# RchalYang/torchrl

Hardware: AMD Instinct MI355X
Metric: env_steps_per_sec_ppo_2048env_halfcheetah_shape (higher is better)
Workload: dtype f32

## Files before the change

include/trl_hip.h:

```cpp
#ifndef TRL_HIP_H
#define TRL_HIP_H
#include <stdint.h>
#ifdef __cplusplus
extern "C" {
#endif

#define TRL_OK            0
#define TRL_EINVAL       -1
#define TRL_EUNSUPPORTED -2

#define TRL_ACT_TANH 0
#define TRL_ACT_RELU 1
#define TRL_ACT_NONE 2

const char* trl_last_error(void);
int trl_abi_version(void);

int trl_gae_f32(const float* rewards, const float* values, const float* terminals,
                const float* time_limits, const float* last_value, const float* last_terminal,
                float* advs, float* rets, int T, int N,
                float gamma, float tau, int tl_filter, void* stream);
int trl_discount_reward_f32(const float* rewards, const float* values, const float* terminals,
                            const float* time_limits, const float* last_value, const float* last_terminal,
                            float* advs, float* rets, int T, int N,
                            float gamma, int tl_filter, void* stream);

int trl_gather_rows_f32(const float* src, const int64_t* row_idx, float* dst,
                        int n_rows, int64_t row_elems, int64_t src_rows, void* stream);
int trl_gather_rows_u8(const uint8_t* src, const int64_t* row_idx, uint8_t* dst,
                       int n_rows, int64_t row_bytes, int64_t src_rows, void* stream);
int trl_gather_rows_multi(const void* const* src, void* const* dst, const int64_t* row_bytes, int n_keys,
                          const int64_t* row_idx, const double* update_count, int n_rows, int64_t src_rows,
                          void* stream);

int trl_adv_stats_f64(const float* advs, const int64_t* row_idx, int n_mb, int rows_mb,
                      int N, double* raw_out, void* stream);
int64_t trl_ppo_epoch_prologue_workspace(int n_mb);
int trl_ppo_epoch_prologue_f64(const float* advs, const int64_t* row_idx, int n_mb, int rows_mb, int N, double* raw_out,
                               void* workspace, double* zero, int64_t zero_doubles, int n_copies, void* const* copy_dst,
                               const void* const* copy_src, const int64_t* copy_words, void* stream);

int trl_mlp2_forward_f32(const float* params, const float* x, float* out,
                         int M, int D, int H, int O, int act, void* stream);
int trl_mlp2_forward_supported(int D, int H, int O);

typedef struct trl_rollout_t {
  const float* pf_params;
  const float* vf_params;
  int D, H, A, act;
  int tanh_action;
  const float* env_A;
  const float* env_B;
  float reward_scale;
  int horizon;
  int64_t env_seed_base;
  float*   cur_obs;
  int32_t* t_env;
  int32_t* cur_step;
  int32_t* episode_idx;
  float*   ep_return;
  const float* noise;
  int64_t noise_step0;
  int deterministic;
  float *obs, *next_obs, *acts, *values, *rewards, *terminals, *time_limits;
  float *old_logp;
  int rows, top;
  int N, n_steps;
  int max_episode_frames;
  float discount;
  double*  epoch_reward;
  int32_t* ep_count;
  float*   ep_log;
  int ep_cap;
  int step0;
  double* norm_state;
  float*  policy_obs;
  double* norm_workspace;
  float norm_clip;
  int norm_update;
  int normalize_partial_reset;
  double* clear_header;
  float* boot_values;
  void* publish_dst; const void* publish_src; int64_t publish_words;
  const uint32_t* noise_flag; uint32_t noise_stamp;
  const float* stage_src; float* stage_dst; int64_t stage_n;
  const uint32_t* stage_ready; uint32_t stage_job; uint32_t* stage_state; uint32_t* stage_ack;
  void* value_wait_event;
} trl_rollout_t;
int trl_rollout_synth_f32(const trl_rollout_t* args, void* stream);
int trl_rollout_supported(int D, int H, int A, int act);
int trl_rollout_synth_cat_f32(const trl_rollout_t* args, int64_t noise_seed, int64_t env_offset, void* stream);
int trl_rollout_cat_supported(int D, int H, int A, int act);
int trl_rollout_synth_sd_f32(const trl_rollout_t* args, void* stream);
int trl_rollout_sd_supported(int D, int H, int A, int act);
int trl_stage_h2d_f32(const float* host_src, float* dev_dst, int64_t n, uint32_t* state, uint32_t stamp, void* stream);
int trl_rollout_norm_workspace(int N);
int trl_rollout_norm_max_envs(int D, int H, int A, int act);

int trl_synth_reset_f32(float* cur_obs, int32_t* t_env, int32_t* cur_step, int32_t* episode_idx,
                        float* ep_return, const uint8_t* mask, int N, int D, int64_t env_seed_base,
                        void* stream);

int trl_gauss_logp_f32(const float* mean, const float* acts, const float* logstd, float* out,
                       int B, int A, int tanh_action, void* stream);

#define TRL_LOSS_PPO_CLIP 0
#define TRL_LOSS_A2C      1
#define TRL_LOSS_REINFORCE 2
typedef struct trl_ppo_batch_t {
  const float *obs, *acts, *advs, *rets, *old_values, *old_logp;
  const int64_t* row_idx;
  int rows_mb, N;
  const double* adv_raw;
  double n_global;
  const float* pf_params; const float* vf_params;
  int D, H, A, act;
  float clip_para, entropy_coeff;
  int clipped_value_loss, tanh_action;
  int loss_mode;
  float* partial;
  double* scal_partial;
  int n_wg;
  int n_wg_pf;
} trl_ppo_batch_t;
int trl_ppo_partial_stride(int D, int H, int A);
int trl_ppo_wg_split(int D, int H, int A, int n_tiles, int n_wg);
int trl_ppo_minibatch_grad_f32(const trl_ppo_batch_t* args, void* stream);
int trl_ppo_reduce_f32(const float* partial, const double* scal_partial, int n_wg, int n_wg_pf,
                       int D, int H, int A, const float* pf_params, float* grads, double* info,
                       void* stream);

int trl_ppo_generic_losses_workspace(int B, int A);
int trl_ppo_generic_losses_f32(const float* mean, const float* logstd, const float* acts, const float* advs,
                               const float* old_logp, const float* v, const float* rets, const float* v_old,
                               const double* adv_raw, double n_global, int B, int A, float clip_para,
                               float entropy_coeff, int clipped_value_loss, int tanh_action, int loss_mode,
                               float* d_mean, float* d_v, float* d_logstd, double* info, double* workspace,
                               void* stream);
int trl_cat_losses_workspace(int B, int A);
int trl_cat_losses_f32(const float* logits, const float* acts, const float* advs, const float* old_logp, const float* v,
                       const float* rets, const float* v_old, const double* adv_raw, double n_global, int B, int A,
                       float clip_para, float entropy_coeff, int clipped_value_loss, int loss_mode, float* d_logits,
                       float* d_v, double* info, double* workspace, void* stream);
int trl_gauss_sd_losses_workspace(int B, int A);
int trl_gauss_sd_losses_f32(const float* head, const float* acts, const float* advs, const float* old_logp, const float* v,
                            const float* rets, const float* v_old, const double* adv_raw, double n_global, int B, int A,
                            float clip_para, float entropy_coeff, int clipped_value_loss, int tanh_action, int loss_mode,
                            float* d_head, float* d_v, double* info, double* workspace, void* stream);

int trl_adv_normalize_f32(const float* advs, const double* adv_raw, double n_global, int B, float eps, float* out,
                          void* stream);
int trl_mse_value_loss_f32(const float* v, const float* rets, int B, double n_global, float* d_v, double* loss_sum,
                           void* stream);
int trl_vmpo_losses_workspace(int n, int A);
int trl_vmpo_losses_f32(const float* mean, const float* target_mean, const float* logstd, const float* target_logstd,
                        const float* acts, const float* adv_n, float* dual_state, int n, int A, int tanh_action,
                        float eta_eps, float alpha_eps, float dual_lr, float* d_mean, float* d_logstd, double* info,
                        double* workspace, void* stream);

int trl_trpo_surrogate_workspace(int n, int A);
int trl_trpo_surrogate_f32(const float* mean, const float* logstd, const float* acts, const float* adv_n, int n, int A,
                           int tanh_action, float entropy_coeff, float* d_mean, float* d_logstd, double* info,
                           double* workspace, void* stream);
int trl_jvp_gate_f32(const float* a, const float* b, const float* h, int act, int64_t n, float* out, void* stream);
int trl_fisher_scale_f32(const float* d_mu, const float* logstd, int n, int A, float* out, void* stream);
int trl_ratio_loss_f32(const float* logp_new, const float* logp_old, const float* adv_n, int n, double* out, void* stream);

typedef struct trl_adam_t {
  float* params; const float* grads; float* exp_avg; float* exp_avg_sq;
  int n_groups;
  int group_sizes[4];
  float group_lr[4];
  float max_norm;
  float beta1, beta2, eps;
  int step_count;
  float grad_scale;
  float* norms_out;
  int device_state;
  double* step_state;
  const float* device_lr;
} trl_adam_t;
int trl_clip_adam_f32(const trl_adam_t* args, void* stream);
int trl_clip_adam_polyak_f32(const trl_adam_t* args, float* target, const float* source, int64_t n, float tau,
                             const void* raw, int raw_bytes, void* ring, int slots, void* stream);
int trl_fold_clip_adam_polyak_workspace(void);
int trl_fold_clip_adam_polyak_f32(int count, const float* const* part, const int* n, const int* splits,
                                  const trl_adam_t* args, float* target, int64_t target_off, int64_t target_n, float tau,
                                  const void* raw, int raw_bytes, void* ring, int slots, void* workspace, void* stream);
int trl_ppo_reduce_adam_workspace(int D, int H, int A);
int trl_ppo_reduce_adam_f32(const float* partial, const double* scal_partial, int n_wg, int n_wg_pf,
                            int D, int H, int A, float* grads, double* info,
                            const trl_adam_t* adam, float* workspace, void* stream);

int trl_ppo_reduce_adam_net_f32(const float* partial, const double* scal_partial, int n_wg, int net,
                                int D, int H, int A, float* grads, double* info,
                                const trl_adam_t* adam, float* workspace, void* stream);

int trl_ppo_cat_supported(int D, int H, int A, int act);
int trl_ppo_cat_partial_stride(int D, int H, int A);
int trl_ppo_cat_minibatch_grad_f32(const trl_ppo_batch_t* args, void* stream);
int trl_ppo_cat_reduce_f32(const float* partial, const double* scal_partial, int n_wg, int n_wg_pf,
                           int D, int H, int A, const float* pf_params, float* grads, double* info,
                           void* stream);
int trl_ppo_cat_reduce_adam_workspace(int D, int H, int A);
int trl_ppo_cat_reduce_adam_f32(const float* partial, const double* scal_partial, int n_wg, int n_wg_pf,
                                int D, int H, int A, float* grads, double* info,
                                const trl_adam_t* adam, float* workspace, void* stream);
int trl_ppo_cat_reduce_adam_net_f32(const float* partial, const double* scal_partial, int n_wg, int net,
                                    int D, int H, int A, float* grads, double* info,
                                    const trl_adam_t* adam, float* workspace, void* stream);

int trl_ppo_sd_supported(int D, int H, int A, int act);
int trl_ppo_sd_partial_stride(int D, int H, int A);
int trl_ppo_sd_scalar_stride(void);
int trl_ppo_sd_minibatch_grad_f32(const trl_ppo_batch_t* args, void* stream);
int trl_ppo_sd_reduce_f32(const float* partial, const double* scal_partial, int n_wg, int n_wg_pf,
                          int D, int H, int A, const float* pf_params, float* grads, double* info,
                          void* stream);
int trl_ppo_sd_reduce_adam_workspace(int D, int H, int A);
int trl_ppo_sd_reduce_adam_f32(const float* partial, const double* scal_partial, int n_wg, int n_wg_pf,
                               int D, int H, int A, float* grads, double* info,
                               const trl_adam_t* adam, float* workspace, void* stream);
int trl_ppo_sd_reduce_adam_net_f32(const float* partial, const double* scal_partial, int n_wg, int net,
                                   int D, int H, int A, float* grads, double* info,
                                   const trl_adam_t* adam, float* workspace, void* stream);

typedef struct trl_comm trl_comm_t;
int trl_comm_unique_id_bytes(void);
int trl_comm_peer_handle_bytes(void);
int trl_comm_max_ranks(void);
int trl_comm_get_unique_id(void* id_out);
int trl_comm_init(trl_comm_t** comm, int rank, int world, const void* unique_id);
int trl_comm_peer_export(trl_comm_t* comm, void* handle_out);
int trl_comm_peer_open(trl_comm_t* comm, const void* handles);
int trl_comm_peer_ready(const trl_comm_t* comm);
int trl_comm_set_wait_footprint(trl_comm_t* comm, int blocks);
int trl_comm_peer_buffer_kind(const trl_comm_t* comm);
int trl_comm_peer_enable(trl_comm_t* comm, int on);
int trl_comm_has_rccl(const trl_comm_t* comm);
int trl_comm_error(trl_comm_t* comm);
int trl_comm_error_peek(trl_comm_t* comm);
int trl_comm_error_detail(trl_comm_t* comm, int32_t* out);
int trl_comm_link_info(int dev_a, int dev_b, int32_t* out);
int trl_comm_destroy(trl_comm_t* comm);
int trl_allreduce_sum_f32(float* buf, int64_t n, trl_comm_t* comm, void* stream);
int trl_allreduce_f64(double* buf, int64_t n, int period, uint64_t max_mask, trl_comm_t* comm, void* stream);
int trl_ppo_reduce_adam_xrank_f32(const float* partial, const double* scal_partial, int n_wg, int n_wg_pf,
                                  int D, int H, int A, float* grads, double* info,
                                  const trl_adam_t* adam, float* workspace, trl_comm_t* comm, void* stream);
int trl_ppo_reduce_adam_xrank_net_f32(const float* partial, const double* scal_partial, int n_wg, int net,
                                      int D, int H, int A, float* grads, double* info,
                                      const trl_adam_t* adam, float* workspace, trl_comm_t* comm, void* stream);

int trl_linear_fwd_f32(const float* x, const float* w, const float* bias, float* y,
                       int M, int K, int N, int act, void* stream);
int trl_linear_fwd_workspace(int M, int K, int N);
int trl_linear_fwd_splitk_group_f32(int G, const float* const* x, const float* const* w, const float* const* bias,
                                    float* const* y, int M, int K, int N, int act, float* workspace, void* stream);
int trl_linear_fwd_splitk_f32(const float* x, const float* w, const float* bias, float* y,
                              int M, int K, int N, int act, float* workspace, void* stream);
int trl_linear_bwd_input_f32(const float* dy, const float* y_gate, int gate_act, const float* w,
                             float* dx, int M, int K, int N, void* stream);
int trl_linear_bwd_input_workspace(int M, int K, int N);
int trl_linear_bwd_input_splitk_f32(const float* dy, const float* y_gate, int gate_act, const float* w, float* dx,
                                    float* workspace, int M, int K, int N, void* stream);
int trl_linear_bwd_weight_workspace(int M, int K, int N);
int trl_linear_bwd_weight_f32(const float* dy, const float* y_gate, int gate_act, const float* x,
                              float* dw, float* db, float* workspace, int M, int K, int N,
                              void* stream);
int trl_linear_fwd_group_f32(int G, const float* const* x, const float* const* w, const float* const* bias,
                             float* const* y, int M, int K, int N, int act, void* stream);
int trl_linear_bwd_input_group_f32(int G, const float* const* dy, const float* const* y_gate, int gate_act,
                                   const float* const* w, float* const* dx, int M, int K, int N, void* stream);
int trl_linear_bwd_weight_group_f32(int G, const float* const* dy, const float* const* y_gate, int gate_act,
                                    const float* const* x, float* const* dw, float* const* db, float* workspace,
                                    int M, int K, int N, void* stream);

int trl_linear_bwd_weight_splits(int M, int K, int N);
int trl_linear_bwd_weight_partials_group_f32(int G, const float* const* dy, const float* const* y_gate, int gate_act,
                                             const float* const* x, int want_db, float* workspace, int M, int K,
                                             int N, void* stream);
int trl_fold_partials_multi_f32(int count, const float* const* part, float* const* out, const int* n,
                                const int* splits, void* stream);
int trl_fold_scope_begin(void);
int trl_fold_scope_end(void* stream);
int trl_linear_bwd_weight_multi_splits(int M, int K, int N);
int trl_linear_bwd_weight_partials_multi_f32(int G, const float* const* dy, const float* const* y_gate, int gate_act,
                                             const float* const* x, const int* K, const int* N, int want_db,
                                             float* const* workspace, int M, void* stream);

int trl_mlp3_forward_ok(int D, int H1, int H2, int O);
int trl_mlp3_forward_group_f32(int G, const float* const* x, const float* const* w1, const float* const* b1,
                               const float* const* w2, const float* const* b2, const float* const* w3,
                               const float* const* b3, float* const* h1, float* const* h2, float* const* y, int M,
                               int D, int O, int act, int last_act, void* stream);

int trl_concat2_f32(const float* a, const float* b, float* out, int rows, int fa, int fb, void* stream);
int trl_tanh_gauss_rsample_fwd_f32(const float* head, const float* eps, float* act, float* logp,
                                   int B, int A, int tanh_action, void* stream);
int trl_tanh_gauss_rsample_bwd_f32(const float* head, const float* eps, const float* act,
                                   const float* d_act, const float* d_logp_ptr, float d_logp_mul,
                                   float w_std, float w_mean, float* d_head, int B, int A,
                                   int tanh_action, void* stream);
int trl_tanh_gauss_rsample_bwd_cols_f32(const float* head, const float* eps, const float* act, const float* dx1,
                                        const float* dx2, int ld, int off, const float* d_logp_ptr,
                                        float d_logp_mul, float w_std, float w_mean, float* d_head, int B,
                                        int A, int tanh_action, void* stream);
int trl_sac_policy_grad_supported(int H, int A);
int trl_sac_policy_grad_f32(int n, const float* const* dy, const float* const* y, int gate_act, const float* const* w,
                            int H, int ldw, int off, const float* head, const float* eps, const float* act,
                            const float* d_logp_ptr, float d_logp_mul, float w_std, float w_mean, float* d_head, int B,
                            int A, int tanh_action, const float* head_w, const float* head_h, int head_act, float* head_dz,
                            void* stream);
int trl_sac_samples_f32(const float* head, const float* head2, float* eps1, const float* eps2,
                        const double* step_state, int64_t seed, const float* obs, const float* acts,
                        const float* next_obs, float* new_a, float* logp, float* next_a, float* next_logp,
                        float* x_sa, float* x_next, float* x_new, int B, int D, int A, int tanh_action,
                        double* mom_part, void* stream);
int trl_sac_alpha_step_f32(const float* logp, int B, float target_entropy, float lr, float beta1,
                           float beta2, float eps, float* state, float* out, void* stream);
int trl_sac_losses_f32(const float* q1, const float* q2, const float* tq1, const float* tq2,
                       const float* logp_next, const float* rew, const float* term, const float* q1n,
                       const float* q2n, const float* logp, const float* alpha, float gamma, int B,
                       float* dq1, float* dq2, float* dq1n, float* dq2n, double* sums,
                       float* alpha_state, float* alpha_out, float target_entropy, float lr, float beta1,
                       float beta2, float eps, const double* mom_part, int A, double* mom_out, void* stream);
int trl_sacv_samples_f32(const float* head, float* eps, const double* step_state, int64_t seed, const float* obs,
                         const float* acts, float* new_a, float* logp, float* x_sa, float* x_new, int B, int D, int A,
                         int tanh_action, double* mom_part, void* stream);
int trl_sacv_losses_f32(const float* q1, const float* q2, const float* tv, const float* rew, const float* term,
                        const float* v, const float* q1n, const float* q2n, const float* logp, const float* alpha,
                        float gamma, int B, int n, float* dq1, float* dq2, float* dv, float* dq1n, float* dq2n,
                        double* sums, float* alpha_state, float* alpha_out, float target_entropy, float lr, float beta1,
// ... 179 lines not shown
```

torchrl_amd/_C.py:

```python
import ctypes as C
import os

import torch

_HERE = os.path.dirname(os.path.abspath(__file__))
LIB_PATH = os.environ.get("TRL_LIB") or os.path.join(_HERE, "lib", "libtrl_hip.so")
_lib = None

ACT_TANH, ACT_RELU, ACT_NONE = 0, 1, 2
ACT_CODES = {"tanh": ACT_TANH, "relu": ACT_RELU}

c_float_p = C.POINTER(C.c_float)
c_double_p = C.POINTER(C.c_double)
c_i64_p = C.POINTER(C.c_int64)
c_i32_p = C.POINTER(C.c_int32)
c_u8_p = C.POINTER(C.c_uint8)


EAGER_FALLBACKS = {}


def note_eager(site, why=""):
    EAGER_FALLBACKS[site] = EAGER_FALLBACKS.get(site, 0) + 1
    if os.environ.get("TRL_STRICT") == "1":
        raise TrlError("%s left the HIP path (%s) and TRL_STRICT=1" % (site, why))
    if EAGER_FALLBACKS[site] == 1:
        import logging
        logging.getLogger("torchrl_amd").warning("%s: a CUDA tensor takes the eager PyTorch route (%s); "
                                                 "this is outside the HIP hot path", site, why)


def eager_fallback_count():
    return sum(EAGER_FALLBACKS.values())


class TrlError(RuntimeError):
    pass


class RolloutArgs(C.Structure):
    _fields_ = [
        ("pf_params", C.c_void_p), ("vf_params", C.c_void_p),
        ("D", C.c_int), ("H", C.c_int), ("A", C.c_int), ("act", C.c_int),
        ("tanh_action", C.c_int),
        ("env_A", C.c_void_p), ("env_B", C.c_void_p),
        ("reward_scale", C.c_float), ("horizon", C.c_int), ("env_seed_base", C.c_int64),
        ("cur_obs", C.c_void_p), ("t_env", C.c_void_p), ("cur_step", C.c_void_p),
        ("episode_idx", C.c_void_p), ("ep_return", C.c_void_p),
        ("noise", C.c_void_p), ("noise_step0", C.c_int64), ("deterministic", C.c_int),
        ("obs", C.c_void_p), ("next_obs", C.c_void_p), ("acts", C.c_void_p), ("values", C.c_void_p),
        ("rewards", C.c_void_p), ("terminals", C.c_void_p), ("time_limits", C.c_void_p),
        ("old_logp", C.c_void_p),
        ("rows", C.c_int), ("top", C.c_int), ("N", C.c_int), ("n_steps", C.c_int),
        ("max_episode_frames", C.c_int), ("discount", C.c_float),
        ("epoch_reward", C.c_void_p), ("ep_count", C.c_void_p), ("ep_log", C.c_void_p),
        ("ep_cap", C.c_int), ("step0", C.c_int),
        ("norm_state", C.c_void_p), ("policy_obs", C.c_void_p), ("norm_workspace", C.c_void_p),
        ("norm_clip", C.c_float), ("norm_update", C.c_int), ("normalize_partial_reset", C.c_int),
        ("clear_header", C.c_void_p), ("boot_values", C.c_void_p),
        ("publish_dst", C.c_void_p), ("publish_src", C.c_void_p), ("publish_words", C.c_int64),
        ("noise_flag", C.c_void_p), ("noise_stamp", C.c_uint32),
        ("stage_src", C.c_void_p), ("stage_dst", C.c_void_p), ("stage_n", C.c_int64),
        ("stage_ready", C.c_void_p), ("stage_job", C.c_uint32), ("stage_state", C.c_void_p), ("stage_ack", C.c_void_p),
        ("value_wait_event", C.c_void_p),
    ]


LOSS_PPO_CLIP, LOSS_A2C, LOSS_REINFORCE = 0, 1, 2


class PpoBatchArgs(C.Structure):
    _fields_ = [
        ("obs", C.c_void_p), ("acts", C.c_void_p), ("advs", C.c_void_p), ("rets", C.c_void_p),
        ("old_values", C.c_void_p), ("old_logp", C.c_void_p),
        ("row_idx", C.c_void_p), ("rows_mb", C.c_int), ("N", C.c_int),
        ("adv_raw", C.c_void_p), ("n_global", C.c_double),
        ("pf_params", C.c_void_p), ("vf_params", C.c_void_p),
        ("D", C.c_int), ("H", C.c_int), ("A", C.c_int), ("act", C.c_int),
        ("clip_para", C.c_float), ("entropy_coeff", C.c_float),
        ("clipped_value_loss", C.c_int), ("tanh_action", C.c_int), ("loss_mode", C.c_int),
        ("partial", C.c_void_p), ("scal_partial", C.c_void_p), ("n_wg", C.c_int), ("n_wg_pf", C.c_int),
    ]


class AdamArgs(C.Structure):
    _fields_ = [
        ("params", C.c_void_p), ("grads", C.c_void_p), ("exp_avg", C.c_void_p), ("exp_avg_sq", C.c_void_p),
        ("n_groups", C.c_int), ("group_sizes", C.c_int * 4), ("group_lr", C.c_float * 4),
        ("max_norm", C.c_float), ("beta1", C.c_float), ("beta2", C.c_float), ("eps", C.c_float),
        ("step_count", C.c_int), ("grad_scale", C.c_float), ("norms_out", C.c_void_p),
        ("device_state", C.c_int), ("step_state", C.c_void_p), ("device_lr", C.c_void_p),
    ]


def adam_args(flat, grads, m, v, sizes, lrs, *, offset=0, max_norm=0.0, eps=1e-8, grad_scale=1.0, norms_out=None,
              step_state=None, step_count=0, device_state=0, device_lr=None):
    a = AdamArgs()
    a.params, a.grads, a.exp_avg, a.exp_avg_sq = (t.data_ptr() + int(offset) * t.element_size() for t in (flat, grads, m, v))
    a.n_groups = len(sizes)
    for k, (size, lr) in enumerate(zip(sizes, lrs)):
        a.group_sizes[k], a.group_lr[k] = size, lr
    a.max_norm, a.beta1, a.beta2, a.eps = max_norm, 0.9, 0.999, eps
    a.step_count, a.grad_scale, a.norms_out, a.step_state = step_count, grad_scale, norms_out, step_state
    a.device_state, a.device_lr = device_state, device_lr
    return a


class ConvRiders(C.Structure):
    _fields_ = [("n_perm", C.c_int), ("perm_src", C.c_void_p * 4), ("perm_dst", C.c_void_p * 4), ("perm_cout", C.c_int * 4),
                ("perm_c", C.c_int * 4), ("perm_khw", C.c_int * 4), ("n_dx", C.c_int), ("dx_w", C.c_void_p * 4),
                ("dx_ws", C.c_void_p * 4), ("dx_cin", C.c_int * 4), ("dx_cout", C.c_int * 4), ("dx_kh", C.c_int * 4),
                ("dx_kw", C.c_int * 4), ("dx_sh", C.c_int * 4), ("dx_sw", C.c_int * 4)]


SIGNATURES = {
    "trl_last_error": (C.c_char_p, []),
    "trl_abi_version": (C.c_int, []),
    "trl_gae_f32": (C.c_int, [C.c_void_p] * 8 + [C.c_int, C.c_int, C.c_float, C.c_float, C.c_int, C.c_void_p]),
    "trl_discount_reward_f32": (C.c_int, [C.c_void_p] * 8 + [C.c_int, C.c_int, C.c_float, C.c_int, C.c_void_p]),
    "trl_gather_rows_f32": (C.c_int, [C.c_void_p, C.c_void_p, C.c_void_p, C.c_int, C.c_int64, C.c_int64, C.c_void_p]),
    "trl_gather_rows_u8": (C.c_int, [C.c_void_p, C.c_void_p, C.c_void_p, C.c_int, C.c_int64, C.c_int64, C.c_void_p]),
    "trl_gather_rows_multi": (C.c_int, [C.c_void_p, C.c_void_p, C.c_void_p, C.c_int, C.c_void_p, C.c_void_p, C.c_int,
                                       C.c_int64, C.c_void_p]),
    "trl_adv_stats_f64": (C.c_int, [C.c_void_p, C.c_void_p, C.c_int, C.c_int, C.c_int, C.c_void_p, C.c_void_p]),
    "trl_ppo_epoch_prologue_workspace": (C.c_int64, [C.c_int]),
    "trl_ppo_epoch_prologue_f64": (C.c_int, [C.c_void_p, C.c_void_p, C.c_int, C.c_int, C.c_int, C.c_void_p, C.c_void_p,
                                           C.c_void_p, C.c_int64, C.c_int, C.c_void_p, C.c_void_p, C.c_void_p, C.c_void_p]),
    "trl_mlp2_forward_f32": (C.c_int, [C.c_void_p, C.c_void_p, C.c_void_p, C.c_int, C.c_int, C.c_int, C.c_int, C.c_int, C.c_void_p]),
    "trl_rollout_synth_f32": (C.c_int, [C.POINTER(RolloutArgs), C.c_void_p]),
    "trl_rollout_supported": (C.c_int, [C.c_int, C.c_int, C.c_int, C.c_int]),
    "trl_rollout_synth_cat_f32": (C.c_int, [C.POINTER(RolloutArgs), C.c_int64, C.c_int64, C.c_void_p]),
    "trl_rollout_cat_supported": (C.c_int, [C.c_int, C.c_int, C.c_int, C.c_int]),
    "trl_rollout_synth_sd_f32": (C.c_int, [C.POINTER(RolloutArgs), C.c_void_p]),
    "trl_rollout_sd_supported": (C.c_int, [C.c_int, C.c_int, C.c_int, C.c_int]),
    "trl_stage_h2d_f32": (C.c_int, [C.c_void_p, C.c_void_p, C.c_int64, C.c_void_p, C.c_uint32, C.c_void_p]),
    "trl_ppo_partial_stride": (C.c_int, [C.c_int, C.c_int, C.c_int]),
    "trl_mlp2_forward_supported": (C.c_int, [C.c_int, C.c_int, C.c_int]),
    "trl_ppo_minibatch_grad_f32": (C.c_int, [C.POINTER(PpoBatchArgs), C.c_void_p]),
    "trl_ppo_wg_split": (C.c_int, [C.c_int, C.c_int, C.c_int, C.c_int, C.c_int]),
    "trl_rollout_norm_workspace": (C.c_int, [C.c_int]),
    "trl_rollout_norm_max_envs": (C.c_int, [C.c_int, C.c_int, C.c_int, C.c_int]),
    "trl_frame_stream_append_u8": (C.c_int, [C.c_void_p, C.c_void_p, C.c_void_p, C.c_void_p, C.c_int, C.c_int, C.c_int, C.c_int, C.c_int, C.c_void_p]),
    "trl_frame_stream_gather_u8": (C.c_int, [C.c_void_p, C.c_void_p, C.c_void_p, C.c_int, C.c_int, C.c_void_p, C.c_void_p, C.c_void_p,
                                             C.c_int, C.c_int, C.c_int, C.c_int, C.c_void_p]),
    "trl_detac_losses_f32": (C.c_int, [C.c_void_p] * 7 + [C.c_float, C.c_int] + [C.c_void_p] * 5),
    "trl_noisy_action_f32": (C.c_int, [C.c_void_p, C.c_void_p, C.c_float, C.c_float, C.c_float, C.c_float, C.c_void_p, C.c_int64, C.c_void_p]),
    "trl_gauss_explore_f32": (C.c_int, [C.c_void_p, C.c_void_p, C.c_void_p, C.c_void_p, C.c_void_p, C.c_int, C.c_int, C.c_int, C.c_void_p]),
    "trl_onpolicy_bookkeep_f32": (C.c_int, [C.c_void_p, C.c_void_p, C.c_void_p, C.c_float, C.c_void_p, C.c_void_p, C.c_void_p, C.c_int,
                                            C.c_void_p, C.c_void_p, C.c_void_p, C.c_void_p, C.c_void_p, C.c_int, C.c_int, C.c_int, C.c_void_p]),
    "trl_select_on_flag_f32": (C.c_int, [C.c_void_p, C.c_void_p, C.c_void_p, C.c_void_p, C.c_int64, C.c_void_p]),
    "trl_comm_unique_id_bytes": (C.c_int, []),
    "trl_comm_peer_handle_bytes": (C.c_int, []),
    "trl_comm_max_ranks": (C.c_int, []),
    "trl_comm_get_unique_id": (C.c_int, [C.c_void_p]),
    "trl_comm_init": (C.c_int, [C.POINTER(C.c_void_p), C.c_int, C.c_int, C.c_void_p]),
    "trl_comm_peer_export": (C.c_int, [C.c_void_p, C.c_void_p]),
    "trl_comm_peer_open": (C.c_int, [C.c_void_p, C.c_void_p]),
    "trl_comm_peer_ready": (C.c_int, [C.c_void_p]),
    "trl_comm_peer_enable": (C.c_int, [C.c_void_p, C.c_int]),
    "trl_comm_has_rccl": (C.c_int, [C.c_void_p]),
    "trl_comm_error": (C.c_int, [C.c_void_p]),
    "trl_comm_error_peek": (C.c_int, [C.c_void_p]),
    "trl_comm_error_detail": (C.c_int, [C.c_void_p, C.c_void_p]),
    "trl_comm_link_info": (C.c_int, [C.c_int, C.c_int, C.c_void_p]),
    "trl_comm_set_wait_footprint": (C.c_int, [C.c_void_p, C.c_int]),
    "trl_comm_peer_buffer_kind": (C.c_int, [C.c_void_p]),
    "trl_comm_destroy": (C.c_int, [C.c_void_p]),
    "trl_allreduce_sum_f32": (C.c_int, [C.c_void_p, C.c_int64, C.c_void_p, C.c_void_p]),
    "trl_allreduce_f64": (C.c_int, [C.c_void_p, C.c_int64, C.c_int, C.c_uint64, C.c_void_p, C.c_void_p]),
    "trl_ppo_reduce_adam_xrank_f32": (C.c_int, [C.c_void_p, C.c_void_p, C.c_int, C.c_int, C.c_int, C.c_int, C.c_int, C.c_void_p,
                                                C.c_void_p, C.POINTER(AdamArgs), C.c_void_p, C.c_void_p, C.c_void_p]),
    "trl_select_on_mask_f32": (C.c_int, [C.c_void_p, C.c_int, C.c_void_p, C.c_void_p, C.c_void_p, C.c_int64, C.c_void_p]),
    "trl_norm_update_filt_f32": (C.c_int, [C.c_void_p, C.c_void_p, C.c_void_p, C.c_int, C.c_int, C.c_float, C.c_int, C.c_void_p]),
    "trl_norm_batch_moments_f64": (C.c_int, [C.c_void_p, C.c_int, C.c_int, C.c_void_p, C.c_void_p]),
    "trl_norm_shard_moments_f64": (C.c_int, [C.c_void_p, C.c_void_p, C.c_int, C.c_int, C.c_void_p, C.c_void_p]),
    "trl_norm_shard_merge_f64": (C.c_int, [C.c_void_p, C.c_void_p, C.c_int, C.c_void_p]),
    "trl_norm_merge_f64": (C.c_int, [C.c_void_p, C.c_void_p, C.c_int, C.c_void_p]),
    "trl_norm_filt_f32": (C.c_int, [C.c_void_p, C.c_void_p, C.c_void_p, C.c_int, C.c_int, C.c_float, C.c_void_p]),
    "trl_ppo_reduce_f32": (C.c_int, [C.c_void_p, C.c_void_p, C.c_int, C.c_int, C.c_int, C.c_int, C.c_int, C.c_void_p, C.c_void_p, C.c_void_p, C.c_void_p]),
    "trl_clip_adam_f32": (C.c_int, [C.POINTER(AdamArgs), C.c_void_p]),
    "trl_clip_adam_polyak_f32": (C.c_int, [C.POINTER(AdamArgs), C.c_void_p, C.c_void_p, C.c_int64, C.c_float, C.c_void_p, C.c_int,
                                          C.c_void_p, C.c_int, C.c_void_p]),
    "trl_ppo_reduce_adam_workspace": (C.c_int, [C.c_int, C.c_int, C.c_int]),
    "trl_ppo_reduce_adam_f32": (C.c_int, [C.c_void_p, C.c_void_p, C.c_int, C.c_int, C.c_int, C.c_int, C.c_int, C.c_void_p, C.c_void_p,
                                          C.POINTER(AdamArgs), C.c_void_p, C.c_void_p]),
    "trl_ppo_reduce_adam_net_f32": (C.c_int, [C.c_void_p, C.c_void_p, C.c_int, C.c_int, C.c_int, C.c_int, C.c_int, C.c_void_p, C.c_void_p,
                                              C.POINTER(AdamArgs), C.c_void_p, C.c_void_p]),
    "trl_ppo_reduce_adam_xrank_net_f32": (C.c_int, [C.c_void_p, C.c_void_p, C.c_int, C.c_int, C.c_int, C.c_int, C.c_int, C.c_void_p,
                                                    C.c_void_p, C.POINTER(AdamArgs), C.c_void_p, C.c_void_p, C.c_void_p]),
    "trl_ppo_cat_supported": (C.c_int, [C.c_int, C.c_int, C.c_int, C.c_int]),
    "trl_ppo_cat_partial_stride": (C.c_int, [C.c_int, C.c_int, C.c_int]),
    "trl_ppo_cat_minibatch_grad_f32": (C.c_int, [C.POINTER(PpoBatchArgs), C.c_void_p]),
    "trl_ppo_cat_reduce_f32": (C.c_int, [C.c_void_p, C.c_void_p, C.c_int, C.c_int, C.c_int, C.c_int, C.c_int, C.c_void_p, C.c_void_p, C.c_void_p, C.c_void_p]),
    "trl_ppo_cat_reduce_adam_workspace": (C.c_int, [C.c_int, C.c_int, C.c_int]),
    "trl_ppo_cat_reduce_adam_f32": (C.c_int, [C.c_void_p, C.c_void_p, C.c_int, C.c_int, C.c_int, C.c_int, C.c_int, C.c_void_p, C.c_void_p,
                                              C.POINTER(AdamArgs), C.c_void_p, C.c_void_p]),
    "trl_ppo_cat_reduce_adam_net_f32": (C.c_int, [C.c_void_p, C.c_void_p, C.c_int, C.c_int, C.c_int, C.c_int, C.c_int, C.c_void_p, C.c_void_p,
                                                  C.POINTER(AdamArgs), C.c_void_p, C.c_void_p]),
    "trl_ppo_sd_supported": (C.c_int, [C.c_int, C.c_int, C.c_int, C.c_int]),
    "trl_ppo_sd_partial_stride": (C.c_int, [C.c_int, C.c_int, C.c_int]),
    "trl_ppo_sd_scalar_stride": (C.c_int, []),
    "trl_ppo_sd_minibatch_grad_f32": (C.c_int, [C.POINTER(PpoBatchArgs), C.c_void_p]),
    "trl_ppo_sd_reduce_f32": (C.c_int, [C.c_void_p, C.c_void_p, C.c_int, C.c_int, C.c_int, C.c_int, C.c_int, C.c_void_p, C.c_void_p, C.c_void_p, C.c_void_p]),
    "trl_ppo_sd_reduce_adam_workspace": (C.c_int, [C.c_int, C.c_int, C.c_int]),
    "trl_ppo_sd_reduce_adam_f32": (C.c_int, [C.c_void_p, C.c_void_p, C.c_int, C.c_int, C.c_int, C.c_int, C.c_int, C.c_void_p, C.c_void_p,
                                              C.POINTER(AdamArgs), C.c_void_p, C.c_void_p]),
    "trl_ppo_sd_reduce_adam_net_f32": (C.c_int, [C.c_void_p, C.c_void_p, C.c_int, C.c_int, C.c_int, C.c_int, C.c_int, C.c_void_p, C.c_void_p,
                                                  C.POINTER(AdamArgs), C.c_void_p, C.c_void_p]),
    "trl_synth_reset_f32": (C.c_int, [C.c_void_p] * 6 + [C.c_int, C.c_int, C.c_int64, C.c_void_p]),
    "trl_gauss_logp_f32": (C.c_int, [C.c_void_p] * 4 + [C.c_int, C.c_int, C.c_int, C.c_void_p]),
    "trl_concat2_f32": (C.c_int, [C.c_void_p] * 3 + [C.c_int] * 3 + [C.c_void_p]),
    "trl_tanh_gauss_rsample_fwd_f32": (C.c_int, [C.c_void_p] * 4 + [C.c_int] * 3 + [C.c_void_p]),
    "trl_tanh_gauss_rsample_bwd_f32": (C.c_int, [C.c_void_p] * 5 + [C.c_float] * 3 + [C.c_void_p] + [C.c_int] * 3 + [C.c_void_p]),
    "trl_tanh_gauss_rsample_bwd_cols_f32": (C.c_int, [C.c_void_p] * 5 + [C.c_int] * 2 + [C.c_void_p] + [C.c_float] * 3 +
                                            [C.c_void_p] + [C.c_int] * 3 + [C.c_void_p]),
    "trl_fold_clip_adam_polyak_workspace": (C.c_int, []),
    "trl_fold_clip_adam_polyak_f32": (C.c_int, [C.c_int, C.c_void_p, C.c_void_p, C.c_void_p, C.POINTER(AdamArgs), C.c_void_p,
                                              C.c_int64, C.c_int64, C.c_float, C.c_void_p, C.c_int, C.c_void_p, C.c_int,
                                              C.c_void_p, C.c_void_p]),
    "trl_fold_scope_begin": (C.c_int, []),
    "trl_fold_scope_end": (C.c_int, [C.c_void_p]),
    "trl_sac_policy_grad_supported": (C.c_int, [C.c_int, C.c_int]),
    "trl_sac_policy_grad_f32": (C.c_int, [C.c_int, C.c_void_p, C.c_void_p, C.c_int, C.c_void_p, C.c_int, C.c_int, C.c_int] +
                                [C.c_void_p] * 4 + [C.c_float] * 3 + [C.c_void_p, C.c_int, C.c_int, C.c_int] +
                                [C.c_void_p, C.c_void_p, C.c_int, C.c_void_p, C.c_void_p]),
    "trl_sac_samples_f32": (C.c_int, [C.c_void_p] * 5 + [C.c_int64] + [C.c_void_p] * 10 + [C.c_int] * 4 +
                            [C.c_void_p, C.c_void_p]),
    "trl_moments_multi_f64": (C.c_int, [C.c_int] + [C.c_void_p] * 9 + [C.c_int, C.c_void_p, C.c_int, C.c_void_p, C.c_void_p]),
    "trl_sac_losses_f32": (C.c_int, [C.c_void_p] * 11 + [C.c_float, C.c_int] + [C.c_void_p] * 7 + [C.c_float] * 5 +
                           [C.c_void_p, C.c_int, C.c_void_p, C.c_void_p]),
    "trl_sacv_samples_f32": (C.c_int, [C.c_void_p] * 3 + [C.c_int64] + [C.c_void_p] * 6 + [C.c_int] * 4 +
                             [C.c_void_p, C.c_void_p]),
    "trl_sacv_losses_f32": (C.c_int, [C.c_void_p] * 10 + [C.c_float, C.c_int, C.c_int] + [C.c_void_p] * 8 + [C.c_float] * 5 +
                            [C.c_void_p, C.c_int, C.c_void_p, C.c_void_p]),
    "trl_synth_collect_step_f32": (C.c_int, [C.c_void_p] * 3 + [C.c_int64, C.c_int64, C.c_int] + [C.c_void_p] * 6 +
                                   [C.c_float, C.c_int, C.c_int, C.c_int64] + [C.c_void_p] * 6 + [C.c_int, C.c_void_p] +
                                   [C.c_void_p] * 4 + [C.c_int] * 6 + [C.c_void_p]),
    "trl_collector_bookkeep_f32": (C.c_int, [C.c_void_p] * 4 + [C.c_int] + [C.c_void_p] * 4 + [C.c_int] * 3 + [C.c_void_p]),
    "trl_sac_alpha_step_f32": (C.c_int, [C.c_void_p, C.c_int] + [C.c_float] * 5 + [C.c_void_p] * 3),
    "trl_slice_add_f32": (C.c_int, [C.c_void_p] * 3 + [C.c_int] * 4 + [C.c_void_p]),
    "trl_polyak_f32": (C.c_int, [C.c_void_p, C.c_void_p, C.c_int64, C.c_float, C.c_void_p]),
    "trl_philox_normal_f32": (C.c_int, [C.c_void_p, C.c_int64, C.c_int64, C.c_int64, C.c_void_p]),
    "trl_synth_env_step_f32": (C.c_int, [C.c_void_p] * 5 + [C.c_float, C.c_int] + [C.c_void_p] * 3 + [C.c_int] * 3 + [C.c_void_p]),
    "trl_im2col_f32": (C.c_int, [C.c_void_p, C.c_void_p] + [C.c_int] * 8 + [C.c_void_p]),
    "trl_im2col_u8_nchw": (C.c_int, [C.c_void_p, C.c_void_p] + [C.c_int] * 8 + [C.c_float, C.c_float, C.c_void_p]),
    "trl_col2im_f32": (C.c_int, [C.c_void_p, C.c_void_p] + [C.c_int] * 8 + [C.c_void_p]),
    "trl_conv_bwd_input_nhwc_ok": (C.c_int, [C.c_int] * 6),
    "trl_conv_bwd_input_nhwc_workspace": (C.c_int, [C.c_int] * 4),
    "trl_conv_bwd_input_nhwc_f32": (C.c_int, [C.c_void_p, C.c_void_p, C.c_int, C.c_void_p, C.c_void_p, C.c_void_p, C.c_int,
                                             C.c_void_p] + [C.c_int] * 10 + [C.c_void_p]),
    "trl_conv_bwd_input_nhwc_prep_f32": (C.c_int, [C.c_int] + [C.c_void_p] * 8 + [C.c_void_p]),
    "trl_transpose_bpc_gate_f32": (C.c_int, [C.c_void_p, C.c_void_p, C.c_int, C.c_int, C.c_void_p] + [C.c_int] * 3
                                   + [C.c_void_p]),
    "trl_transpose_bpc_f32": (C.c_int, [C.c_void_p, C.c_void_p] + [C.c_int] * 3 + [C.c_void_p]),
    "trl_conv_fwd_u8_f32": (C.c_int, [C.c_void_p] * 4 + [C.c_int] * 8 + [C.c_float, C.c_float, C.c_int, C.c_int] +
                            [C.POINTER(ConvRiders), C.c_void_p]),
    "trl_conv_fwd_u8_pair_f32": (C.c_int, [C.c_void_p] * 8 + [C.c_int] * 8 + [C.c_float, C.c_float, C.c_int, C.c_int] +
                                 [C.POINTER(ConvRiders), C.c_void_p]),
    "trl_conv_bwd_weight_workspace": (C.c_int, [C.c_int] * 9),
    "trl_conv_fwd_nhwc_f32": (C.c_int, [C.c_void_p] * 4 + [C.c_int] * 12 + [C.c_void_p]),
    "trl_conv_bwd_weight_nhwc_f32": (C.c_int, [C.c_void_p, C.c_void_p, C.c_int] + [C.c_void_p] * 4 + [C.c_int] * 9
                                     + [C.c_void_p]),
    "trl_conv_bwd_weight_u8_f32": (C.c_int, [C.c_void_p, C.c_void_p, C.c_int] + [C.c_void_p] * 4 + [C.c_int] * 8
                                   + [C.c_float, C.c_float, C.c_int, C.c_void_p]),
    "trl_dqn_td_loss_f32": (C.c_int, [C.c_void_p] * 6 + [C.c_float, C.c_int, C.c_int, C.c_void_p, C.c_void_p, C.c_void_p,
                                     C.c_int, C.c_void_p, C.c_void_p]),
    "trl_dqn_head_supported": (C.c_int, [C.c_int, C.c_int]),
    "trl_dqn_head_workspace": (C.c_int64, [C.c_int, C.c_int]),
    "trl_dqn_head_f32": (C.c_int, [C.c_void_p] * 10 + [C.c_float, C.c_int, C.c_int, C.c_int] + [C.c_void_p] * 7 +
                         [C.c_int, C.c_void_p, C.c_void_p, C.c_void_p]),
    "trl_quantile_huber_f32": (C.c_int, [C.c_void_p] * 6 + [C.c_float, C.c_int, C.c_int, C.c_int] + [C.c_void_p] * 4 +
                               [C.c_int, C.c_void_p, C.c_void_p]),
    "trl_boot_act_i64": (C.c_int, [C.c_void_p, C.c_void_p, C.c_int, C.c_int, C.c_int, C.c_void_p, C.c_void_p, C.c_void_p,
                                   C.c_void_p]),
    "trl_boot_heads_i64": (C.c_int, [C.c_void_p, C.c_void_p, C.c_int, C.c_int, C.c_int64, C.c_int64, C.c_int64, C.c_void_p]),
    "trl_boot_masks_f32": (C.c_int, [C.c_void_p, C.c_int, C.c_int, C.c_float, C.c_int64, C.c_int64, C.c_int64, C.c_void_p]),
    "trl_boot_td_loss_workspace": (C.c_int64, []),
    "trl_boot_td_loss_f32": (C.c_int, [C.c_void_p] * 7 + [C.c_float, C.c_int, C.c_int, C.c_int, C.c_void_p, C.c_void_p,
                                                          C.c_void_p, C.c_int, C.c_void_p, C.c_void_p, C.c_void_p]),
    "trl_boot_fold_f32": (C.c_int, [C.c_void_p, C.c_void_p, C.c_int, C.c_int64, C.c_void_p]),
    "trl_dqn_act_supported": (C.c_int, [C.c_int, C.c_int]),
    "trl_dqn_act_f32": (C.c_int, [C.c_void_p, C.c_void_p, C.c_void_p, C.c_int, C.c_int, C.c_int, C.c_void_p, C.c_void_p, C.c_float,
                                  C.c_void_p, C.c_void_p, C.c_void_p, C.c_int, C.c_void_p]),
    "trl_eps_greedy_i64": (C.c_int, [C.c_void_p, C.c_int, C.c_int, C.c_int, C.c_void_p, C.c_void_p, C.c_float, C.c_void_p, C.c_void_p,
                                     C.c_int, C.c_void_p]),
    "trl_synth_frames_step_u8": (C.c_int, [C.c_void_p] * 3 + [C.c_int64, C.c_int, C.c_int] + [C.c_void_p] * 3 + [C.c_int] * 3 + [C.c_void_p]),
    "trl_synth_frames_reset_u8": (C.c_int, [C.c_void_p, C.c_void_p, C.c_int64, C.c_void_p, C.c_void_p] + [C.c_int] * 4 + [C.c_void_p]),
    "trl_synth_frames_collect_u8": (C.c_int, [C.c_void_p] * 3 + [C.c_int64, C.c_int, C.c_int] + [C.c_void_p] * 7 + [C.c_int] +
                                    [C.c_void_p] * 2 + [C.c_void_p, C.c_void_p, C.c_int, C.c_void_p, C.c_void_p, C.c_void_p,
                                                        C.c_void_p, C.c_int, C.c_int] + [C.c_int] * 3 + [C.c_void_p]),
    "trl_linear_fwd_f32": (C.c_int, [C.c_void_p] * 4 + [C.c_int, C.c_int, C.c_int, C.c_int, C.c_void_p]),
    "trl_mt19937_advance": (C.c_int, [C.c_void_p, C.c_void_p, C.c_void_p, C.c_int64]),
# ... 141 lines not shown
        k = self._k
        dst.copy_(self._bufs[k], non_blocking=True)
        if dst.is_cuda:
            ev = self._events[k] or torch.cuda.Event()
            ev.record(torch.cuda.current_stream(dst.device))
            self._events[k] = ev
        self._k = (k + 1) % len(self._bufs)
        return dst


def gae(rewards, values, terminals, time_limits, last_value, advs, rets, gamma, tau, tl_filter,
        last_terminal=None):
    T, N = rewards.shape[0], rewards.shape[1]
    check(lib().trl_gae_f32(dev_ptr(rewards, name="rewards"), dev_ptr(values, name="values"),
                            dev_ptr(terminals, name="terminals"),
                            dev_ptr(time_limits, name="time_limits", allow_none=not tl_filter),
                            dev_ptr(last_value, name="last_value"),
                            dev_ptr(last_terminal, name="last_terminal", allow_none=True),
                            dev_ptr(advs, name="advs"),
                            dev_ptr(rets, name="rets"), T, N, float(gamma), float(tau), int(bool(tl_filter)),
                            stream_ptr(rewards.device)), "trl_gae_f32")


def discount_reward(rewards, values, terminals, time_limits, last_value, advs, rets, gamma, tl_filter,
                    last_terminal=None):
    T, N = rewards.shape[0], rewards.shape[1]
    check(lib().trl_discount_reward_f32(dev_ptr(rewards, name="rewards"), dev_ptr(values, name="values"),
                                        dev_ptr(terminals, name="terminals"),
                                        dev_ptr(time_limits, name="time_limits", allow_none=not tl_filter),
                                        dev_ptr(last_value, name="last_value"),
                                        dev_ptr(last_terminal, name="last_terminal", allow_none=True),
                                        dev_ptr(advs, name="advs"),
                                        dev_ptr(rets, name="rets"), T, N, float(gamma), int(bool(tl_filter)),
                                        stream_ptr(rewards.device)), "trl_discount_reward_f32")


def gather_rows(src, row_idx, out=None):
    n = int(row_idx.numel())
    if out is None:
        out = torch.empty((n,) + tuple(src.shape[1:]), dtype=src.dtype, device=src.device)
    row_elems = 1
    for s in src.shape[1:]:
        row_elems *= int(s)
    if src.dtype == torch.float32:
        fn, name = lib().trl_gather_rows_f32, "trl_gather_rows_f32"
    elif src.dtype == torch.uint8:
        fn, name = lib().trl_gather_rows_u8, "trl_gather_rows_u8"
    else:
        raise TrlError("gather_rows: dtype %s not supported" % src.dtype)
    check(fn(dev_ptr(src, src.dtype, "src"), dev_ptr(row_idx, torch.int64, "row_idx"),
             dev_ptr(out, src.dtype, "out"), n, row_elems, int(src.shape[0]), stream_ptr(src.device)), name)
    return out


def gather_rows_multi(srcs, row_idx, outs, slab_counter=None, n_rows=None):
    n, k = int(row_idx.numel()) if slab_counter is None else int(n_rows), len(srcs)
    rows = int(srcs[0].shape[0])
    if any(int(s.shape[0]) != rows for s in srcs):
        raise TrlError("gather_rows_multi: keys with different row counts")
    sp, dp, nb = (C.c_void_p * k)(), (C.c_void_p * k)(), (C.c_int64 * k)()
    for j, (s, o) in enumerate(zip(srcs, outs)):
        if s.dtype != o.dtype or o.numel() != n * s[0].numel():
            raise TrlError("gather_rows_multi: out[%d] does not match the batch" % j)
        sp[j], dp[j] = dev_ptr(s, s.dtype, "src"), dev_ptr(o, o.dtype, "out")
        nb[j] = s[0].numel() * s.element_size()
    check(lib().trl_gather_rows_multi(sp, dp, nb, k, dev_ptr(row_idx, torch.int64, "row_idx"),
                                      dev_ptr(slab_counter, torch.float64, "counter", allow_none=True), n, rows,
                                      stream_ptr(srcs[0].device)), "trl_gather_rows_multi")
    return outs


def adv_stats(advs, row_idx_2d, raw_out):
    n_mb, rows_mb = int(row_idx_2d.shape[0]), int(row_idx_2d.shape[1])
    check(lib().trl_adv_stats_f64(dev_ptr(advs, name="advs"), dev_ptr(row_idx_2d, torch.int64, "row_idx"),
                                  n_mb, rows_mb, int(advs.shape[1]),
                                  dev_ptr(raw_out, torch.float64, "raw_out"), stream_ptr(advs.device)),
          "trl_adv_stats_f64")
    return raw_out


def stage_h2d(host, dev, state, stamp, stream):
    if not (host.is_pinned() and host.dtype == torch.float32 and host.is_contiguous() and host.numel() == dev.numel()):
        raise TrlError("stage_h2d: a contiguous page-locked float32 source of the destination's size is required")
    check(lib().trl_stage_h2d_f32(C.c_void_p(host.data_ptr()), dev_ptr(dev, name="dev"), host.numel(),
                                  dev_ptr(state, torch.int32, "state"), int(stamp) & 0xFFFFFFFF,
                                  C.c_void_p(stream.cuda_stream)), "trl_stage_h2d_f32")


def ppo_epoch_prologue_workspace(n_mb, device):
    return torch.zeros(int(lib().trl_ppo_epoch_prologue_workspace(int(n_mb))), dtype=torch.uint8, device=device)


def _mapped_ptr(t, name):
    if not isinstance(t, torch.Tensor) or not t.is_contiguous():
        raise TrlError("%s must be a contiguous tensor" % name)
    if t.device.type != "cuda" and not t.is_pinned():
        raise TrlError("%s lives in pageable host memory: the device cannot read it" % name)
    return C.c_void_p(t.data_ptr())


def ppo_epoch_prologue(advs, row_idx_2d, raw_out, workspace, zero=None, copies=()):
    n_mb, rows_mb = int(row_idx_2d.shape[0]), int(row_idx_2d.shape[1])
    if row_idx_2d.dtype != torch.int64:
        raise TrlError("row_idx must be int64")
    n = len(copies)
    dsts, srcs, words = (C.c_void_p * max(n, 1))(), (C.c_void_p * max(n, 1))(), (C.c_int64 * max(n, 1))()
    for q, (dst, src) in enumerate(copies):
        nb = dst.numel() * dst.element_size()
        if nb != src.numel() * src.element_size() or nb % 4:
            raise TrlError("ppo_epoch_prologue: copy %d needs two tensors of one byte size, a multiple of 4" % q)
        dsts[q], srcs[q], words[q] = dev_ptr(dst, dst.dtype, "copy_dst").value, _mapped_ptr(src, "copy_src").value, nb // 4
    check(lib().trl_ppo_epoch_prologue_f64(
        dev_ptr(advs, name="advs"), _mapped_ptr(row_idx_2d, "row_idx"), n_mb, rows_mb, int(advs.shape[1]),
        dev_ptr(raw_out, torch.float64, "raw_out"), dev_ptr(workspace, torch.uint8, "workspace", allow_none=True),
        dev_ptr(zero, torch.float64, "zero", allow_none=True), 0 if zero is None else zero.numel(),
        n, dsts, srcs, words, stream_ptr(advs.device)), "trl_ppo_epoch_prologue_f64")
    return raw_out


def mlp2_forward(params, x, D, H, O, act, out=None):
    M = int(x.shape[0])
    if out is None:
        out = torch.empty((M, O), dtype=torch.float32, device=x.device)
    check(lib().trl_mlp2_forward_f32(dev_ptr(params, name="params"), dev_ptr(x, name="x"),
                                     dev_ptr(out, name="out"), M, D, H, O, act, stream_ptr(x.device)),
          "trl_mlp2_forward_f32")
    return out


def rollout(args, device):
    check(lib().trl_rollout_synth_f32(C.byref(args), stream_ptr(device)), "trl_rollout_synth_f32")


def rollout_cat(args, noise_seed, env_offset, device):
    check(lib().trl_rollout_synth_cat_f32(C.byref(args), int(noise_seed), int(env_offset), stream_ptr(device)),
          "trl_rollout_synth_cat_f32")


def rollout_sd(args, device):
    check(lib().trl_rollout_synth_sd_f32(C.byref(args), stream_ptr(device)), "trl_rollout_synth_sd_f32")


def _partial_stride(name, D, H, A):
    ps = getattr(lib(), name)(D, H, A)
    if ps < 0:
        check(ps, name)
    return ps


def ppo_partial_stride(D, H, A):
    return _partial_stride("trl_ppo_partial_stride", D, H, A)


def ppo_cat_partial_stride(D, H, A):
    return _partial_stride("trl_ppo_cat_partial_stride", D, H, A)


def ppo_cat_minibatch_grad(args, device):
    check(lib().trl_ppo_cat_minibatch_grad_f32(C.byref(args), stream_ptr(device)), "trl_ppo_cat_minibatch_grad_f32")


def ppo_cat_reduce(partial, scal_partial, n_wg, D, H, A, grads, info, n_wg_pf=0):
    check(lib().trl_ppo_cat_reduce_f32(dev_ptr(partial, name="partial"),
                                       dev_ptr(scal_partial, torch.float64, "scal_partial"), n_wg, n_wg_pf, D, H, A,
                                       None, dev_ptr(grads, name="grads"), dev_ptr(info, torch.float64, "info"),
                                       stream_ptr(partial.device)), "trl_ppo_cat_reduce_f32")


def ppo_sd_partial_stride(D, H, A):
    return _partial_stride("trl_ppo_sd_partial_stride", D, H, A)


def ppo_sd_scalar_stride():
    return lib().trl_ppo_sd_scalar_stride()


def ppo_sd_minibatch_grad(args, device):
    check(lib().trl_ppo_sd_minibatch_grad_f32(C.byref(args), stream_ptr(device)), "trl_ppo_sd_minibatch_grad_f32")


def ppo_sd_reduce(partial, scal_partial, n_wg, D, H, A, grads, info, n_wg_pf=0):
    check(lib().trl_ppo_sd_reduce_f32(dev_ptr(partial, name="partial"),
                                      dev_ptr(scal_partial, torch.float64, "scal_partial"), n_wg, n_wg_pf, D, H, A,
                                      None, dev_ptr(grads, name="grads"), dev_ptr(info, torch.float64, "info"),
                                      stream_ptr(partial.device)), "trl_ppo_sd_reduce_f32")


def ppo_minibatch_grad(args, device):
    check(lib().trl_ppo_minibatch_grad_f32(C.byref(args), stream_ptr(device)), "trl_ppo_minibatch_grad_f32")


def ppo_reduce(partial, scal_partial, n_wg, D, H, A, grads, info, pf_params=None, n_wg_pf=0):
    check(lib().trl_ppo_reduce_f32(dev_ptr(partial, name="partial"),
                                   dev_ptr(scal_partial, torch.float64, "scal_partial"), n_wg, n_wg_pf, D, H, A,
                                   dev_ptr(pf_params, name="pf_params", allow_none=True),
                                   dev_ptr(grads, name="grads"), dev_ptr(info, torch.float64, "info"),
                                   stream_ptr(partial.device)), "trl_ppo_reduce_f32")


def clip_adam(args, device):
    check(lib().trl_clip_adam_f32(C.byref(args), stream_ptr(device)), "trl_clip_adam_f32")


def clip_adam_polyak(args, target, source, tau, device, file=None):
    raw, ring = file if file is not None else (None, None)
    if ring is not None and (ring.dim() != 2 or int(ring.shape[1]) != raw.numel() or not ring.is_contiguous()):
        raise TrlError("clip_adam_polyak: ring rows must be statistics blocks")
    check(lib().trl_clip_adam_polyak_f32(C.byref(args), dev_ptr(target, name="target"), dev_ptr(source, name="source"),
                                         int(target.numel()), float(tau), dev_ptr(raw, torch.uint8, "raw", allow_none=True),
                                         0 if raw is None else int(raw.numel()),
                                         dev_ptr(ring, torch.uint8, "ring", allow_none=True),
                                         0 if ring is None else int(ring.shape[0]), stream_ptr(device)),
          "trl_clip_adam_polyak_f32")


def fold_clip_adam_polyak_workspace(device):
    return torch.zeros(int(lib().trl_fold_clip_adam_polyak_workspace()), dtype=torch.uint8, device=device)


def synth_collect_step(env, head, eps, cur_step, ep_return, max_frames, rows, mask, epoch_reward, ep_count, ep_log, step,
                       tanh_action, noise=None):
    N, D, A = int(env.cur_obs.shape[0]), int(env.cur_obs.shape[1]), int(head.shape[1]) // 2
    obs_row, acts_row, next_row, rew_row, done_row, tl_row = rows
    seed, ctr, row0 = noise if eps is None else (0, 0, 0)
    check(lib().trl_synth_collect_step_f32(
        dev_ptr(env.cur_obs, name="cur_obs"), dev_ptr(head, name="head"), dev_ptr(eps, name="eps", allow_none=True),
        int(seed), int(ctr), int(row0), dev_ptr(env.env_A, name="env_A"), dev_ptr(env.env_B, name="env_B"), dev_ptr(env.t_env, torch.int32, "t_env"),
        dev_ptr(cur_step, torch.int32, "cur_step"), dev_ptr(env.episode_idx, torch.int32, "episode_idx"),
        dev_ptr(ep_return, name="ep_return"), float(env.effective_reward_scale), int(env.horizon), int(max_frames),
        int(env.seed_base), dev_ptr(obs_row, name="obs_row", allow_none=True),
        dev_ptr(acts_row, name="acts_row", allow_none=True), dev_ptr(next_row, name="next_row"),
        dev_ptr(rew_row, name="rew_row"), dev_ptr(done_row, name="done_row"),
        dev_ptr(tl_row, name="tl_row", allow_none=True), 0, None, dev_ptr(mask, torch.uint8, "mask"),
        dev_ptr(epoch_reward, torch.float64, "epoch_reward"), dev_ptr(ep_count, torch.int32, "ep_count"),
        dev_ptr(ep_log, name="ep_log"), int(ep_log.shape[0]), int(step), N, D, A, int(bool(tanh_action)),
        stream_ptr(head.device)), "trl_synth_collect_step_f32")


def synth_collect_step_dyn(env, head, cur_step, ep_return, max_frames, ring, state, mask, epoch_reward, ep_count, ep_log,
                           tanh_action, noise_seed, noise_row0):
    N, D, A = int(env.cur_obs.shape[0]), int(env.cur_obs.shape[1]), int(head.shape[1]) // 2
    check(lib().trl_synth_collect_step_f32(
        dev_ptr(env.cur_obs, name="cur_obs"), dev_ptr(head, name="head"), None, int(noise_seed), 0, int(noise_row0),
        dev_ptr(env.env_A, name="env_A"), dev_ptr(env.env_B, name="env_B"), dev_ptr(env.t_env, torch.int32, "t_env"),
        dev_ptr(cur_step, torch.int32, "cur_step"), dev_ptr(env.episode_idx, torch.int32, "episode_idx"),
        dev_ptr(ep_return, name="ep_return"), float(env.effective_reward_scale), int(env.horizon), int(max_frames),
        int(env.seed_base), *[dev_ptr(t, name="ring") for t in ring], int(ring[0].shape[0]),
        dev_ptr(state, torch.int64, "state"), dev_ptr(mask, torch.uint8, "mask"),
        dev_ptr(epoch_reward, torch.float64, "epoch_reward"), dev_ptr(ep_count, torch.int32, "ep_count"),
        dev_ptr(ep_log, name="ep_log"), int(ep_log.shape[0]), 0, N, D, A, int(bool(tanh_action)), stream_ptr(head.device)),
        "trl_synth_collect_step_f32")


def synth_reset(cur_obs, t_env, cur_step, episode_idx, ep_return, mask, seed_base):
    N, D = int(cur_obs.shape[0]), int(cur_obs.shape[1])
    check(lib().trl_synth_reset_f32(dev_ptr(cur_obs, name="cur_obs"), dev_ptr(t_env, torch.int32, "t_env"),
                                    dev_ptr(cur_step, torch.int32, "cur_step"),
                                    dev_ptr(episode_idx, torch.int32, "episode_idx"),
                                    dev_ptr(ep_return, name="ep_return"),
                                    dev_ptr(mask, torch.uint8, "mask", allow_none=True), N, D, int(seed_base),
                                    stream_ptr(cur_obs.device)), "trl_synth_reset_f32")


def gauss_logp(mean, acts, logstd, tanh_action, out=None):
    B, A = int(mean.shape[0]), int(mean.shape[1])
    if out is None:
        out = torch.empty((B,), dtype=torch.float32, device=mean.device)
    check(lib().trl_gauss_logp_f32(dev_ptr(mean, name="mean"), dev_ptr(acts, name="acts"),
                                   dev_ptr(logstd, name="logstd"), dev_ptr(out, name="out"), B, A,
                                   int(bool(tanh_action)), stream_ptr(mean.device)), "trl_gauss_logp_f32")
    return out


def linear_fwd(x, w, bias, act):
    M, K = int(x.shape[0]), int(x.shape[1])
    N = int(w.shape[0])
    y = torch.empty((M, N), dtype=torch.float32, device=x.device)
    need = lib().trl_linear_fwd_workspace(M, K, N)
    if need > 0:
        ws = torch.empty((need,), dtype=torch.float32, device=x.device)
        check(lib().trl_linear_fwd_splitk_f32(dev_ptr(x, name="x"), dev_ptr(w, name="w"),
                                              dev_ptr(bias, name="bias", allow_none=True), dev_ptr(y, name="y"),
                                              M, K, N, act, dev_ptr(ws, name="workspace"), stream_ptr(x.device)),
              "trl_linear_fwd_splitk_f32")
        return y
    check(lib().trl_linear_fwd_f32(dev_ptr(x, name="x"), dev_ptr(w, name="w"),
                                   dev_ptr(bias, name="bias", allow_none=True), dev_ptr(y, name="y"),
                                   M, K, N, act, stream_ptr(x.device)), "trl_linear_fwd_f32")
    return y


def ppo_generic_losses(mean, logstd, acts, advs, old_logp, v, rets, v_old, adv_raw, n_global, clip_para, entropy_coeff,
                       clipped_value_loss, tanh_action, loss_mode, d_logstd, info, workspace=None):
    B, A = int(mean.shape[0]), int(mean.shape[1])
    critic = int(loss_mode) != LOSS_REINFORCE
    need = lib().trl_ppo_generic_losses_workspace(B, A)
    if need < 0:
        raise TrlError("ppo_generic_losses: unsupported sizes B=%d A=%d" % (B, A))
    if workspace is None or workspace.numel() < need:
        workspace = torch.empty((need,), dtype=torch.float64, device=mean.device)
    d_mean = torch.empty((B, A), dtype=torch.float32, device=mean.device)
    d_v = torch.empty((B, 1), dtype=torch.float32, device=mean.device) if critic else None
    check(lib().trl_ppo_generic_losses_f32(
        dev_ptr(mean, name="mean"), dev_ptr(logstd, name="logstd"), dev_ptr(acts, name="acts"), dev_ptr(advs, name="advs"),
        dev_ptr(old_logp, name="old_logp", allow_none=True), dev_ptr(v, name="v", allow_none=not critic),
        dev_ptr(rets, name="rets", allow_none=not critic),
# ... 1309 lines not shown
```

torchrl_amd/algo/on_policy/ppo.py:

```python
import copy
import os
import math

import numpy as np
import torch
import torch.optim as optim

from ... import _C
from ... import dist
from ...networks import flatten_into
from ...policies.continuous_policy import HEAD_CAT, HEAD_GAUSS, HEAD_NAME, HEAD_SD, HEAD_TAG, head_kind, is_state_std
from .. import utils as atu
from .._graphs import GraphCache, LastGraph
from .a2c import A2C

_HALF_LOG_2PI_PLUS_HALF = 0.5 + 0.5 * math.log(2 * math.pi)


def _hyper(algo):
    return (float(getattr(algo, "clip_para", 0.0)), float(algo.entropy_coeff),
            int(bool(getattr(algo, "clipped_value_loss", False))), int(bool(algo.pf.tanh_action)))


def _stat_views(block, K):
    return block[:4 * K].view(K, 4), block[4 * K:28 * K].view(K, 24), block[28 * K:].view(torch.float32).view(K, 2)


class PPO(A2C):
    loss_mode = _C.LOSS_PPO_CLIP

    def __init__(self, pf, clip_para=0.2, opt_epochs=10, clipped_value_loss=False, **kwargs):
        self.target_pf = copy.deepcopy(pf)
        super().__init__(pf=pf, **kwargs)
        self.clip_para = clip_para
        self.opt_epochs = opt_epochs
        self.clipped_value_loss = clipped_value_loss
        self.sample_key = ["obs", "acts", "advs", "estimate_returns", "values"]
        self._engine = None

    @property
    def networks(self):
        return [self.pf, self.vf, self.target_pf]

    def engine(self):
        if self._engine is None:
            if self.optimizer_class is not optim.Adam:
                raise _C.TrlError("the fused PPO step implements torch.optim.Adam only")
            self._engine = make_engine(self)
        return self._engine

    def _fill_old_logp(self):
        buf = self.replay_buffer
        rows, n = buf._max_replay_buffer_size, buf.env_nums
        tgt = self.target_pf
        kind = head_kind(tgt)
        if kind == HEAD_CAT:
            with torch.no_grad():
                _C.cat_logp(tgt.logits(buf._obs.reshape(rows * n, -1)).contiguous(), buf._acts.reshape(rows * n),
                            out=buf._ensure_key("old_logp", (n, 1)).view(rows * n))
            return
        if kind == HEAD_SD:
            from ... import ops
            with torch.no_grad():
                layers, code = ops.net_layers(tgt)
                head, _ = ops.mlp_forward(layers, buf._obs.reshape(rows * n, -1), code, keep=False)
                _C.gauss_sd_logp(head, buf._acts.reshape(rows * n, -1), bool(tgt.tanh_action),
                                 out=buf._ensure_key("old_logp", (n, 1)).view(rows * n))
            return
        with torch.no_grad():
            mean, _, log_std = tgt.forward(buf._obs.reshape(rows * n, -1))
            _C.gauss_logp(mean.contiguous(), buf._acts.reshape(rows * n, -1), log_std.float().contiguous(),
                          bool(tgt.tanh_action), out=buf._ensure_key("old_logp", (n, 1)).view(rows * n))

    def update_per_epoch(self):
        atu.update_linear_schedule(self.pf_optimizer, self.current_epoch, self.num_epochs, self.plr)
        atu.update_linear_schedule(self.vf_optimizer, self.current_epoch, self.num_epochs, self.vlr)
        buf = self.replay_buffer
        buf._scan_inputs()
        buf._ensure_key("old_logp", (buf.env_nums, 1))
        passes = [buf.epoch_row_indices(self.batch_size, self.shuffle) for _ in range(self.opt_epochs)]
        row_idx = np.concatenate(passes, axis=0)
        tensors = {"obs": buf._obs, "acts": buf._acts, "advs": buf._advs, "rets": buf._estimate_returns,
                   "old_values": buf._values, "old_logp": buf._old_logp}
        fresh = bool(getattr(buf, "_old_logp_fresh", False))
        buf._old_logp_fresh = False

        def device_prologue():
            self.process_epoch_samples()
            self.engine().sync_target_pf(in_prologue=True)
            if not fresh:
                self._fill_old_logp()
        self._run_and_log(tensors, row_idx, buf.env_nums, pre=device_prologue,
                          pre_key=(fresh, self.gae, bool(getattr(buf, "_boot_fresh", False))))

    def update(self, batch):
        self.training_update_num += 1
        dev = self.device
        as_t = lambda x: (x if isinstance(x, torch.Tensor) else torch.as_tensor(np.asarray(x))) \
            .to(device=dev, dtype=torch.float32).contiguous()
        obs, acts = as_t(batch['obs']), as_t(batch['acts'])
        B = obs.shape[0]
        if "old_logp" in batch:
            old_lp = as_t(batch["old_logp"]).reshape(B, 1)
        else:
            with torch.no_grad():
                old_lp = self.target_pf.update(obs, acts)["log_prob"].reshape(B, 1).contiguous()
        tensors = {"obs": obs.reshape(1, B, -1), "acts": acts.reshape(1, B, -1),
                   "advs": as_t(batch['advs']).reshape(1, B, 1), "rets": as_t(batch['estimate_returns']).reshape(1, B, 1),
                   "old_values": as_t(batch['values']).reshape(1, B, 1), "old_logp": old_lp.reshape(1, B, 1)}
        return self.engine().run(tensors, np.zeros((1, 1), dtype=np.int64), B)[0]


class _FusedPPO:

    def __init__(self, algo):
        self.algo = algo
        pf, vf = algo.pf, algo.vf
        ps, vs = pf.mlp2_spec(), vf.mlp2_spec()
        needs = "fused PPO needs MLP2 nets and a GuassianContPolicyBasicBias, GuassianContPolicy or CategoricalDisPolicy policy"
        if ps is None or vs is None:
            raise _C.TrlError(needs)
        self.head = head_kind(pf, refuse=needs)
        self.categorical, self.state_std = self.head == HEAD_CAT, self.head == HEAD_SD
        if self.head != HEAD_GAUSS:
            ps = _head_spec(self.head, ps)
            why = _fused_head_refusal(self.head, ps)
            if why:
                raise _C.TrlError(why)
        if vs[0] != ps[0] or vs[1] != ps[1] or vs[2] != 1 or vs[3] != ps[3]:
            raise _C.TrlError("policy %s and value %s must share input, width and activation" % (ps, vs))
        self.D, self.H, self.A, self.act = ps
        self.dev = next(pf.parameters()).device
        if self.dev.type != "cuda":
            raise _C.TrlError("PPO networks live on %s: the fused path needs a GPU (no CPU path exists)" % self.dev)
        tail = (lambda net: []) if (self.categorical or self.state_std) else (lambda net: [net.logstd])
        pf_list = pf._mlp2_param_list() + tail(pf)
        vf_list = vf._mlp2_param_list()
        tgt = getattr(algo, "target_pf", None)
        self._home(pf_list, vf_list, None if tgt is None else tgt._mlp2_param_list() + tail(tgt))
        if tgt is not None and (self.categorical or self.state_std):
            tgt._flat = self.target_flat
        lib = _C.lib()
        sfx = HEAD_TAG[self.head]
        kernel = lambda name: (getattr(lib, name), name)
        self._k_grad = kernel("trl_ppo_%sminibatch_grad_f32" % sfx)
        self._k_fold, self._k_fold_net = kernel("trl_ppo_%sreduce_adam_f32" % sfx), kernel("trl_ppo_%sreduce_adam_net_f32" % sfx)
        self._k_fold_x, self._k_fold_net_x = kernel("trl_ppo_reduce_adam_xrank_f32"), kernel("trl_ppo_reduce_adam_xrank_net_f32")
        self.p_stride = getattr(_C, "ppo_%spartial_stride" % sfx)(self.D, self.H, self.A)
        self.scal_w = _C.ppo_sd_scalar_stride() if self.state_std else 8
        self.n_cu = torch.cuda.get_device_properties(self.dev).multi_processor_count
        self.max_wg = 2 * max(1, self.n_cu // 2)
        self.partial = torch.zeros(self.max_wg, self.p_stride, device=self.dev)
        self.scal = torch.zeros(self.max_wg, self.scal_w, dtype=torch.float64, device=self.dev)
        n_ws = getattr(lib, "trl_ppo_%sreduce_adam_workspace" % sfx)(self.D, self.H, self.A)
        self.red_ws = torch.zeros(n_ws, device=self.dev)
        self.two_chains = os.environ.get("TRL_PPO_CHAINS", "two") != "joint"
        self.red_ws_v = torch.zeros(n_ws, device=self.dev)
        self.red_ws_v[4:8].view(torch.float64).fill_(1.0)
        self._side, self._value_done, self._hdr_owner, self._chain_graphs = None, None, "joint", {}
        self._joint = LastGraph()
        self._pending, self._chain_pend, self._chain_seen = None, [], set()
        self._stats2_key = self._chain_rows = self._pro_ws = None
        self.red_ws[4:8].view(torch.float64).fill_(1.0)

    def _home(self, pf_list, vf_list, target_list):
        self.P_pf = sum(p.numel() for p in pf_list)
        self.P_vf = sum(p.numel() for p in vf_list)
        self.flat = flatten_into(pf_list + vf_list)
        for net, lo, hi in ((self.algo.pf, 0, self.P_pf), (self.algo.vf, self.P_pf, self.P_pf + self.P_vf)):
            if getattr(net, "mlp2_spec", lambda: None)() is not None:
                net._flat = self.flat[lo:hi]
        self.m, self.v, self.grads = torch.zeros_like(self.flat), torch.zeros_like(self.flat), torch.zeros_like(self.flat)
        self.step_count = 0
        self.target_flat = None if target_list is None else flatten_into(target_list)
        self._alias_optimizer_state(self.algo.pf_optimizer, pf_list, 0)
        self._alias_optimizer_state(self.algo.vf_optimizer, vf_list, self.P_pf)

    def _alias_optimizer_state(self, opt, plist, offset):
        self._opt_steps = getattr(self, "_opt_steps", [])
        for p in plist:
            n = p.numel()
            step = torch.tensor(0.0)
            opt.state[p] = {"step": step, "exp_avg": self.m[offset:offset + n].view(p.shape),
                            "exp_avg_sq": self.v[offset:offset + n].view(p.shape)}
            self._opt_steps.append(step)
            offset += n

    def sync_target_pf(self, in_prologue=False):
        if self.target_flat is not None and in_prologue:
            self._copy_in_prologue = True
        elif self.target_flat is not None:
            self.target_flat.copy_(self.flat[:self.P_pf])
        else:
            atu.copy_model_params_from_to(self.algo.pf, self.algo.target_pf)

    def _n_wg(self, n_samples):
        tiles = (n_samples + 15) // 16
        n_wg = 2 * max(1, min(self.max_wg // 2, (tiles + 3) // 4))
        n_pf = _C.lib().trl_ppo_wg_split(self.D, self.H, self.A, tiles, n_wg)
        if not 0 < n_pf < n_wg:
            raise _C.TrlError("trl_ppo_wg_split(%d tiles, %d workgroups) returned %d" % (tiles, n_wg, n_pf))
        if n_wg >= self.n_cu and n_wg % 8 == 0 and n_wg >= 16:
            waves = lambda x: -(-tiles // (4 * x))
            cost = lambda x: max(waves(x) * 15.3, waves(n_wg - x) * 11.8)
            cands = [x for x in (n_pf // 8 * 8, -(-n_pf // 8) * 8) if 0 < x < n_wg]
            if cands:
                n_pf = min(cands, key=lambda x: (cost(x), abs(x - n_pf)))
        return n_wg, n_pf

    def _buffers(self, K, rows_mb):
        key = (K, rows_mb)
        if getattr(self, "_buf_key", None) != key:
            self._buf_key = key
            self._idx_buf = torch.zeros(K * rows_mb, dtype=torch.int64, device=self.dev)
            self._stats = torch.zeros(29 * K, dtype=torch.float64, device=self.dev)
            self._slab_host = torch.zeros(K * rows_mb + 1, dtype=torch.int64).pin_memory()
            self._idx_host = self._slab_host[:K * rows_mb]
            self._hyper_host = self._slab_host[K * rows_mb:].view(torch.float32)
            self._hyper = None
            self._stats_host = torch.zeros(29 * K, dtype=torch.float64).pin_memory()
            if self._joint is not None:
                self._joint.clear()
        return self._idx_buf, self._stats

    @property
    def _graph(self):
        return None if self._joint is None else self._joint.graph

    def _set_device_hyper(self, lr_pf, lr_vf, upload=True):
        hyper = (float(lr_pf), float(lr_vf))
        if getattr(self, "_hyper", None) != hyper or not upload:
            self._hyper = hyper if upload else None
            self._hyper_host[0], self._hyper_host[1] = hyper
            if upload:
                self.red_ws[2:4].copy_(self._hyper_host, non_blocking=True)

    def _adam_args(self, lrs=(0.0, 0.0), **kw):
        return _C.adam_args(self.flat, self.grads, self.m, self.v, (self.P_pf, self.P_vf), lrs, max_norm=0.5, eps=1e-5, **kw)

    def _batch_args(self, t, hyper, loss_mode, rows_mb, N, n_global, partial, scal, n_wg, n_wg_pf):
        g = _C.PpoBatchArgs()
        for k in ("obs", "acts", "advs", "rets", "old_values", "old_logp"):
            setattr(g, k, _C.dev_ptr(t[k], name=k).value if t.get(k) is not None else None)
        g.loss_mode = loss_mode
        g.rows_mb, g.N, g.n_global = rows_mb, N, n_global
        g.pf_params, g.vf_params = self.flat.data_ptr(), self.flat.data_ptr() + 4 * self.P_pf
        g.D, g.H, g.A, g.act = self.D, self.H, self.A, self.act
        g.clip_para, g.entropy_coeff, g.clipped_value_loss, g.tanh_action = hyper
        g.partial, g.scal_partial, g.n_wg, g.n_wg_pf = partial.data_ptr(), scal.data_ptr(), n_wg, n_wg_pf
        return g

    def _prologue(self, pre, advs, idx, raw, zero, copies):
        self._copy_in_prologue = False
        if pre is not None:
            pre()
        if self._pro_ws is None or self._pro_ws_k != tuple(idx.shape):
            self._pro_ws, self._pro_ws_k = _C.ppo_epoch_prologue_workspace(idx.shape[0], self.dev), tuple(idx.shape)
        if self._copy_in_prologue:
            copies = [(self.target_flat, self.flat[:self.P_pf])] + copies
        _C.ppo_epoch_prologue(advs, idx, raw, self._pro_ws, zero=zero, copies=copies)
        dist.reduce_adv_raw_(raw)

    def _fold(self, kernel, partial, scal, n_wg, which, info, ws, comm=False):
        import ctypes as C
        fn, name = kernel
        head = (partial.data_ptr(), scal.data_ptr(), n_wg, which, self.D, self.H, self.A, self.grads.data_ptr())
        tail = (ws.data_ptr(),) + ((dist.comm_handle(),) if comm else ()) + (_C.stream_ptr(self.dev),)
        info_base = info.data_ptr()
        return lambda k, g, a: _C.check(fn(*head, info_base + 192 * k, C.byref(a), *tail), name)

    def _minibatches(self, K, g, a, idx_dev, raw, norms, fold, probe=None):
        import ctypes as C
        stream = _C.stream_ptr(self.dev)
        idx_base, raw_base, norm_base = idx_dev.data_ptr(), raw.data_ptr(), norms.data_ptr()
        for k in range(K):
            g.row_idx = idx_base + 8 * g.rows_mb * k
            g.adv_raw = raw_base + 32 * k
            a.step_count = self.step_count + k + 1
            a.norms_out = norm_base + 8 * k
            if probe is not None:
                ev = (torch.cuda.Event(enable_timing=True), torch.cuda.Event(enable_timing=True))
                ev[0].record()
            _C.check(self._k_grad[0](C.byref(g), stream), self._k_grad[1])
            if probe is not None:
                ev[1].record()
                probe.append(ev)
            fold(k, g, a)

    def _stepped(self, K):
        self.step_count += K
        for s in self._opt_steps:
            s.fill_(float(self.step_count))

    defers = True

    def run(self, t, row_idx, N, pre=None, pre_key=None, defer=False):
        algo, dev = self.algo, self.dev
        K, rows_mb = row_idx.shape
        world = dist.world_size()
        n_local = rows_mb * N
        n_global = float(n_local * world)
        n_wg, n_wg_pf = self._n_wg(n_local)
        loss_mode = int(getattr(algo, "loss_mode", _C.LOSS_PPO_CLIP))
        probe = getattr(self, "probe", None)
        fused = not dist.collectives_active()
        if (self.categorical or self.state_std) and not fused:
            raise _C.TrlError("the fused %s update runs on one rank (no cross-rank fold exists for this head)"
                              % ("categorical" if self.categorical else "state-dependent-std"))
        xrank_chains = not fused and self.chains_across_ranks()
        if (fused or xrank_chains) and probe is None and self.two_chains and n_wg_pf >= 1 and n_wg - n_wg_pf >= 1:
            return self._run_chains(t, row_idx, N, pre, pre_key, defer, n_wg, n_wg_pf, loss_mode, n_global, xrank=not fused)
        for last in [self._pending] + list(self._chain_pend):
            if last is not None:
                last.land()
        self._pending, self._chain_pend = None, []
        idx_dev, stats = self._buffers(K, rows_mb)
        self._idx_host.numpy()[:] = row_idx.reshape(-1)
        rows_total = t["advs"].shape[0]
        raw, info, norms = _stat_views(stats, K)
        xrank = not fused and dist.peer_ready()
        self._settle_value_chain()
        if self._value_done is not None:
            from ...networks import nets as _nets
            _nets.set_pending(algo.vf, None)
            self._value_done = None
        self._hdr_owner = "joint"
        graph_coll = not fused and not xrank and os.environ.get("TRL_GRAPH_COLLECTIVES") == "1"
        lr_pf, lr_vf = algo.pf_optimizer.param_groups[0]['lr'], algo.vf_optimizer.param_groups[0]['lr']
        in_place = fused and probe is None
        if not in_place:
            idx_dev.copy_(self._idx_host, non_blocking=True)
        if fused or xrank:
            self._set_device_hyper(lr_pf, lr_vf, upload=not in_place)
        elif graph_coll:
            if getattr(self, "step_state", None) is None:
                n = float(self.step_count)
                self.step_state = torch.tensor([n, 0.9 ** n, 0.999 ** n, 0.0], dtype=torch.float64, device=dev)
                self.lr_dev = torch.zeros(2, device=dev)
            if getattr(self, "_lr_host", None) != (float(lr_pf), float(lr_vf)):
                self._lr_host = (float(lr_pf), float(lr_vf))
                self.lr_dev.copy_(torch.tensor(self._lr_host, dtype=torch.float32), non_blocking=True)
        hyper = _hyper(algo)
        use_graph = (fused or xrank or graph_coll) and probe is None and os.environ.get("TRL_NO_GRAPH") != "1"
        key = (n_wg, n_wg_pf, loss_mode, n_global, rows_total, N, pre_key, pre is not None, xrank, in_place) + hyper + tuple(
            0 if t.get(k) is None else t[k].data_ptr() for k in ("obs", "acts", "advs", "rets", "old_values", "old_logp"))

        def launch_all():
            g = self._batch_args(t, hyper, loss_mode, rows_mb, N, n_global, self.partial, self.scal, n_wg, n_wg_pf)
            a = self._adam_args((lr_pf, lr_vf), device_state=int(fused or xrank))
            slab = [(idx_dev, self._idx_host), (self.red_ws[2:4], self._hyper_host)] if in_place else []
            self._prologue(pre, t["advs"].reshape(rows_total, N), (self._idx_host if in_place else idx_dev).view(K, rows_mb),
                           raw, stats[4 * K:], slab)
            if fused:
                fold = self._fold(self._k_fold, self.partial, self.scal, n_wg, n_wg_pf, info, self.red_ws)
            elif xrank:
                fold = self._fold(self._k_fold_x, self.partial, self.scal, n_wg, n_wg_pf, info, self.red_ws, comm=True)
            else:
                import ctypes as C
                lib, stream = _C.lib(), _C.stream_ptr(dev)

                def fold(k, g, a):
                    _C.check(lib.trl_ppo_reduce_f32(self.partial.data_ptr(), self.scal.data_ptr(), n_wg, n_wg_pf, self.D,
                                                    self.H, self.A, self.flat.data_ptr(), self.grads.data_ptr(),
                                                    info.data_ptr() + 192 * k, stream), "trl_ppo_reduce_f32")
                    dist.all_reduce_sum_(self.grads)
                    if graph_coll:
                        a.step_count, a.step_state, a.device_lr = 0, self.step_state.data_ptr(), self.lr_dev.data_ptr()
                    _C.check(lib.trl_clip_adam_f32(C.byref(a), stream), "trl_clip_adam_f32")
            self._minibatches(K, g, a, idx_dev, raw, norms, fold, probe)

        self._joint.run(key, launch_all, eager=not use_graph)
        dist.reduce_info_(info)
        self._stats_host.copy_(stats, non_blocking=True)
        landed = torch.cuda.Event()
        landed.record()
        self._stepped(K)
        host = self._stats_host
        make = self._infos_a2c if loss_mode == _C.LOSS_A2C else self._infos

        def build(host):
            if xrank:
                dist.check_comm(peek=True)
            return make(*(v.numpy() for v in _stat_views(host, K)), n_global)
        pending = _PendingInfos(K, landed, host, build)
        if defer:
            self._pending = pending
            return pending
        return pending.resolve()

    def chains_across_ranks(self):
        if not (self.two_chains and dist.collectives_active() and dist.peer_ready()):
            return False
        want = os.environ.get("TRL_PPO_CHAINS_XRANK")
        return want == "1" if want in ("0", "1") else dist.ranks_per_device() == 1

    def _settle_value_chain(self):
        if self._value_done is not None:
            torch.cuda.current_stream(self.dev).wait_event(self._value_done)

    def _sync_headers(self, owner):
        if self._hdr_owner != owner:
            if owner == "two":
                self.red_ws_v[:8].copy_(self.red_ws[:8])
            self._hdr_owner = owner

    def _run_chains(self, t, row_idx, N, pre, pre_key, defer, n_wg, n_wg_pf, loss_mode, n_global, xrank=False):
        algo, dev = self.algo, self.dev
        K, rows_mb = row_idx.shape
        main = torch.cuda.current_stream(dev)
        if self._side is None:
            self._side = torch.cuda.Stream(dev)
        side = self._side
        last = self._pending
        if last is not None:
            last.land()
            self._pending = None
        pend = self._chain_pend
        while len(pend) > (0 if os.environ.get("TRL_CHAIN_HOST_AHEAD") == "0" else 1):
            pend.pop(0).land()
        self._settle_value_chain()
        self._sync_headers("two")
        idx_dev, _ = self._buffers(K, rows_mb)
        if self._stats2_key != (K, rows_mb):
            for q in pend:
                q.land()
            del pend[:]
            self._stats2_key = (K, rows_mb)
            self._stats2 = torch.zeros(2, 29 * K, dtype=torch.float64, device=dev)
            self._chain_host = [(torch.zeros(K * rows_mb + 1, dtype=torch.int64).pin_memory(),
                                 torch.zeros(2, 29 * K, dtype=torch.float64).pin_memory()) for _ in range(2)]
            self._chain_graphs, self._chain_turn = {}, 0
        stats2 = self._stats2
        turn = self._chain_turn = 1 - self._chain_turn
        slab, stats_host = self._chain_host[turn]
        idx_host, hyper_host = slab[:K * rows_mb], slab[K * rows_mb:].view(torch.float32)
        idx_host.numpy()[:] = row_idx.reshape(-1)
        rows_total = t["advs"].shape[0]
        raw = stats2[0, :4 * K].view(K, 4)
        lr_pf, lr_vf = algo.pf_optimizer.param_groups[0]['lr'], algo.vf_optimizer.param_groups[0]['lr']
        hyper_host[0], hyper_host[1] = float(lr_pf), float(lr_vf)
        self._hyper = None
        hyper = _hyper(algo)
        n_wg_vf = n_wg - n_wg_pf
        if self._chain_rows is None:
            self._chain_rows = (torch.zeros(self.max_wg, self.p_stride, device=dev),
                                torch.zeros(self.max_wg, self.scal_w, dtype=torch.float64, device=dev))
        partial_v, scal_v = self._chain_rows
        shape_key = (n_wg, n_wg_pf, loss_mode, n_global, rows_total, N, pre_key, pre is not None, xrank) + hyper
        key = shape_key + (turn,) + tuple(
            0 if t.get(k) is None else t[k].data_ptr() for k in ("obs", "acts", "advs", "rets", "old_values", "old_logp"))

        def head():
            self._prologue(pre, t["advs"].reshape(rows_total, N), idx_host.view(K, rows_mb), raw, stats2.view(-1)[4 * K:],
                           [(idx_dev, idx_host), (self.red_ws[2:4], hyper_host), (self.red_ws_v[2:4], hyper_host)])

        def chain(net):
            part, scal, ws, wgs, wgs_pf = (self.partial, self.scal, self.red_ws, n_wg_pf, n_wg_pf) if net == 0 else \
                (partial_v, scal_v, self.red_ws_v, n_wg_vf, -1)
            g = self._batch_args(t, hyper, loss_mode, rows_mb, N, n_global, part, scal, wgs, wgs_pf)
            a = self._adam_args((lr_pf, lr_vf), device_state=1)
            _, info, norms = _stat_views(stats2[net], K)
            fold = self._fold(self._k_fold_net_x if xrank else self._k_fold_net, part, scal, wgs, net, info, ws, comm=xrank)
            self._minibatches(K, g, a, idx_dev, raw, norms, fold)

        use_graph = os.environ.get("TRL_NO_GRAPH") != "1"
        cache, seen = self._chain_graphs, self._chain_seen
        graphs = cache.get(key) if use_graph else None
        if use_graph and graphs is None and shape_key in seen and len(cache) < 8:
            g0, _ = _C.capture_graph(head)
            gp, _ = _C.capture_graph(lambda: chain(0))
            with torch.cuda.stream(side):
                gv, _ = _C.capture_graph(lambda: chain(1))
            graphs = cache[key] = (g0, gp, gv)
        elif graphs is None:
            seen.add(shape_key)
        run_head, run_p, run_v = (head, lambda: chain(0), lambda: chain(1)) if graphs is None else \
            (graphs[0].replay, graphs[1].replay, graphs[2].replay)
        only = os.environ.get("TRL_CHAIN_ONLY")
        if only == "v":
            run_p = lambda: None
        if only == "p":
            run_v = lambda: None
        run_head()
        forked = torch.cuda.Event()
        forked.record(main)
        run_p()
        if not xrank:
            stats_host[0].copy_(stats2[0], non_blocking=True)
        landed_p = torch.cuda.Event()
        landed_p.record(main)
        with torch.cuda.stream(side):
            side.wait_event(forked)
            if getattr(self, "_test_value_chain_delay", 0):
                torch.cuda._sleep(int(self._test_value_chain_delay))
            run_v()
            if xrank:
                side.wait_event(landed_p)
                for st_ in (stats2[0], stats2[1]):
                    dist.reduce_info_(st_[4 * K:28 * K].view(K, 24))
                stats_host[0].copy_(stats2[0], non_blocking=True)
            stats_host[1].copy_(stats2[1], non_blocking=True)
            done_v = torch.cuda.Event()
            done_v.record(side)
        self._value_done = done_v
        from ...networks import nets as _nets
        _nets.set_pending(algo.vf, done_v)
        self._stepped(K)
        make = self._infos_a2c if loss_mode == _C.LOSS_A2C else self._infos

        class _Both:
            @staticmethod
            def synchronize():
                landed_p.synchronize()
                done_v.synchronize()

        def build(host):
            if xrank:
                dist.check_comm(peek=True)
            (raw, info, norms), (_, info_v, norms_v) = _stat_views(host[0], K), _stat_views(host[1], K)
            info, norms = info.clone(), norms.clone()
            for col in (7, 12, 13, 14, 15):
                info[:, col] = info_v[:, col]
            norms[:, 1] = norms_v[:, 1]
            return make(raw.numpy(), info.numpy(), norms.numpy(), n_global)
        pending = _PendingInfos(K, _Both, stats_host, build)
        if defer:
            pend.append(pending)
            return pending
        out = pending.resolve()
        self._settle_value_chain()
        return out

    def _infos_a2c(self, raw, info, norms, n):
        out = []
        c_ent = float(self.algo.entropy_coeff)
        A = self.A
        categorical, state_std = getattr(self, "categorical", False), getattr(self, "state_std", False)
        for r, i, g in zip(raw, info, norms):
            v_var = max((i[13] - i[12] * i[12] / n) / (n - 1), 0.0)
            if categorical or state_std:
                ent, std_std = i[20] / n, i[17]
            else:
                ent = A * _HALF_LOG_2PI_PLUS_HALF + A * i[8]
                std_ss = (i[17] ** 2) * (A - 1) if A > 1 else 0.0
                std_std = math.sqrt(n * std_ss / (n * A - 1))
            d = {'Training/policy_loss': i[0] / n - c_ent * ent, 'Training/vf_loss': i[7] / n,
                 'v_pred/mean': i[12] / n, 'v_pred/std': math.sqrt(v_var), 'v_pred/max': i[14], 'v_pred/min': -i[15]}
            if not categorical:
                d.update({'std/mean': i[16], 'std/std': std_std, 'std/max': i[18], 'std/min': i[19]})
            d['ent'], d['log_prob'] = ent, i[1] / n
            out.append(d)
        return out

    def _infos(self, raw, info, norms, n):
        c_ent = float(self.algo.entropy_coeff)
        r, i = raw, info
        adv_var = np.maximum((r[:, 1] - r[:, 0] * r[:, 0] / n) / (n - 1), 0.0)
        lp_var = np.maximum((i[:, 2] - i[:, 1] * i[:, 1] / n) / (n - 1), 0.0)
        categorical = getattr(self, "categorical", False)
        ent = i[:, 20] / n if (categorical or getattr(self, "state_std", False)) else \
            self.A * _HALF_LOG_2PI_PLUS_HALF + self.A * i[:, 8]
        cols = (('advs/mean', r[:, 0] / n), ('advs/std', np.sqrt(adv_var)), ('advs/max', r[:, 2]), ('advs/min', -r[:, 3]),
                ('Training/vf_loss', i[:, 7] / n), ('grad_norm/vf', norms[:, 1].astype(np.float64)),
                ('Training/policy_loss', i[:, 0] / n - c_ent * ent),
                ('logprob/mean', i[:, 1] / n), ('logprob/std', np.sqrt(lp_var)), ('logprob/max', i[:, 3]),
                ('logprob/min', -i[:, 4]), ('log_std/mean', i[:, 8]), ('log_std/std', i[:, 9]), ('log_std/max', i[:, 10]),
                ('log_std/min', i[:, 11]), ('ratio/max', i[:, 5]), ('ratio/min', -i[:, 6]),
                ('grad_norm/pf', norms[:, 0].astype(np.float64)))
        if categorical:
            cols = tuple(c for c in cols if not c[0].startswith('log_std/'))
        keys = [k for k, _ in cols]
        table = np.stack([v for _, v in cols], axis=1).tolist()
        return [dict(zip(keys, row)) for row in table]


class _PendingInfos:

    def __init__(self, count, landed, host, build):
        self.count, self._landed, self._host, self._build, self._snap, self._infos = count, landed, host, build, None, None

    def __len__(self):
        return self.count

    def land(self):
        if self._snap is None and self._infos is None:
            self._landed.synchronize()
            self._snap, self._host = self._host.clone(), None

    def resolve(self):
        if self._infos is None:
            self.land()
            self._infos, self._build, self._snap = self._build(self._snap), None, None
        return self._infos


_HEAD_OPT_IN = {HEAD_CAT: "TRL_CAT_FUSED_UPDATE", HEAD_SD: "TRL_SD_FUSED_UPDATE"}


def _head_spec(kind, ps):
    return (ps[0], ps[1], ps[2] // 2, ps[3]) if kind == HEAD_SD else tuple(ps)


def _fused_head_refusal(kind, ps):
    if not getattr(_C.lib(), "trl_ppo_%ssupported" % HEAD_TAG[kind])(*ps):
        return "the fused %s update carries H == 64, 2 <= D <= 32, %d <= A <= 8, Tanh / ReLU; got %s" \
            % (HEAD_NAME[kind], 2 if kind == HEAD_CAT else 1, ps)
    if dist.collectives_active():
        return "the fused %s update runs on one rank (no cross-rank fold exists for this head)" % HEAD_NAME[kind]
    return None


def make_engine(algo):
    pf, vf = algo.pf, algo.vf
# ... 149 lines not shown
```

torchrl_amd/algo/on_policy/reinforce.py:

```python
import math
import os

import numpy as np
import torch
import torch.optim as optim

from ... import _C
from ... import dist
from ...networks import ZeroNet, flatten_into
from ...policies.continuous_policy import HEAD_CAT, HEAD_GAUSS, HEAD_NAME, HEAD_SD, HEAD_TAG, head_kind
from .._graphs import GraphCache, LastGraph
from .a2c import A2C
from .on_rl_algo import OnRLAlgo
from .ppo import (_FusedPPO, _GenericPPO, _HEAD_OPT_IN, _HALF_LOG_2PI_PLUS_HALF, _PendingInfos, _fused_head_refusal,
                  _head_spec, _hyper, _stat_views)

_ONE_RANK = "Reinforce runs on one rank (several ranks are not built: no cross-rank fold of a policy-only update exists)"


class Reinforce(OnRLAlgo):
    loss_mode = _C.LOSS_REINFORCE
    sample_key = ("obs", "acts", "advs")

    def __init__(self, pf=None, plr=None, optimizer_class=optim.Adam, entropy_coeff=0.001, **kwargs):
        if pf is None or plr is None:
            raise _C.TrlError("Reinforce without a policy (`pf`, `plr`) is not built: pass the policy network and its "
                              "learning rate (reference: torchrl/algo/on_policy/reinforce.py)")
        super().__init__(**kwargs)
        self.pf = pf
        self.vf = ZeroNet()
        self.to(self.device)
        self.plr = plr
        self.optimizer_class = optimizer_class
        self.pf_optimizer = optimizer_class(self.pf.parameters(), lr=self.plr)
        self.entropy_coeff = entropy_coeff
        self.gae = False
        self._engine = None

    def engine(self):
        if self._engine is None:
            if self.optimizer_class is not optim.Adam:
                raise _C.TrlError("the Reinforce step implements torch.optim.Adam only")
            self._engine = make_engine(self)
        return self._engine

    _run_and_log = A2C._run_and_log

    def update_per_epoch(self):
        self.process_epoch_samples()
        buf = self.replay_buffer
        row_idx = buf.epoch_row_indices(self.batch_size, self.shuffle)
        tensors = {"obs": buf._obs, "acts": buf._acts, "advs": buf._advs}
        self._run_and_log(tensors, row_idx, buf.env_nums)

    def update(self, batch):
        self.training_update_num += 1
        dev = self.device
        as_t = lambda x: (x if isinstance(x, torch.Tensor) else torch.as_tensor(np.asarray(x))) \
            .to(device=dev, dtype=torch.float32).contiguous()
        obs, acts = as_t(batch['obs']), as_t(batch['acts'])
        B = obs.shape[0]
        tensors = {"obs": obs.reshape(1, B, -1), "acts": acts.reshape(1, B, -1), "advs": as_t(batch['advs']).reshape(1, B, 1)}
        return self.engine().run(tensors, np.zeros((1, 1), dtype=np.int64), B)[0]

    @property
    def snapshot_networks(self):
        return [("pf", self.pf)]


def make_engine(algo):
    if dist.collectives_active() or dist.world_size() > 1:
        raise _C.TrlError(_ONE_RANK)
    pf = algo.pf
    ps = pf.mlp2_spec() if hasattr(pf, "mlp2_spec") else None
    kind = head_kind(pf)
    generic = os.environ.get("TRL_GENERIC_PPO") == "1"
    if kind in _HEAD_OPT_IN:
        if os.environ.get(_HEAD_OPT_IN[kind]) == "1" and not generic and ps is not None \
                and _fused_head_refusal(kind, _head_spec(kind, ps)) is None:
            return _FusedReinforce(algo)
        return _GenericReinforce(algo)
    if ps is not None and hasattr(pf, "logstd") and _C.lib().trl_ppo_partial_stride(ps[0], ps[1], ps[2]) > 0 and not generic:
        return _FusedReinforce(algo)
    return _GenericReinforce(algo)


def _infos_reinforce(engine, raw, info, n):
    c_ent = float(engine.algo.entropy_coeff)
    out = []
    for r, i in zip(raw, info):
        adv_var = max((r[1] - r[0] * r[0] / n) / n, 0.0)
        lp_var = max((i[2] - i[1] * i[1] / n) / (n - 1), 0.0)
        ent = i[20] / n if (engine.categorical or engine.state_std) else \
            engine.A * _HALF_LOG_2PI_PLUS_HALF + engine.A * i[8]
        out.append({'advs/mean': r[0] / n, 'advs/std': math.sqrt(adv_var), 'advs/max': r[2], 'advs/min': -r[3],
                    'Training/policy_loss': i[0] / n - c_ent * ent, 'ent': ent,
                    'logprob/mean': i[1] / n, 'logprob/std': math.sqrt(lp_var), 'logprob/max': i[3], 'logprob/min': -i[4]})
    return [{k: float(v) for k, v in d.items()} for d in out]


class _PolicyOnly:

    def _home(self, pf_list, vf_list, target_list):
        assert not vf_list and target_list is None
        self.P_pf, self.P_vf = sum(p.numel() for p in pf_list), 0
        self.flat = flatten_into(pf_list)
        if getattr(self.algo.pf, "mlp2_spec", lambda: None)() is not None:
            self.algo.pf._flat = self.flat
        self.m, self.v, self.grads = torch.zeros_like(self.flat), torch.zeros_like(self.flat), torch.zeros_like(self.flat)
        self.step_count = 0
        self.target_flat = None
        self._alias_optimizer_state(self.algo.pf_optimizer, pf_list, 0)

    def _adam_args(self, lrs=(0.0,), **kw):
        eps = float(self.algo.pf_optimizer.param_groups[0]['eps'])
        return _C.adam_args(self.flat, self.grads, self.m, self.v, (self.P_pf,), lrs[:1], max_norm=0.5, eps=eps, **kw)

    def _infos_reinforce(self, raw, info, norms, n):
        return _infos_reinforce(self, raw, info, n)


class _FusedReinforce(_PolicyOnly, _FusedPPO):

    def __init__(self, algo):
        self.algo = algo
        pf = algo.pf
        ps = pf.mlp2_spec()
        needs = "fused Reinforce needs an MLP2 GuassianContPolicyBasicBias, GuassianContPolicy or CategoricalDisPolicy policy"
        if ps is None:
            raise _C.TrlError(needs)
        self.head = head_kind(pf, refuse=needs)
        self.categorical, self.state_std = self.head == HEAD_CAT, self.head == HEAD_SD
        if self.head != HEAD_GAUSS:
            ps = _head_spec(self.head, ps)
            why = _fused_head_refusal(self.head, ps)
            if why:
                raise _C.TrlError(why)
        self.D, self.H, self.A, self.act = ps
        self.dev = next(pf.parameters()).device
        if self.dev.type != "cuda":
            raise _C.TrlError("Reinforce networks live on %s: the fused path needs a GPU (no CPU path exists)" % self.dev)
        tail = [] if (self.categorical or self.state_std) else [pf.logstd]
        self._home(pf._mlp2_param_list() + tail, [], None)
        lib = _C.lib()
        sfx = HEAD_TAG[self.head]
        kernel = lambda name: (getattr(lib, name), name)
        self._k_grad = kernel("trl_ppo_%sminibatch_grad_f32" % sfx)
        self._k_fold_net = kernel("trl_ppo_%sreduce_adam_net_f32" % sfx)
        self.p_stride = getattr(_C, "ppo_%spartial_stride" % sfx)(self.D, self.H, self.A)
        if self.p_stride <= 0:
            raise _C.TrlError("fused Reinforce: shape %s is not instantiated in the gradient kernel" % (ps,))
        self.scal_w = _C.ppo_sd_scalar_stride() if self.state_std else 8
        self.n_cu = torch.cuda.get_device_properties(self.dev).multi_processor_count
        self.max_wg = 2 * max(1, self.n_cu // 2)
        self.partial = torch.zeros(self.max_wg, self.p_stride, device=self.dev)
        self.scal = torch.zeros(self.max_wg, self.scal_w, dtype=torch.float64, device=self.dev)
        n_ws = getattr(lib, "trl_ppo_%sreduce_adam_workspace" % sfx)(self.D, self.H, self.A)
        self.red_ws = torch.zeros(n_ws, device=self.dev)
        self.red_ws[4:8].view(torch.float64).fill_(1.0)
        self._joint = LastGraph()
        self._pending = None
        self._pro_ws = None

    def _n_wg(self, n_samples):
        tiles = (n_samples + 15) // 16
        return max(1, min(self.max_wg, (tiles + 3) // 4))

    def sync_target_pf(self, in_prologue=False):
        raise _C.TrlError("Reinforce has no target policy")

    def run(self, t, row_idx, N, pre=None, pre_key=None, defer=False):
        algo, dev = self.algo, self.dev
        if dist.collectives_active():
            raise _C.TrlError(_ONE_RANK)
        K, rows_mb = row_idx.shape
        n_local = rows_mb * N
        n_global = float(n_local)
        n_wg = self._n_wg(n_local)
        if self._pending is not None:
            self._pending.land()
            self._pending = None
        idx_dev, stats = self._buffers(K, rows_mb)
        self._idx_host.numpy()[:] = row_idx.reshape(-1)
        rows_total = t["advs"].shape[0]
        raw, info, norms = _stat_views(stats, K)
        lr_pf = float(algo.pf_optimizer.param_groups[0]['lr'])
        self._set_device_hyper(lr_pf, 0.0, upload=False)
        hyper = _hyper(algo)
        use_graph = os.environ.get("TRL_NO_GRAPH") != "1"
        key = (n_wg, n_global, rows_total, N, pre_key, pre is not None) + hyper + tuple(
            t[k].data_ptr() for k in ("obs", "acts", "advs"))

        def launch_all():
            g = self._batch_args(t, hyper, _C.LOSS_REINFORCE, rows_mb, N, n_global, self.partial, self.scal, n_wg, n_wg)
            g.vf_params = None
            a = self._adam_args((lr_pf,), device_state=1)
            slab = [(idx_dev, self._idx_host), (self.red_ws[2:4], self._hyper_host)]
            self._prologue(pre, t["advs"].reshape(rows_total, N), self._idx_host.view(K, rows_mb), raw, stats[4 * K:], slab)
            fold = self._fold(self._k_fold_net, self.partial, self.scal, n_wg, 0, info, self.red_ws)
            self._minibatches(K, g, a, idx_dev, raw, norms, fold)

        self._joint.run(key, launch_all, eager=not use_graph)
        self._stats_host.copy_(stats, non_blocking=True)
        landed = torch.cuda.Event()
        landed.record()
        self._stepped(K)
        build = lambda host: _infos_reinforce(self, *(v.numpy() for v in _stat_views(host, K)[:2]), n_global)
        pending = _PendingInfos(K, landed, self._stats_host, build)
        if defer:
            self._pending = pending
            return pending
        return pending.resolve()


class _GenericReinforce(_PolicyOnly, _GenericPPO):

    def __init__(self, algo):
        from ... import ops
        self.algo, self.ops = algo, ops
        pf = algo.pf
        self.head = head_kind(pf, refuse="Reinforce kernels need a GuassianContPolicyBasicBias, a GuassianContPolicy or a "
                                         "CategoricalDisPolicy")
        self.categorical, self.state_std = self.head == HEAD_CAT, self.head == HEAD_SD
        if self.state_std:
            head_w = int(ops.linear_layers(pf)[-1][0].shape[0])
            if not 1 <= head_w // 2 <= 32:
                raise _C.TrlError("a state-dependent-std policy emits [mean | log_std] with 1 <= A <= 32 action dimensions, "
                                  "got a head of %d" % head_w)
        self.dev = next(pf.parameters()).device
        if self.dev.type != "cuda":
            raise _C.TrlError("Reinforce networks live on %s: the HIP path needs a GPU (no CPU path exists)" % self.dev)
        self.pf_layers, self.act = ops.net_layers(pf)
        self.vf_layers = []
        tail = [] if (self.categorical or self.state_std) else [pf.logstd]
        self.D, self.A = int(self.pf_layers[0][0].shape[1]), int(self.pf_layers[-1][0].shape[0])
        if self.state_std:
            self.A //= 2
        self._home(ops.plan_params(self.pf_layers) + tail, [], None)
        views, off = [], 0
        for layer in self.pf_layers:
            view = []
            for p in ops.plan_params([layer]):
                view.append(self.grads[off:off + p.numel()].view(p.shape)); off += p.numel()
            views.append(tuple(view))
        self.gviews = [views]
        if tail:
            self.g_logstd = self.grads[off:off + self.A]
        self.step_state = torch.tensor([0.0, 1.0, 1.0, 0.0], dtype=torch.float64, device=self.dev)
        self.lr_dev = torch.zeros(1, device=self.dev)
        self._graphs, self._joint = GraphCache(4), None
        self.workspace = None

    def sync_target_pf(self, in_prologue=False):
        raise _C.TrlError("Reinforce has no target policy")

    def run(self, t, row_idx, N, pre=None, pre_key=None):
        algo, dev, ops = self.algo, self.dev, self.ops
        if dist.collectives_active():
            raise _C.TrlError(_ONE_RANK)
        K, rows_mb = row_idx.shape
        n_local = rows_mb * N
        n_global = float(n_local)
        idx_dev, stats = self._buffers(K, rows_mb)
        idx_dev.copy_(torch.from_numpy(np.ascontiguousarray(row_idx).reshape(-1)), non_blocking=True)
        rows_total = t["advs"].shape[0]
        raw, info, norms = _stat_views(stats, K)
        ws = self._ws(n_local)
        idx2d = idx_dev.view(K, rows_mb)
        lr = float(algo.pf_optimizer.param_groups[0]['lr'])
        if getattr(self, "_lr_host", None) != lr:
            self._lr_host = lr
            self.lr_dev.copy_(torch.tensor([lr], dtype=torch.float32), non_blocking=True)
        gather = lambda key, k: _C.gather_rows(t[key].reshape(rows_total, N, -1), idx2d[k]).reshape(n_local, -1)
        c_ent, tanh = float(algo.entropy_coeff), int(bool(algo.pf.tanh_action))
        mode = _C.LOSS_REINFORCE

        def launch_all():
            if pre is not None:
                pre()
            stats.zero_()
            _C.adv_stats(t["advs"].reshape(rows_total, N), idx2d, raw)
            for k in range(K):
                obs, acts, advs = gather("obs", k), gather("acts", k), gather("advs", k)
                mean, tape_pf = ops.mlp_forward(self.pf_layers, obs, self.act)
                if self.categorical:
                    d_mean, _ = _C.cat_losses(mean, acts.view(-1), advs.view(-1), None, None, None, None, raw[k], n_global,
                                              0.0, c_ent, 0, mode, info[k])
                elif self.state_std:
                    d_mean, _ = _C.gauss_sd_losses(mean, acts, advs.view(-1), None, None, None, None, raw[k], n_global,
                                                   0.0, c_ent, 0, tanh, mode, info[k])
                else:
                    d_mean, _ = _C.ppo_generic_losses(mean, algo.pf.logstd.detach(), acts, advs.view(-1), None, None, None,
                                                      None, raw[k], n_global, 0.0, c_ent, 0, tanh, mode, self.g_logstd,
                                                      info[k])
                ops.mlp_backward(tape_pf, d_mean, grads=self.gviews[0], workspace=ws)
                _C.clip_adam(self._adam_args(norms_out=norms[k].data_ptr(), step_state=self.step_state.data_ptr(),
                                             device_lr=self.lr_dev.data_ptr()), dev)

        key = (K, rows_mb, N, rows_total, n_global, idx_dev.data_ptr(), stats.data_ptr(), pre_key, pre is not None, c_ent,
               tanh) + tuple(t[k_].data_ptr() for k_ in ("obs", "acts", "advs"))
        self._graphs.run(key, launch_all)
        self._stepped(K)
        host = stats.cpu()
        return _infos_reinforce(self, *(v.numpy() for v in _stat_views(host, K)[:2]), n_global)
```

torchrl_amd/csrc/k_ppo.hip:

```cpp
#include <cstdlib>
#include "trl_common.h"
#include "trl_mlp.h"
#include "trl_head.h"
#include "trl_comm.h"

struct PpoDev {
  const float *obs, *acts, *advs, *rets, *old_values, *old_logp;
  const int64_t* row_idx;
  int rows_mb, N;
  const double* adv_raw;
  double n_global;
  const float *pf_params, *vf_params;
  float clip_para, entropy_coeff;
  int clipped_value_loss, tanh_action;
  int loss_mode;
  float* partial;
  double* scal_partial;
  int n_wg, n_pf, p_stride;
  int D, A;
};

template <int D, int H, int A> struct PpoShape {
  static_assert(H == 64 && D > 16 && D <= 32 && A <= 8, "instantiated for 16 < D <= 32, H == 64, A <= 8");
  static constexpr int P_PF = MlpFlat<D, H, A>::P_PF, P_VF = MlpFlat<D, H, 1>::P_VF;
  static constexpr int P_STRIDE = ((P_PF > P_VF ? P_PF : P_VF) + 63) & ~63;
};

#define WV_WAVES 4
#ifdef TRL_EXP_CLK
#define WCLK_DECL long long clk_prev = clock64(); float clk_acc[24]; for (int q_ = 0; q_ < 24; ++q_) clk_acc[q_] = 0.f;
#define WCLK(ph) { __builtin_amdgcn_sched_barrier(0); const long long c_ = clock64(); clk_acc[ph] += (float)(c_ - clk_prev); clk_prev = c_; __builtin_amdgcn_sched_barrier(0); }
#else
#define WCLK_DECL
#define WCLK(ph)
#endif
#define WV_THREADS (64 * WV_WAVES)
#define LDT 20
#define LDW 68

template <int D, int H, int A> struct WvShape {
  static_assert(H == 64 && (D == 17 || D == 32) && A <= 8, "instantiated for D == 17 / 32, H == 64, A <= 8");
  static constexpr int O_W2F = 0, O_W2B = H * LDW, O_B1 = 2 * H * LDW, O_B2 = O_B1 + H, O_SCR = O_B2 + H;
  static constexpr int O_H1 = 0, O_H2 = H * LDT, O_DZ2 = 2 * H * LDT, O_DO = 3 * H * LDT, WSCR = O_DO + 16 * LDT;
  static constexpr int P_STRIDE = PpoShape<D, H, A>::P_STRIDE;
  static constexpr int MAIN = O_SCR + WV_WAVES * WSCR;
  static constexpr int XS_W2 = 0, XS_W1 = 16, XS_W1B = 20, XS_W3 = D > 17 ? 24 : 20, XS_PF = XS_W3 + 4, XS_VF = XS_W3;
  static constexpr int XSC_PF = 3 * H + 32, XSC_VF = 4 * H + 16;
  static constexpr int XCH_PF = WV_WAVES * (XS_PF * 256 + XSC_PF), XCH_VF = WV_WAVES * (XS_VF * 256 + XSC_VF);
  static constexpr int XCH = XCH_PF > XCH_VF ? XCH_PF : XCH_VF;
  static constexpr int LDS_FLOATS = MAIN > XCH ? MAIN : XCH;
};

template <int D, int H, int A> struct WvShapeSD : WvShape<D, H, A> {
  static constexpr int P_PF_SD = H * D + H + H * H + H + 2 * A * H + 2 * A, P_VF = MlpFlat<D, H, 1>::P_VF;
  static constexpr int P_STRIDE = ((P_PF_SD > P_VF ? P_PF_SD : P_VF) + 63) & ~63;
};
template <int D, int H, int A, int HEAD> struct WvPick { using T = WvShape<D, H, A>; };
template <int D, int H, int A> struct WvPick<D, H, A, HEAD_SD> { using T = WvShapeSD<D, H, A>; };
#define SD_HALF_LOG_2PI_PLUS_HALF 1.4189385332046727f

__device__ __forceinline__ f32x4 lds4(const float* p) { return *reinterpret_cast<const f32x4*>(p); }
__device__ __forceinline__ float row_sum16(float v) {
  v += __builtin_bit_cast(float, __builtin_amdgcn_update_dpp(0, __builtin_bit_cast(int, v), 0x128, 0xF, 0xF, false));
  v += __builtin_bit_cast(float, __builtin_amdgcn_update_dpp(0, __builtin_bit_cast(int, v), 0x124, 0xF, 0xF, false));
  v += __builtin_bit_cast(float, __builtin_amdgcn_update_dpp(0, __builtin_bit_cast(int, v), 0x122, 0xF, 0xF, false));
  v += __builtin_bit_cast(float, __builtin_amdgcn_update_dpp(0, __builtin_bit_cast(int, v), 0x121, 0xF, 0xF, false));
  return v;
}

template <int D, int H, int A, int ACT, bool IS_PF, bool CONTIG, bool RT, int HEAD = HEAD_GAUSS>
__device__ void ppo_wave_pass(const PpoDev& a, float* lds, int wg_in_net, int n_wg_net) {
  using S = typename WvPick<D, H, A, HEAD>::T;
  constexpr bool WIDE = D > 17,
                 CAT = HEAD == HEAD_CAT, SD = HEAD == HEAD_SD,
                 SDP = SD && IS_PF;
  static_assert(!WIDE || RT, "the wide tile exists as a runtime-dims instantiation only");
  static_assert(!CAT || (IS_PF && RT), "the categorical head is a policy pass of the runtime-dims kernels");
  static_assert(!SD || RT, "the state-dependent-std head belongs to the runtime-dims kernels");
  constexpr int AS = CAT ? 1 : 0;
  const int Dr = RT ? a.D : D;
  const int O = IS_PF ? (RT ? a.A : A) : 1;
  const int OH = SDP ? 2 * O : O;
  const int F_W1 = 0, F_B1 = H * Dr, F_W2 = F_B1 + H, F_B2 = F_W2 + H * H, F_W3 = F_B2 + H, F_B3 = F_W3 + OH * H,
            F_LS = F_B3 + OH, F_END = (CAT || SDP) ? F_LS : F_LS + O;
  auto sd_has = [&](int o) -> bool { return (o & 7) < O; };
  auto sd_row = [&](int o) -> int { return o < 8 ? o : O + (o - 8); };
  const int PS = RT ? a.p_stride : S::P_STRIDE;
  const int tid = threadIdx.x, lane = tid & 63, wave = tid >> 6;
  const int j = lane & 15, g = lane >> 4, i = j;
  const float* gp = IS_PF ? a.pf_params : a.vf_params;
  WCLK_DECL
  float* W2F = lds + S::O_W2F;
  float* W2B = lds + S::O_W2B;
  float* scr = lds + S::O_SCR + wave * S::WSCR;
  float* H1S = scr + S::O_H1;
  float* H2S = scr + S::O_H2;
  float* DZ2S = scr + S::O_DZ2;
  float* DOS = scr + S::O_DO;

  const double adv_s1 = IS_PF ? a.adv_raw[0] : 0.0, adv_s2 = IS_PF ? a.adv_raw[1] : 0.0;
  const int B = a.rows_mb * a.N;
  const int n_tiles = (B + 15) / 16;
  const int tile_stride = n_wg_net * WV_WAVES;

  float xq[5], xtq[4], lq[6];
  float xq2[4], xtq2[4];
  int tile = wg_in_net * WV_WAVES + wave;
  const int tpr = a.N >> 4;
  int p1r = 0, p1c = 0, p2r = 0, p2c = 0, st_r = 0, st_c = 0;
  int64_t ridx1 = 0, ridx2 = 0;
  bool fv[4], fv2[4];
  const bool f16 = !WIDE && (!RT || Dr > 16), jv = !RT || i < Dr, jv2 = WIDE && 16 + i < Dr;
  const unsigned ox16 = (unsigned)(j * Dr + (f16 ? 16 : 0)) * 4u, os = (unsigned)j * 4u;
  unsigned oxq[4], oxt[4], oa_[4], oxq2[4], oxt2[4];
#pragma unroll
  for (int q = 0; q < 4; ++q) {
    fv[q] = !RT || 4 * g + q < Dr;
    fv2[q] = WIDE && 16 + 4 * g + q < Dr;
    oxq[q] = (unsigned)(j * Dr + (fv[q] ? 4 * g + q : 0)) * 4u;
    oxt[q] = (unsigned)((4 * g + q) * Dr + (jv ? i : 0)) * 4u;
    oxq2[q] = (unsigned)(j * Dr + (fv2[q] ? 16 + 4 * g + q : 0)) * 4u;
    oxt2[q] = (unsigned)((4 * g + q) * Dr + (jv2 ? 16 + i : 0)) * 4u;
    if constexpr (SDP) oa_[q] = (unsigned)(j * O + (4 * (g & 1) + q < O ? 4 * (g & 1) + q : 0)) * 4u;
    else oa_[q] = CAT ? (unsigned)j * 4u : (unsigned)(j * O + (4 * g + q < O ? 4 * g + q : 0)) * 4u;
  }
  auto ldb = [](const float* base, unsigned byte_off) -> float {
    return *reinterpret_cast<const float*>(reinterpret_cast<const char*>(base) + byte_off);
  };
  auto pos_advance = [&](int& r, int& c) { c += st_c; r += st_r; if (c >= tpr) { c -= tpr; ++r; } };
  auto load_ridx = [&](int r) -> int64_t {
    const int rr = r < a.rows_mb ? r : 0;
    return a.row_idx ? a.row_idx[rr] : (int64_t)rr;
  };
  auto fetch_contig = [&](int64_t ridx, int r, int c) {
    const int64_t cell0 = (r < a.rows_mb) ? ridx * a.N + 16 * c : 0;
    const float* ob = a.obs + cell0 * Dr;
#pragma unroll
    for (int q = 0; q < 4; ++q) xq[q] = ldb(ob, oxq[q]);
    xq[4] = ldb(ob, ox16);
#pragma unroll
    for (int q = 0; q < 4; ++q) xtq[q] = ldb(ob, oxt[q]);
    if constexpr (WIDE) {
#pragma unroll
      for (int q = 0; q < 4; ++q) { xq2[q] = ldb(ob, oxq2[q]); xtq2[q] = ldb(ob, oxt2[q]); }
    }
    if constexpr (IS_PF) {
      const float* ab = a.acts + cell0 * (CAT ? AS : O);
      if constexpr (CAT) { lq[0] = ldb(ab, oa_[0]); lq[1] = lq[2] = lq[3] = 0.0f; }
      else {
#pragma unroll
        for (int q = 0; q < 4; ++q) lq[q] = ldb(ab, oa_[q]);
      }
      lq[4] = ldb(a.advs + cell0, os);
      lq[5] = a.old_logp ? ldb(a.old_logp + cell0, os) : 0.0f;
    } else {
      lq[0] = lq[1] = lq[2] = lq[3] = 0.0f;
      lq[4] = ldb(a.rets + cell0, os);
      lq[5] = a.clipped_value_loss ? ldb(a.old_values + cell0, os) : 0.0f;
    }
  };
  auto row_of = [&](int smp, int& e) -> int { const int sm = smp < B ? smp : 0; const int r = sm / a.N; e = sm - r * a.N; return r; };
  auto fetch_inputs = [&](int64_t p, int s0) {
#pragma unroll
    for (int r = 0; r < 4; ++r) xq[r] = a.obs[p * Dr + (fv[r] ? 4 * g + r : 0)];
    xq[4] = a.obs[p * Dr + (f16 ? 16 : 0)];
#pragma unroll
    for (int q = 0; q < 4; ++q) {
      const int sj = 4 * g + q;
      const int64_t pr = __shfl(p, sj, 64);
      xtq[q] = a.obs[(s0 + sj < B ? pr : 0) * Dr + (jv ? i : 0)];
      if constexpr (WIDE) {
        xq2[q] = a.obs[p * Dr + (fv2[q] ? 16 + 4 * g + q : 0)];
        xtq2[q] = a.obs[(s0 + sj < B ? pr : 0) * Dr + (jv2 ? 16 + i : 0)];
      }
    }
    if constexpr (IS_PF) {
      if constexpr (CAT) { lq[0] = a.acts[p]; lq[1] = lq[2] = lq[3] = 0.0f; }
      else if constexpr (SDP) {
#pragma unroll
        for (int r = 0; r < 4; ++r) lq[r] = a.acts[p * O + (4 * (g & 1) + r < O ? 4 * (g & 1) + r : 0)];
      } else {
#pragma unroll
        for (int r = 0; r < 4; ++r) lq[r] = a.acts[p * O + (4 * g + r < O ? 4 * g + r : 0)];
      }
      lq[4] = a.advs[p]; lq[5] = a.old_logp ? a.old_logp[p] : 0.0f;
    } else {
      lq[0] = lq[1] = lq[2] = lq[3] = 0.0f;
      lq[4] = a.rets[p]; lq[5] = a.clipped_value_loss ? a.old_values[p] : 0.0f;
    }
  };
  int e_nn = 0;
  int64_t ridx_nn = 0;
  auto fetch_row = [&](int t) {
    const int r = row_of(t * 16 + j, e_nn);
    ridx_nn = a.row_idx ? a.row_idx[r] : (int64_t)r;
  };
  auto prefetch_next = [&](int nt) {
    if constexpr (CONTIG) {
      fetch_contig(ridx1, p1r, p1c);
      p1r = p2r; p1c = p2c; ridx1 = ridx2;
      pos_advance(p2r, p2c);
      ridx2 = load_ridx(p2r);
    } else {
      const int64_t pn = (nt * 16 + j < B) ? ridx_nn * a.N + e_nn : 0;
      fetch_inputs(pn, nt * 16);
      fetch_row(nt + tile_stride);
    }
  };
  if constexpr (CONTIG) {
    const int t0 = __builtin_amdgcn_readfirstlane(tile);
    const int ts = __builtin_amdgcn_readfirstlane(tile_stride);
    st_r = ts / tpr; st_c = ts - st_r * tpr;
    int r0 = t0 / tpr, c0 = t0 - (t0 / tpr) * tpr;
    fetch_contig(load_ridx(r0), r0, c0);
    p1r = r0; p1c = c0;
    pos_advance(p1r, p1c);
    ridx1 = load_ridx(p1r);
    p2r = p1r; p2c = p1c;
    pos_advance(p2r, p2c);
    ridx2 = load_ridx(p2r);
  } else {
    fetch_row(tile);
    const int64_t p0 = (tile * 16 + j < B) ? ridx_nn * a.N + e_nn : 0;
    fetch_inputs(p0, tile * 16);
    fetch_row(tile + tile_stride);
  }
  constexpr int NV = H * H / (4 * WV_THREADS);
  f32x4 wv[NV], wt[NV];
  const int tc = tid & 63, tq = tid >> 6;
  const float bias1 = tid < H ? gp[F_B1 + tid] : 0.0f, bias2 = tid < H ? gp[F_B2 + tid] : 0.0f;
  {
    static_assert(WV_THREADS == 256 && H == 64, "the transposed staging maps (column, 4 rows) onto 256 threads");
    const bool w2_al = !RT || ((reinterpret_cast<uintptr_t>(gp + F_W2) & 15) == 0);
#pragma unroll
    for (int t = 0; t < NV; ++t) {
      if (w2_al) wv[t] = *reinterpret_cast<const f32x4*>(gp + F_W2 + 4 * (tid + WV_THREADS * t));
      else {
#pragma unroll
        for (int x = 0; x < 4; ++x) wv[t][x] = gp[F_W2 + 4 * (tid + WV_THREADS * t) + x];
      }
    }
#pragma unroll
    for (int t = 0; t < NV; ++t)
#pragma unroll
      for (int x = 0; x < 4; ++x) wt[t][x] = gp[F_W2 + (4 * (tq + 4 * t) + x) * H + tc];
  }
  for (int e = lane; e < 16 * LDT; e += 64) DOS[e] = 0.0f;
  float w1[4][5], w3h[4][4], w3t[4][4];
  float w1b[4][4];
#pragma unroll
  for (int so = 0; so < 4; ++so) {
    const int row = 16 * so + i;
#pragma unroll
    for (int r = 0; r < 4; ++r) w1[so][r] = fv[r] ? gp[F_W1 + row * Dr + (fv[r] ? 4 * g + r : 0)] : 0.0f;
    w1[so][4] = (g == 0 && f16) ? gp[F_W1 + row * Dr + (f16 ? 16 : 0)] : 0.0f;
    if constexpr (WIDE) {
#pragma unroll
      for (int r = 0; r < 4; ++r) w1b[so][r] = fv2[r] ? gp[F_W1 + row * Dr + (fv2[r] ? 16 + 4 * g + r : 0)] : 0.0f;
    }
#pragma unroll
    for (int r = 0; r < 4; ++r) {
      if constexpr (SDP) {
        const int o = 4 * g + r;
        w3h[so][r] = sd_has(i) ? gp[F_W3 + (sd_has(i) ? sd_row(i) : 0) * H + 16 * so + 4 * g + r] : 0.0f;
        w3t[so][r] = sd_has(o) ? gp[F_W3 + (sd_has(o) ? sd_row(o) : 0) * H + row] : 0.0f;
      } else if constexpr (IS_PF) {
        w3h[so][r] = (i < O) ? gp[F_W3 + (i < O ? i : 0) * H + 16 * so + 4 * g + r] : 0.0f;
        const int o = 4 * g + r;
        w3t[so][r] = (o < O) ? gp[F_W3 + (o < O ? o : 0) * H + row] : 0.0f;
      } else {
        w3h[so][r] = gp[F_W3 + 16 * so + 4 * g + r];
        w3t[so][r] = 0.0f;
      }
    }
  }
  float lsv[4], ivv[4], b3v[4], lspass[4];
#pragma unroll
  for (int r = 0; r < 4; ++r) {
    const int o = 4 * g + r;
    const float raw = (IS_PF && !CAT && !SDP && o < O) ? gp[F_LS + (o < O ? o : 0)] : 0.0f;
    lsv[r] = fminf(fmaxf(raw, -20.0f), 2.0f);
    ivv[r] = __expf(-2.0f * lsv[r]);
    lspass[r] = (raw >= -20.0f && raw <= 2.0f) ? 1.0f : 0.0f;
    if constexpr (SDP) b3v[r] = sd_has(o) ? gp[F_B3 + (sd_has(o) ? sd_row(o) : 0)] : 0.0f;
    else b3v[r] = (o < O) ? gp[F_B3 + (o < O ? o : 0)] : 0.0f;
  }
  const float vb3 = IS_PF ? 0.0f : gp[F_B3];
#ifdef TRL_EXP_CLK
  WCLK(22)
  __builtin_amdgcn_s_waitcnt(0);
  WCLK(23)
#endif
#pragma unroll
  for (int t = 0; t < NV; ++t) {
    const int e = 4 * (tid + WV_THREADS * t), r = e / H, c = e - r * H;
    *reinterpret_cast<f32x4*>(W2F + r * LDW + c) = wv[t];
    *reinterpret_cast<f32x4*>(W2B + tc * LDW + 4 * (tq + 4 * t)) = wt[t];
  }
  if (tid < H) { lds[S::O_B1 + tid] = bias1; lds[S::O_B2 + tid] = bias2; }
  __syncthreads();

  const double ng = a.n_global;
  const double adv_mean = adv_s1 / ng;
  const double adv_var = (adv_s2 - adv_s1 * adv_s1 / ng) / (ng - 1.0);
  const float adv_mu = (float)adv_mean;
  const float adv_rstd = 1.0f / ((float)sqrt(fmax(adv_var, 0.0)) + 1e-5f);
  const float inv_b = (float)(1.0 / ng);

  f32x4 gW2[4][4], gW1[4], gW3[4];
  f32x4 gW1b[4];
  float gb1[4][4], gb2[4][4], gW1c[4][4];
  float db3[4], dls[4], stv[7];
  float ent_sum = 0.0f;
  float sdst[8] = {0.0f, 0.0f, -INFINITY, -INFINITY, 0.0f, 0.0f, -INFINITY, -INFINITY}, sd_cnt = 0.0f;
#pragma unroll
  for (int x = 0; x < 4; ++x) {
    gW1[x] = gW3[x] = gW1b[x] = f32x4{0.f, 0.f, 0.f, 0.f};
    db3[x] = dls[x] = 0.0f;
#pragma unroll
    for (int y = 0; y < 4; ++y) { gW2[x][y] = f32x4{0.f, 0.f, 0.f, 0.f}; gb1[x][y] = gb2[x][y] = gW1c[x][y] = 0.0f; }
  }
#pragma unroll
  for (int k = 0; k < 7; ++k) stv[k] = (k >= 2 && k <= 5) ? -INFINITY : 0.0f;

  WCLK(0)
  for (; tile < n_tiles; tile += tile_stride) {
    const int s = tile * 16 + j;
    const bool valid = CONTIG ? true : (s < B);
    float xb[5], xt[4], lin[6], xb2[4], xt2[4];
#pragma unroll
    for (int r = 0; r < 4; ++r) xb[r] = (valid && fv[r]) ? xq[r] : 0.0f;
    xb[4] = (valid && f16) ? xq[4] : 0.0f;
#pragma unroll
    for (int q = 0; q < 4; ++q) xt[q] = (jv && (CONTIG || tile * 16 + 4 * g + q < B)) ? xtq[q] : 0.0f;
    if constexpr (WIDE) {
#pragma unroll
      for (int q = 0; q < 4; ++q) {
        xb2[q] = (valid && fv2[q]) ? xq2[q] : 0.0f;
        xt2[q] = (jv2 && (CONTIG || tile * 16 + 4 * g + q < B)) ? xtq2[q] : 0.0f;
      }
    }
#pragma unroll
    for (int q = 0; q < 6; ++q) lin[q] = lq[q];
    const float x16 = xb[4];

#define PIN_DS() __builtin_amdgcn_sched_barrier(0x676)
    f32x4 h1[4], h2[4];
    f32x4 wq[4], bq;
#pragma unroll
    for (int so = 0; so < 4; ++so) h1[so] = lds4(lds + S::O_B1 + 16 * so + 4 * g);
#pragma unroll
    for (int sl = 0; sl < 4; ++sl) wq[sl] = lds4(W2F + i * LDW + 16 * sl + 4 * g);
    bq = lds4(lds + S::O_B2 + 4 * g);
    PIN_DS();
    WCLK(9)
#pragma unroll
    for (int q = 0; q < (WIDE ? 4 : 5); ++q)
#pragma unroll
      for (int so = 0; so < 4; ++so) h1[so] = mfma16(w1[so][q], xb[q], h1[so]);
    if constexpr (WIDE) {
#pragma unroll
      for (int q = 0; q < 4; ++q)
#pragma unroll
        for (int so = 0; so < 4; ++so) h1[so] = mfma16(w1b[so][q], xb2[q], h1[so]);
    }
    WCLK(10)
#pragma unroll
    for (int so = 0; so < 4; ++so)
#pragma unroll
      for (int r = 0; r < 4; ++r) {
        h1[so][r] = act_fn<ACT>(h1[so][r]);
        H1S[(16 * so + 4 * g + r) * LDT + j] = h1[so][r];
      }
    WCLK(1)
#pragma unroll
    for (int so = 0; so < 4; ++so) {
      f32x4 acc = bq;
      f32x4 wc[4];
#pragma unroll
      for (int sl = 0; sl < 4; ++sl) wc[sl] = wq[sl];
      if (so < 3) {
#pragma unroll
        for (int sl = 0; sl < 4; ++sl) wq[sl] = lds4(W2F + (16 * (so + 1) + i) * LDW + 16 * sl + 4 * g);
        bq = lds4(lds + S::O_B2 + 16 * (so + 1) + 4 * g);
        PIN_DS();
      }
#pragma unroll
      for (int sl = 0; sl < 4; ++sl)
#pragma unroll
        for (int r = 0; r < 4; ++r) acc = mfma16(wc[sl][r], h1[sl][r], acc);
      WCLK(11)
#pragma unroll
      for (int r = 0; r < 4; ++r) h2[so][r] = act_fn<ACT>(acc[r]);
      WCLK(12)
    }

    prefetch_next(tile + tile_stride);
    WCLK(2)
    f32x4 dz2[4];
    f32x4 wb[4];
    if constexpr (IS_PF) {
#pragma unroll
      for (int so = 0; so < 4; ++so)
#pragma unroll
        for (int r = 0; r < 4; ++r) H2S[(16 * so + 4 * g + r) * LDT + j] = h2[so][r];
      f32x4 oa = f32x4{b3v[0], b3v[1], b3v[2], b3v[3]}, ob = f32x4{0.f, 0.f, 0.f, 0.f};
#pragma unroll
      for (int sl = 0; sl < 4; sl += 2)
#pragma unroll
        for (int r = 0; r < 4; ++r) { oa = mfma16(w3h[sl][r], h2[sl][r], oa); ob = mfma16(w3h[sl + 1][r], h2[sl + 1][r], ob); }
      WCLK(14)
      float zc[4], lp = 0.0f;
      float pk[4], lpk[4], ent = 0.0f;
      int ai = 0;
      if constexpr (CAT) {
        float lg[4], ek[4], m = -INFINITY;
#pragma unroll
        for (int r = 0; r < 4; ++r) {
          lg[r] = oa[r] + ob[r];
          m = (4 * g + r < O) ? fmaxf(m, lg[r]) : m;
        }
        m = fmaxf(m, __shfl_xor(m, 16, 64));
        m = g < 2 ? m : 0.0f;
#pragma unroll
        for (int r = 0; r < 4; ++r) ek[r] = (4 * g + r < O) ? expf(lg[r] - m) : 0.0f;
        const float c_own = ((ek[0] + ek[1]) + ek[2]) + ek[3];
        const float c_lo = __shfl_xor(c_own, 16, 64);
        float Ssum = g == 1 ? (((c_lo + ek[0]) + ek[1]) + ek[2]) + ek[3] : c_own;
        const float S_hi = __shfl_xor(Ssum, 16, 64);
        Ssum = g == 0 ? S_hi : (g == 1 ? Ssum : 1.0f);
        const float logS = logf(Ssum);
        ai = min(max((int)lin[0], 0), O - 1);
#pragma unroll
        for (int r = 0; r < 4; ++r) {
          const bool has = 4 * g + r < O;
          lpk[r] = has ? (lg[r] - m) - logS : 0.0f;
          pk[r] = ek[r] / Ssum;
          lp += (has && 4 * g + r == ai) ? lpk[r] : 0.0f;
// ... 396 lines not shown
    }
  }
  return fold_chain_tree(acc);
}
__device__ __forceinline__ float fold_waves_tree(const float (*s_acc)[RED_CHUNK], int lane) {
  float t4[RED_WAVES / 4];
#pragma unroll
  for (int q = 0; q < RED_WAVES / 4; ++q)
    t4[q] = (s_acc[4 * q][lane] + s_acc[4 * q + 1][lane]) + (s_acc[4 * q + 2][lane] + s_acc[4 * q + 3][lane]);
  float gval = t4[0];
#pragma unroll
  for (int q = 1; q < RED_WAVES / 4; ++q) gval += t4[q];
  return gval;
}
__device__ __noinline__ void fold_scalar_stats(const double* __restrict__ base, int nrow, int net, int lane,
                                                  double* __restrict__ info) {
  double v[7];
#pragma unroll
  for (int k = 0; k < 7; ++k) v[k] = (k >= 2 && k <= 5) ? -INFINITY : 0.0;
  for (int w0 = 0; w0 < nrow; w0 += 192) {
    double o[3][7];
#pragma unroll
    for (int q = 0; q < 3; ++q) {
      const int w = w0 + lane + 64 * q;
#pragma unroll
      for (int k = 0; k < 7; ++k) {
        double x = (k >= 2 && k <= 5) ? -INFINITY : 0.0;
        if (w < nrow) x = base[(size_t)w * 8 + k];
        o[q][k] = x;
      }
    }
#pragma unroll
    for (int q = 0; q < 3; ++q)
#pragma unroll
      for (int k = 0; k < 7; ++k) v[k] = (k >= 2 && k <= 5) ? fmax(v[k], o[q][k]) : v[k] + o[q][k];
  }
#pragma unroll
  for (int k = 0; k < 7; ++k) v[k] = (k >= 2 && k <= 5) ? wave_max(v[k]) : wave_sum(v[k]);
  if (lane == 0) {
    if (net == 0) {
      info[0] = v[6]; info[1] = v[0]; info[2] = v[1]; info[3] = v[2]; info[4] = v[3]; info[5] = v[4]; info[6] = v[5];
    } else {
      info[7] = v[6];
      info[12] = v[0]; info[13] = v[1]; info[14] = v[2]; info[15] = v[3];
    }
  }
}
__device__ __noinline__ void fold_logstd_stats_raw(float raw, int n_act, int lane, double* __restrict__ info) {
  const bool has = lane < n_act;
  const double x = has ? fmin(fmax((double)raw, -20.0), 2.0) : 0.0;
  const double e = has ? exp(x) : 0.0;
  const double sm = wave_sum(x), sq = wave_sum(x * x), es = wave_sum(e), eq = wave_sum(e * e);
  const double mx = wave_max(has ? x : -INFINITY), mn = -wave_max(has ? -x : -INFINITY);
  const double emx = wave_max(has ? e : -INFINITY), emn = -wave_max(has ? -e : -INFINITY);
  if (lane == 0) {
    const double mean = sm / n_act, em = es / n_act;
    info[8] = mean;
    info[9] = n_act > 1 ? sqrt(fmax((sq - sm * mean) / (n_act - 1), 0.0)) : NAN;
    info[10] = mx; info[11] = mn;
    info[16] = em;
    info[17] = n_act > 1 ? sqrt(fmax((eq - es * em) / (n_act - 1), 0.0)) : NAN;
    info[18] = emx; info[19] = emn;
  }
}
__device__ __forceinline__ void fold_logstd_stats(const float* __restrict__ logstd, int n_act, int lane, double* __restrict__ info) {
  fold_logstd_stats_raw(logstd[lane < n_act ? lane : 0], n_act, lane, info);
}

__device__ __noinline__ void fold_entropy_stats(const double* __restrict__ base, int nrow, int lane, double* __restrict__ info) {
  double v = 0.0;
  for (int w = lane; w < nrow; w += 64) v += base[(size_t)w * 8 + 7];
  v = wave_sum(v);
  if (lane == 0) {
    info[20] = v;
#pragma unroll
    for (int k = 0; k < 4; ++k) info[8 + k] = info[16 + k] = 0.0;
  }
}

__device__ __noinline__ void fold_sd_stats(const double* __restrict__ base, const double* __restrict__ sd, int nrow, int n_act,
                                           int lane, double* __restrict__ info) {
  double v[10];
#pragma unroll
  for (int k = 0; k < 10; ++k) v[k] = (k < 8 && (k & 2)) ? -INFINITY : 0.0;
  for (int w = lane; w < nrow; w += 64) {
#pragma unroll
    for (int k = 0; k < 9; ++k) {
      const double o = sd[(size_t)w * SD_SCAL + k];
      v[k] = (k < 8 && (k & 2)) ? fmax(v[k], o) : v[k] + o;
    }
    v[9] += base[(size_t)w * 8 + 7];
  }
#pragma unroll
  for (int k = 0; k < 10; ++k) v[k] = (k < 8 && (k & 2)) ? wave_max(v[k]) : wave_sum(v[k]);
  if (lane == 0) {
    const double n = v[8] * (double)n_act, lm = v[0] / n, em = v[4] / n;
    info[8] = lm; info[9] = n > 1.0 ? sqrt(fmax((v[1] - v[0] * lm) / (n - 1.0), 0.0)) : NAN;
    info[10] = v[2]; info[11] = -v[3];
    info[16] = em; info[17] = n > 1.0 ? sqrt(fmax((v[5] - v[4] * em) / (n - 1.0), 0.0)) : NAN;
    info[18] = v[6]; info[19] = -v[7];
    info[20] = v[9];
  }
}

template <int HEAD = HEAD_GAUSS>
__device__ __forceinline__ float ppo_reduce_block(const float* __restrict__ partial,
                                                  const double* __restrict__ scal, int n_wg, int n_pf,
                                                  int p_stride, int p_pf, int p_vf,
                                                  const float* __restrict__ logstd, int n_act,
                                                  float* __restrict__ grads, double* __restrict__ info,
                                                  int net, int bx, bool stats) {
  __shared__ float s_acc[RED_WAVES][RED_CHUNK];
  const int row0 = net == 0 ? 0 : n_pf, nrow = net == 0 ? n_pf : n_wg - n_pf;
  const int lane = threadIdx.x & 63, wave = threadIdx.x >> 6;
  const int p = bx * RED_CHUNK + lane;
  const int pn = net == 0 ? p_pf : p_vf;
  s_acc[wave][lane] = fold_rows_wave(partial + (size_t)row0 * p_stride + p, nrow, p_stride, wave, p < pn);
  __syncthreads();
  float gval = 0.0f;
  if (wave == 0 && p < pn) {
    gval = fold_waves_tree(s_acc, lane);
    grads[(net == 0 ? 0 : p_pf) + p] = gval;
  }
  if (stats && wave == 2) fold_scalar_stats(scal + (size_t)row0 * 8, nrow, net, lane, info);
  if constexpr (HEAD == HEAD_SD) {
    if (stats && net == 0 && wave == 3)
      fold_sd_stats(scal + (size_t)row0 * 8, scal + (size_t)n_wg * 8 + (size_t)row0 * SD_SCAL, nrow, n_act, lane, info);
  } else if constexpr (HEAD == HEAD_CAT) {
    if (stats && net == 0 && wave == 3) fold_entropy_stats(scal + (size_t)row0 * 8, nrow, lane, info);
  } else {
    if (stats && net == 0 && wave == 3 && logstd) fold_logstd_stats(logstd, n_act, lane, info);
  }
  return gval;
}

template <int HEAD = HEAD_GAUSS>
__global__ __launch_bounds__(64 * RED_WAVES) void ppo_reduce_kernel(const float* __restrict__ partial,
                                                         const double* __restrict__ scal, int n_wg, int n_pf,
                                                         int p_stride, int p_pf, int p_vf,
                                                         const float* __restrict__ logstd, int n_act,
                                                         float* __restrict__ grads, double* __restrict__ info) {
  ppo_reduce_block<HEAD>(partial, scal, n_wg, n_pf, p_stride, p_pf, p_vf, logstd, n_act, grads, info, blockIdx.y, blockIdx.x,
                        blockIdx.x == gridDim.x - 1);
}

struct AdamDev {
  float* params; const float* grads; float* m; float* v;
  int n_groups; int off[5]; float lr[4];
  float max_norm, beta1, beta2, eps, grad_scale, bc1, bc2_sqrt;
  float* norms_out;
  double* step_state;
  const float* device_lr;
  int self_tick;
};
__global__ __launch_bounds__(256) void clip_adam_kernel(AdamDev a) {
  __shared__ float s_part[4][4];
  __shared__ float s_coef[4];
  __shared__ float s_bc[2];
  const int tid = threadIdx.x, lane = tid & 63, wave = tid >> 6;
  if (a.step_state && tid == 0) {
    s_bc[0] = (float)(1.0 - a.step_state[1] * (double)a.beta1);
    s_bc[1] = (float)sqrt(1.0 - a.step_state[2] * (double)a.beta2);
    if (a.self_tick) {
      unsigned* cnt = reinterpret_cast<unsigned*>(a.step_state + 3);
      const unsigned before = __hip_atomic_fetch_add(cnt, 1u, __ATOMIC_ACQ_REL, __HIP_MEMORY_SCOPE_AGENT);
      if (before == gridDim.x - 1) {
        a.step_state[0] += 1.0; a.step_state[1] *= (double)a.beta1; a.step_state[2] *= (double)a.beta2;
        __hip_atomic_store(cnt, 0u, __ATOMIC_RELAXED, __HIP_MEMORY_SCOPE_AGENT);
      }
    }
  }
  const bool need_norm = a.max_norm > 0.0f;
  for (int g = 0; g < a.n_groups; ++g) {
    if (!need_norm) { if (lane == 0) s_part[g][wave] = 0.0f; continue; }
    float s0 = 0.f, s1 = 0.f, s2 = 0.f, s3 = 0.f;
    int e = a.off[g] + tid;
    for (; e + 7 * 256 < a.off[g + 1]; e += 8 * 256) {
      float x[8];
#pragma unroll
      for (int k = 0; k < 8; ++k) x[k] = a.grads[e + 256 * k];
      s0 = fmaf(x[0], x[0], s0); s1 = fmaf(x[1], x[1], s1); s2 = fmaf(x[2], x[2], s2); s3 = fmaf(x[3], x[3], s3);
      s0 = fmaf(x[4], x[4], s0); s1 = fmaf(x[5], x[5], s1); s2 = fmaf(x[6], x[6], s2); s3 = fmaf(x[7], x[7], s3);
    }
    for (; e < a.off[g + 1]; e += 256) { const float x = a.grads[e]; s0 = fmaf(x, x, s0); }
    float ss = wave_sum((s0 + s1) + (s2 + s3)) * a.grad_scale * a.grad_scale;
    if (lane == 0) s_part[g][wave] = ss;
  }
  __syncthreads();
  if (tid < a.n_groups) {
    const float norm = sqrtf(s_part[tid][0] + s_part[tid][1] + s_part[tid][2] + s_part[tid][3]);
    s_coef[tid] = (a.max_norm > 0.0f) ? fminf(a.max_norm / (norm + 1e-6f), 1.0f) : 1.0f;
    if (blockIdx.x == 0 && a.norms_out) a.norms_out[tid] = norm;
  }
  __syncthreads();
  const float bc1 = a.step_state ? s_bc[0] : a.bc1, bc2_sqrt = a.step_state ? s_bc[1] : a.bc2_sqrt;
  const int e = blockIdx.x * 256 + tid;
  if (e < a.off[a.n_groups]) {
    int g = 0;
    while (e >= a.off[g + 1]) ++g;
    const float gr = a.grads[e] * a.grad_scale * s_coef[g];
    const float m = a.beta1 * a.m[e] + (1.0f - a.beta1) * gr;
    const float v = a.beta2 * a.v[e] + (1.0f - a.beta2) * gr * gr;
    a.m[e] = m; a.v[e] = v;
    const float denom = sqrtf(v) / bc2_sqrt + a.eps;
    const float lr = a.device_lr ? a.device_lr[g] : a.lr[g];
    a.params[e] -= (lr / bc1) * (m / denom);
  }
}

__global__ void adam_tick_kernel(double* __restrict__ st, float beta1, float beta2) {
  st[0] += 1.0; st[1] *= (double)beta1; st[2] *= (double)beta2;
}

__device__ __forceinline__ void adam_element(const AdamDev& a, int e, float gr) {
  const float m = a.beta1 * a.m[e] + (1.0f - a.beta1) * gr;
  const float v = a.beta2 * a.v[e] + (1.0f - a.beta2) * gr * gr;
  a.m[e] = m; a.v[e] = v;
  const float denom = sqrtf(v) / a.bc2_sqrt + a.eps;
  int g = 0;
  while (e >= a.off[g + 1]) ++g;
  a.params[e] -= (a.lr[g] / a.bc1) * (m / denom);
}

template <bool LOOP, int HEAD = HEAD_GAUSS>
__global__ __launch_bounds__(64 * RED_WAVES, 4) void ppo_reduce_adam_kernel(const float* __restrict__ partial,
                                                              const double* __restrict__ scal, int n_wg, int n_pf,
                                                              int p_stride, int p_pf, int p_vf,
                                                              const float* __restrict__ logstd, int n_act,
                                                              float* __restrict__ grads, double* __restrict__ info,
                                                              AdamDev a, float* __restrict__ ws, unsigned epoch,
                                                              int device_state, int xrank, XrArgs xr, int only_net) {
  __shared__ float s_coef[2];
  __shared__ float s_hyper[4];
  const int tid = threadIdx.x, lane = tid & 63, wave = tid >> 6;
  const int nb = (p_stride + RED_CHUNK - 1) / RED_CHUNK, grid = gridDim.x, job0 = only_net == 1 ? nb : 0;
  const int n_jobs = only_net >= 0 ? job0 + nb : 2 * nb, blk = job0 + (int)blockIdx.x;
  double* bpow = reinterpret_cast<double*>(ws + 4);
  double b1p = 0.0, b2p = 0.0;
  float lr0 = 0.0f, lr1 = 0.0f;
  if (device_state) {
    epoch = reinterpret_cast<const unsigned*>(ws)[1] + 1u;
    if (tid == 64 * (RED_WAVES - 1)) { b1p = bpow[0]; b2p = bpow[1]; lr0 = ws[2]; lr1 = ws[3]; }
  }
  unsigned long long* slots = reinterpret_cast<unsigned long long*>(ws + 16);
  unsigned xepoch = 0u;
  if (xrank) {
    const unsigned e4 = __hip_atomic_load(xr.ctl + 4, __ATOMIC_RELAXED, __HIP_MEMORY_SCOPE_AGENT);
    const unsigned e6 = __hip_atomic_load(xr.ctl + 6, __ATOMIC_RELAXED, __HIP_MEMORY_SCOPE_AGENT);
    xepoch = (only_net == 0 ? e4 : only_net == 1 ? e6 : (e4 > e6 ? e4 : e6)) + 1u;
  }
  float gval0 = 0.0f;
  for (int j = blk; j < (LOOP ? n_jobs : blk + 1); j += LOOP ? grid : 1) {
    const int net = j / nb, bx = j - net * nb;
    if (j != blk) __syncthreads();
    float gval = ppo_reduce_block<HEAD>(partial, scal, n_wg, n_pf, p_stride, p_pf, p_vf, logstd, n_act, grads, info, net, bx, bx == nb - 1);
    if (wave == 0) {
      if (xrank) {
        const int pe = bx * RED_CHUNK + lane;
        const bool act = pe < (net == 0 ? p_pf : p_vf);
        const int ge = (net == 0 ? 0 : p_pf) + pe;
        gval = xr_allsum_f32(xr, xepoch, act ? ge : 0, gval, act);
        if (act) grads[ge] = gval;
      }
      if (j == blk) gval0 = gval;
      const float ss = wave_sum(gval * gval);
      if (lane == 0)
        __hip_atomic_store(slots + net * nb + bx, ((unsigned long long)epoch << 32) | (unsigned long long)__float_as_uint(ss),
                           __ATOMIC_RELAXED, __HIP_MEMORY_SCOPE_AGENT);
    }
  }
  if (device_state && tid == 64 * (RED_WAVES - 1)) {
    b1p *= (double)a.beta1; b2p *= (double)a.beta2;
    s_hyper[0] = (float)(1.0 - b1p);
    s_hyper[1] = (float)sqrt(1.0 - b2p);
    s_hyper[2] = lr0; s_hyper[3] = lr1;
  }
  if (LOOP && blk >= n_jobs) return;
  const int net_ = blk / nb, pe_ = (blk - net_ * nb) * RED_CHUNK + lane;
  const bool own_ = wave == 0 && pe_ < (net_ == 0 ? p_pf : p_vf);
  const int ge_ = (net_ == 0 ? 0 : p_pf) + pe_;
  float m_old = 0.0f, v_old = 0.0f, p_old = 0.0f;
  if (own_) { m_old = a.m[ge_]; v_old = a.v[ge_]; p_old = a.params[ge_]; }
  if (wave < 2 && (only_net < 0 || wave == only_net)) {
    float acc = 0.0f;
    for (int b = lane; b < nb; b += 64) {
      unsigned long long v;
      unsigned it = 0;
      unsigned long long t0 = 0;
      while ((unsigned)((v = __hip_atomic_load(slots + wave * nb + b, __ATOMIC_RELAXED, __HIP_MEMORY_SCOPE_AGENT)) >> 32) != epoch) {
        __builtin_amdgcn_s_sleep(1);
        if ((++it & 1023u) == 0) {
          const unsigned long long now = wall_clock64();
          if (t0 == 0) t0 = now;
          if (now - t0 > (xrank ? xr.wait_ticks + xr.wait_ticks / 4 : 200000000ull)) {
            __hip_atomic_store(reinterpret_cast<unsigned*>(ws), 1u, __ATOMIC_RELAXED, __HIP_MEMORY_SCOPE_AGENT);
            break;
          }
        }
      }
      acc += __uint_as_float((unsigned)v);
    }
    acc = wave_sum(acc) * a.grad_scale * a.grad_scale;
    if (lane == 0) {
      const float norm = sqrtf(acc);
      s_coef[wave] = (a.max_norm > 0.0f) ? fminf(a.max_norm / (norm + 1e-6f), 1.0f) : 1.0f;
      if (a.norms_out && blk == job0) a.norms_out[wave] = norm;
    }
  }
  __syncthreads();
  float bc1 = a.bc1, bc2_sqrt = a.bc2_sqrt, lr_pf = a.lr[0], lr_vf = a.lr[1];
  if (device_state) {
    bc1 = s_hyper[0]; bc2_sqrt = s_hyper[1]; lr_pf = s_hyper[2]; lr_vf = s_hyper[3];
    if (blk == job0) {
      if (tid == 0) __hip_atomic_store(reinterpret_cast<unsigned*>(ws) + 1, epoch, __ATOMIC_RELAXED, __HIP_MEMORY_SCOPE_AGENT);
      if (tid == 64 * (RED_WAVES - 1)) { bpow[0] = b1p; bpow[1] = b2p; }
    }
  }
  if (xrank && blk == job0 && tid == 0) {
    if (only_net != 1) __hip_atomic_store(xr.ctl + 4, xepoch, __ATOMIC_RELAXED, __HIP_MEMORY_SCOPE_AGENT);
    if (only_net != 0) __hip_atomic_store(xr.ctl + 6, xepoch, __ATOMIC_RELAXED, __HIP_MEMORY_SCOPE_AGENT);
  }
  const bool xfail = xrank && __hip_atomic_load(xr.ctl + 2, __ATOMIC_RELAXED, __HIP_MEMORY_SCOPE_AGENT) != 0u;
  if (wave == 0 && !xfail) {
    for (int j = blk; j < (LOOP ? n_jobs : blk + 1); j += LOOP ? grid : 1) {
      const int net = j / nb, pe = (j - net * nb) * RED_CHUNK + lane;
      if (pe >= (net == 0 ? p_pf : p_vf)) continue;
      const int ge = (net == 0 ? 0 : p_pf) + pe;
      const bool first = j == blk;
      const float g_ = first ? gval0 : grads[ge];
      const float mo = first ? m_old : a.m[ge], vo = first ? v_old : a.v[ge], po = first ? p_old : a.params[ge];
      const float gr = g_ * a.grad_scale * s_coef[net];
      const float m = a.beta1 * mo + (1.0f - a.beta1) * gr;
      const float v = a.beta2 * vo + (1.0f - a.beta2) * gr * gr;
      a.m[ge] = m; a.v[ge] = v;
      const float denom = sqrtf(v) / bc2_sqrt + a.eps;
      a.params[ge] = po - ((net == 0 ? lr_pf : lr_vf) / bc1) * (m / denom);
    }
  }
}

template <int D, int H, int A, int ACT, bool CONTIG, bool RT, int HEAD = HEAD_GAUSS>
__global__ __launch_bounds__(WV_THREADS, 1) void ppo_grad_wave_kernel(PpoDev a) {
  static_assert(HEAD == HEAD_GAUSS || RT, "categorical / state-dependent-std head: runtime-dims tiles");
  constexpr int HEAD_VF = HEAD == HEAD_CAT ? HEAD_GAUSS : HEAD;
  extern __shared__ __attribute__((aligned(16))) float lds[];
#ifdef TRL_CHAIN_CLK
  const unsigned long long clk0 = wall_clock64();
#endif
  if ((int)blockIdx.x < a.n_pf) ppo_wave_pass<D, H, A, ACT, true, CONTIG, RT, HEAD>(a, lds, blockIdx.x, a.n_pf);
  else                          ppo_wave_pass<D, H, A, ACT, false, CONTIG, RT, HEAD_VF>(a, lds, blockIdx.x - a.n_pf, a.n_wg - a.n_pf);
#ifdef TRL_CHAIN_CLK
  __syncthreads();
  if (threadIdx.x == 0) {
    a.scal_partial[(size_t)blockIdx.x * 8 + 7] = (double)wall_clock64();
    float* pad = a.partial + (size_t)blockIdx.x * a.p_stride + a.p_stride - 3;
    pad[0] = (float)(clk0 >> 40); pad[1] = (float)((clk0 >> 20) & 0xFFFFFull); pad[2] = (float)(clk0 & 0xFFFFFull);
  }
#endif
}

template <int D, int H, int O, int ACT>
__global__ __launch_bounds__(256) void mlp2_forward_kernel(const float* __restrict__ params,
                                                           const float* __restrict__ x,
                                                           float* __restrict__ out, int M) {
  using L = MlpLds<D, H, O>;
  constexpr int NT = H / 32, KS = ksteps_for(D);
  __shared__ __attribute__((aligned(16))) float sp[L::SIZE];
  const int tid = threadIdx.x, lane = tid & 63, wave = tid >> 6, i = lane & 31, hi = lane >> 5;
  L::load(sp, params, false, tid, 256);
  __syncthreads();
  const int n_tiles = (M + 31) / 32;
  for (int tile = blockIdx.x * 4 + wave; tile < n_tiles; tile += gridDim.x * 4) {
    const int s = tile * 32 + i;
    float xb[KS];
#pragma unroll
    for (int q = 0; q < KS; ++q) { const int k = rowmap(q, hi); xb[q] = (k < D && s < M) ? x[(size_t)s * D + k] : 0.0f; }
    f32x16 h1[NT], h2[NT];
#pragma unroll
    for (int mo = 0; mo < NT; ++mo)
      h1[mo] = act_tile<ACT>(layer1_tile<D, L::LD1, KS>(bias_tile(sp + L::B1 + 32 * mo, hi), sp + L::W1, mo, xb, i, hi));
#pragma unroll
    for (int mo = 0; mo < NT; ++mo)
      h2[mo] = act_tile<ACT>(layer_tile<NT, L::LD2>(bias_tile(sp + L::B2 + 32 * mo, hi), sp + L::W2, mo, h1, i, hi));
    float o[O];
    head_fwd<NT, H, O>(sp + L::W3, sp + L::B3, h2, hi, o);
    if (hi == 0 && s < M) {
#pragma unroll
      for (int c = 0; c < O; ++c) out[(size_t)s * O + c] = o[c];
    }
  }
}

#define SHAPE_IS(d, h, o) (D == (d) && H == (h) && A == (o))

static int ppo_stride_for(int D, int H, int A, int head) {
  if (head == HEAD_GAUSS && SHAPE_IS(17, 64, 6)) return PpoShape<17, 64, 6>::P_STRIDE;
  if (head_shape_ok(head, D, H, A)) {
    const int p_pf = ppo_p_pf(D, H, A, head), p_vf = ppo_p_vf(D, H);
    return ((p_pf > p_vf ? p_pf : p_vf) + 63) & ~63;
  }
  trl_set_error("trl_ppo_%spartial_stride: shape D=%d H=%d A=%d not instantiated (H == 64, 2 <= D <= 32, %d <= A <= %d)",
                HEADS[head].tag, D, H, A, HEADS[head].a_min, HEADS[head].a_max);
  return TRL_EUNSUPPORTED;
}
extern "C" int trl_ppo_partial_stride(int D, int H, int A) { return ppo_stride_for(D, H, A, HEAD_GAUSS); }
extern "C" int trl_ppo_cat_partial_stride(int D, int H, int A) { return ppo_stride_for(D, H, A, HEAD_CAT); }
extern "C" int trl_ppo_sd_partial_stride(int D, int H, int A) { return ppo_stride_for(D, H, A, HEAD_SD); }
extern "C" int trl_ppo_cat_supported(int D, int H, int A, int act) { return head_supported(HEAD_CAT, D, H, A, act); }
extern "C" int trl_ppo_sd_supported(int D, int H, int A, int act) { return head_supported(HEAD_SD, D, H, A, act); }
extern "C" int trl_ppo_sd_scalar_stride(void) { return HEADS[HEAD_SD].scal_stride; }
static_assert(WvShapeSD<17, 64, 8>::P_STRIDE == 6400 && WvShapeSD<32, 64, 8>::P_STRIDE == 7360, "SD image strides at A = 8");
static_assert(WvShapeSD<32, 64, 8>::LDS_FLOATS * sizeof(float) <= 160 * 1024, "the wide tile's exchange area fits the LDS");

template <int D, int H, int A, int ACT, bool CONTIG, bool RT, int HEAD>
static int launch_ppo_v(const PpoDev& d, hipStream_t s) {
  using S = typename WvPick<D, H, A, HEAD>::T;
  const size_t lds = S::LDS_FLOATS * sizeof(float);
  static bool attr_set = false;
  if (!attr_set) {
    hipError_t e = hipFuncSetAttribute((const void*)ppo_grad_wave_kernel<D, H, A, ACT, CONTIG, RT, HEAD>,
                                       hipFuncAttributeMaxDynamicSharedMemorySize, (int)lds);
    if (e != hipSuccess) { trl_set_error("ppo_grad: hipFuncSetAttribute: %s", hipGetErrorString(e)); return (int)e; }
    attr_set = true;
  }
  hipLaunchKernelGGL((ppo_grad_wave_kernel<D, H, A, ACT, CONTIG, RT, HEAD>), dim3(d.n_wg), dim3(WV_THREADS), lds, s, d);
  TRL_LAUNCH_CHECK();
  return TRL_OK;
}
template <int D, int H, int A, int ACT, bool RT, int HEAD = HEAD_GAUSS>
static int launch_ppo(const PpoDev& d, hipStream_t s) {
  return (d.N % 16 == 0) ? launch_ppo_v<D, H, A, ACT, true, RT, HEAD>(d, s) : launch_ppo_v<D, H, A, ACT, false, RT, HEAD>(d, s);
}

extern "C" int trl_ppo_wg_split(int D, int H, int A, int n_tiles, int n_wg) {
  if (n_wg < 2 || n_tiles <= 0) { trl_set_error("trl_ppo_wg_split: need n_wg >= 2 and n_tiles > 0"); return TRL_EINVAL; }
  const double c_pf = 16.7, c_vf = 12.1;
  int best = n_wg / 2;
  double best_t = 1e300;
  for (int x = 1; x < n_wg; ++x) {
    const double t_pf = (double)((n_tiles + WV_WAVES * x - 1) / (WV_WAVES * x)) * c_pf;
    const double t_vf = (double)((n_tiles + WV_WAVES * (n_wg - x) - 1) / (WV_WAVES * (n_wg - x))) * c_vf;
    const double t = t_pf > t_vf ? t_pf : t_vf;
    if (t < best_t - 1e-9 || (t < best_t + 1e-9 && abs(2 * x - n_wg) < abs(2 * best - n_wg))) { best_t = t; best = x; }
  }
  (void)D; (void)H; (void)A;
  return best;
}
static int resolve_pf_wgs(int n_wg, int n_wg_pf) { return n_wg_pf < 0 ? 0 : (n_wg_pf > 0 ? n_wg_pf : n_wg / 2); }

static int ppo_grad_launch(const trl_ppo_batch_t* p, void* stream, int head = HEAD_GAUSS) {
  if (!p) { trl_set_error("ppo_grad: null descriptor"); return TRL_EINVAL; }
  if (!head_supported(head, p->D, p->H, p->A, p->act)) {
    trl_set_error("ppo_%sgrad: shape D=%d H=%d A=%d act=%d not instantiated (H == 64, 2 <= D <= 32, %d <= A <= %d, Tanh / ReLU)",
                  HEADS[head].tag, p->D, p->H, p->A, p->act, HEADS[head].a_min, HEADS[head].a_max);
    return TRL_EUNSUPPORTED;
  }
  const bool reinforce = p->loss_mode == TRL_LOSS_REINFORCE;
  TRL_REQUIRE(p->obs && p->acts && p->advs && (p->rets || reinforce), "null rollout tensor");
  TRL_REQUIRE(p->loss_mode == TRL_LOSS_PPO_CLIP || p->loss_mode == TRL_LOSS_A2C || reinforce, "unknown loss_mode");
  TRL_REQUIRE(!reinforce || p->n_wg_pf == p->n_wg, "TRL_LOSS_REINFORCE runs in an all-policy launch only (n_wg_pf == n_wg)");
  TRL_REQUIRE(!reinforce || !p->clipped_value_loss, "TRL_LOSS_REINFORCE has no value loss: clipped_value_loss must be 0");
  TRL_REQUIRE(p->loss_mode != TRL_LOSS_PPO_CLIP || p->old_logp, "the clipped surrogate needs old_logp");
  TRL_REQUIRE(!p->clipped_value_loss || p->old_values, "the clipped value loss needs old_values");
  TRL_REQUIRE(p->adv_raw && (p->pf_params || p->vf_params) && p->partial && p->scal_partial, "null pointer");
  TRL_REQUIRE(p->rows_mb > 0 && p->N > 0, "empty minibatch");
  TRL_REQUIRE(p->n_wg >= 1 && (p->n_wg >= 2 || p->n_wg_pf == -1 || p->n_wg_pf == p->n_wg), "n_wg must be >= 2 (>= 1 for one network)");
  TRL_REQUIRE(p->n_wg_pf >= -1 && p->n_wg_pf <= p->n_wg, "n_wg_pf must be 0 (even split), in [1, n_wg], or -1 (value net only)");
  TRL_REQUIRE(p->n_wg_pf == p->n_wg || p->vf_params, "null value parameters");
  TRL_REQUIRE(p->n_wg_pf == -1 || p->pf_params, "null policy parameters");
  TRL_REQUIRE(p->n_global > 1.0, "n_global must exceed 1 (unbiased std)");
  const int D = p->D, H = p->H, A = p->A;
  TRL_REQUIRE(((uintptr_t)p->partial & 15) == 0 && (((uintptr_t)p->pf_params | (uintptr_t)p->vf_params) & 3) == 0,
              "partial rows must be 16-byte aligned, parameter blocks 4-byte aligned");
  TRL_REQUIRE(head != HEAD_GAUSS || !SHAPE_IS(17, 64, 6) || (((uintptr_t)p->pf_params | (uintptr_t)p->vf_params) & 15) == 0,
              "parameter blocks of the benchmark shape must be 16-byte aligned");
  PpoDev d;
  d.obs = p->obs; d.acts = p->acts; d.advs = p->advs; d.rets = p->rets; d.old_values = p->old_values;
  d.old_logp = p->old_logp; d.row_idx = p->row_idx; d.rows_mb = p->rows_mb; d.N = p->N;
  d.adv_raw = p->adv_raw; d.n_global = p->n_global; d.pf_params = p->pf_params; d.vf_params = p->vf_params;
  d.clip_para = p->clip_para; d.entropy_coeff = p->entropy_coeff;
  d.clipped_value_loss = p->clipped_value_loss; d.tanh_action = p->tanh_action;
  d.loss_mode = reinforce ? TRL_LOSS_A2C : p->loss_mode;
  d.partial = p->partial; d.scal_partial = p->scal_partial; d.n_wg = p->n_wg;
  d.n_pf = resolve_pf_wgs(p->n_wg, p->n_wg_pf);
  d.D = D; d.A = A;
  hipStream_t s = (hipStream_t)stream;
  d.p_stride = ppo_stride_for(D, H, A, head);
  if (head == HEAD_CAT) d.tanh_action = 0;
  if (head == HEAD_GAUSS && SHAPE_IS(17, 64, 6))
    return p->act == TRL_ACT_TANH ? launch_ppo<17, 64, 6, TRL_ACT_TANH, false>(d, s) : launch_ppo<17, 64, 6, TRL_ACT_RELU, false>(d, s);
  return with_head(head, [&](auto hd) {
    return with_tile_act(D, p->act, [&](auto tile, auto act) {
      return launch_ppo<decltype(tile)::value, 64, 8, decltype(act)::value, true, decltype(hd)::value>(d, s);
    });
  });
}

extern "C" int trl_ppo_minibatch_grad_f32(const trl_ppo_batch_t* p, void* stream) { return ppo_grad_launch(p, stream); }
extern "C" int trl_ppo_cat_minibatch_grad_f32(const trl_ppo_batch_t* p, void* stream) { return ppo_grad_launch(p, stream, HEAD_CAT); }
extern "C" int trl_ppo_sd_minibatch_grad_f32(const trl_ppo_batch_t* p, void* stream) { return ppo_grad_launch(p, stream, HEAD_SD); }

static int launch_reduce(const float* partial, const double* scal_partial, int n_wg, int n_wg_pf, int D, int H, int A,
                         const float* pf_params, float* grads, double* info, void* stream, int head) {
  TRL_REQUIRE(partial && scal_partial && grads && info, "null pointer");
  TRL_REQUIRE(n_wg >= 2 && n_wg_pf >= 0 && n_wg_pf < n_wg, "need n_wg >= 2 and n_wg_pf in [0, n_wg)");
  const int ps = ppo_stride_for(D, H, A, head);
  if (ps < 0) return ps;
  const int p_pf = ppo_p_pf(D, H, A, head), p_vf = ppo_p_vf(D, H);
  const float* logstd = (HEADS[head].logstd_tail && pf_params) ? pf_params + (p_pf - A) : nullptr;
  with_head(head, [&](auto hd) {
    hipLaunchKernelGGL(ppo_reduce_kernel<decltype(hd)::value>, dim3(trl_ceil_div(ps, RED_CHUNK), 2), dim3(64 * RED_WAVES), 0,
                       (hipStream_t)stream, partial, scal_partial, n_wg, resolve_pf_wgs(n_wg, n_wg_pf), ps, p_pf, p_vf,
                       logstd, A, grads, info);
    return 0;
  });
  TRL_LAUNCH_CHECK();
  return TRL_OK;
}
extern "C" int trl_ppo_reduce_f32(const float* partial, const double* scal_partial, int n_wg, int n_wg_pf, int D,
                                  int H, int A, const float* pf_params, float* grads, double* info, void* stream) {
  return launch_reduce(partial, scal_partial, n_wg, n_wg_pf, D, H, A, pf_params, grads, info, stream, HEAD_GAUSS);
}
extern "C" int trl_ppo_cat_reduce_f32(const float* partial, const double* scal_partial, int n_wg, int n_wg_pf, int D,
                                      int H, int A, const float* pf_params, float* grads, double* info, void* stream) {
  return launch_reduce(partial, scal_partial, n_wg, n_wg_pf, D, H, A, pf_params, grads, info, stream, HEAD_CAT);
}
extern "C" int trl_ppo_sd_reduce_f32(const float* partial, const double* scal_partial, int n_wg, int n_wg_pf, int D,
                                     int H, int A, const float* pf_params, float* grads, double* info, void* stream) {
  return launch_reduce(partial, scal_partial, n_wg, n_wg_pf, D, H, A, pf_params, grads, info, stream, HEAD_SD);
}

static int fill_adam(const trl_adam_t* p, AdamDev& d) {
  if (!p) { trl_set_error("clip_adam: null descriptor"); return TRL_EINVAL; }
  TRL_REQUIRE(p->params && p->grads && p->exp_avg && p->exp_avg_sq, "null pointer");
  TRL_REQUIRE(p->n_groups >= 1 && p->n_groups <= 4, "n_groups must be 1..4");
  TRL_REQUIRE(p->step_count >= 1 || p->device_state || p->step_state, "step_count starts at 1");
  d.params = p->params; d.grads = p->grads; d.m = p->exp_avg; d.v = p->exp_avg_sq;
  d.n_groups = p->n_groups; d.off[0] = 0;
  for (int g = 0; g < p->n_groups; ++g) {
    TRL_REQUIRE(p->group_sizes[g] >= 0, "negative group size");
    d.off[g + 1] = d.off[g] + p->group_sizes[g];
    d.lr[g] = p->group_lr[g];
  }
  for (int g = p->n_groups; g < 4; ++g) { d.off[g + 1] = d.off[g]; if (g < 4) d.lr[g] = 0.f; }
  d.max_norm = p->max_norm; d.beta1 = p->beta1; d.beta2 = p->beta2; d.eps = p->eps;
  d.grad_scale = p->grad_scale;
  d.bc1 = (float)(1.0 - pow((double)p->beta1, (double)p->step_count));
  d.bc2_sqrt = (float)sqrt(1.0 - pow((double)p->beta2, (double)p->step_count));
  d.norms_out = p->norms_out;
  d.step_state = p->step_state;
  d.device_lr = p->device_lr;
  d.self_tick = 0;
  return TRL_OK;
}

static int reduce_adam_workspace(int D, int H, int A, int head) {
  const int ps = ppo_stride_for(D, H, A, head);
  if (ps < 0) return ps;
  return 16 + 4 * trl_ceil_div(ps, RED_CHUNK);
}
extern "C" int trl_ppo_reduce_adam_workspace(int D, int H, int A) { return reduce_adam_workspace(D, H, A, HEAD_GAUSS); }
extern "C" int trl_ppo_cat_reduce_adam_workspace(int D, int H, int A) { return reduce_adam_workspace(D, H, A, HEAD_CAT); }
extern "C" int trl_ppo_sd_reduce_adam_workspace(int D, int H, int A) { return reduce_adam_workspace(D, H, A, HEAD_SD); }

static int launch_reduce_adam(const float* partial, const double* scal_partial, int n_wg, int n_wg_pf, int D, int H, int A,
                              float* grads, double* info, const trl_adam_t* adam, float* workspace, const XrArgs* xr,
                              int max_blocks, void* stream, int only_net = -1, int head = HEAD_GAUSS) {
  TRL_REQUIRE(partial && scal_partial && grads && info && workspace, "null pointer");
  TRL_REQUIRE(only_net >= 0 ? n_wg >= 1 : (n_wg >= 2 && n_wg_pf >= 0 && n_wg_pf < n_wg), "need n_wg >= 2 and n_wg_pf in [0, n_wg)");
  const int ps = ppo_stride_for(D, H, A, head);
  if (ps < 0) return ps;
  AdamDev d;
  int rc = fill_adam(adam, d);
  if (rc) return rc;
  const int p_pf = ppo_p_pf(D, H, A, head), p_vf = ppo_p_vf(D, H);
  TRL_REQUIRE((adam->n_groups == 2 && adam->group_sizes[0] == p_pf && adam->group_sizes[1] == p_vf) ||
              (only_net == 0 && !xr && adam->n_groups == 1 && adam->group_sizes[0] == p_pf),
              "optimiser groups must be [policy | value] of this shape");
  TRL_REQUIRE(adam->grads == grads, "adam->grads must be the reduce output");
  TRL_REQUIRE(!xr || p_pf + p_vf <= TRL_XR_CAP_GRAD, "gradient exceeds the peer buffer");
  XrArgs none;
  none.rank = 0; none.world = 1; none.ctl = nullptr; none.wait_ticks = 0;
  for (int r = 0; r < TRL_MAX_RANKS; ++r) none.peer[r] = nullptr;
  int grid = (only_net >= 0 ? 1 : 2) * trl_ceil_div(ps, RED_CHUNK);
  if (max_blocks > 0 && max_blocks < grid) grid = max_blocks;
  const int n_pf = only_net == 0 ? n_wg : (only_net == 1 ? 0 : resolve_pf_wgs(n_wg, n_wg_pf));
  const int jobs = (only_net >= 0 ? 1 : 2) * trl_ceil_div(ps, RED_CHUNK);
  const float* logstd = HEADS[head].logstd_tail ? adam->params + (p_pf - A) : nullptr;
  const unsigned epoch = (unsigned)adam->step_count;
  with_head(head, [&](auto hd) {
    auto launch = [&](auto loop) {
      hipLaunchKernelGGL((ppo_reduce_adam_kernel<decltype(loop)::value, decltype(hd)::value>), dim3(grid), dim3(64 * RED_WAVES), 0,
                         (hipStream_t)stream, partial, scal_partial, n_wg, n_pf, ps, p_pf, p_vf, logstd, A, grads, info, d,
                         workspace, epoch, adam->device_state, xr ? 1 : 0, xr ? *xr : none, only_net);
    };
    if (grid == jobs) launch(std::false_type{}); else launch(std::true_type{});
    return 0;
  });
  TRL_LAUNCH_CHECK();
  return TRL_OK;
}

extern "C" int trl_ppo_reduce_adam_f32(const float* partial, const double* scal_partial, int n_wg, int n_wg_pf,
                                       int D, int H, int A, float* grads, double* info, const trl_adam_t* adam,
                                       float* workspace, void* stream) {
  return launch_reduce_adam(partial, scal_partial, n_wg, n_wg_pf, D, H, A, grads, info, adam, workspace, nullptr, 0, stream);
}

extern "C" int trl_ppo_reduce_adam_net_f32(const float* partial, const double* scal_partial, int n_wg, int net,
                                           int D, int H, int A, float* grads, double* info, const trl_adam_t* adam,
                                           float* workspace, void* stream) {
  TRL_REQUIRE(net == 0 || net == 1, "net: 0 = policy, 1 = value function");
  return launch_reduce_adam(partial, scal_partial, n_wg, 0, D, H, A, grads, info, adam, workspace, nullptr, 0, stream, net);
}

extern "C" int trl_ppo_cat_reduce_adam_f32(const float* partial, const double* scal_partial, int n_wg, int n_wg_pf,
                                           int D, int H, int A, float* grads, double* info, const trl_adam_t* adam,
                                           float* workspace, void* stream) {
  return launch_reduce_adam(partial, scal_partial, n_wg, n_wg_pf, D, H, A, grads, info, adam, workspace, nullptr, 0, stream, -1, HEAD_CAT);
}
extern "C" int trl_ppo_cat_reduce_adam_net_f32(const float* partial, const double* scal_partial, int n_wg, int net,
                                               int D, int H, int A, float* grads, double* info, const trl_adam_t* adam,
                                               float* workspace, void* stream) {
  TRL_REQUIRE(net == 0 || net == 1, "net: 0 = policy, 1 = value function");
  return launch_reduce_adam(partial, scal_partial, n_wg, 0, D, H, A, grads, info, adam, workspace, nullptr, 0, stream, net, HEAD_CAT);
}

extern "C" int trl_ppo_sd_reduce_adam_f32(const float* partial, const double* scal_partial, int n_wg, int n_wg_pf,
                                          int D, int H, int A, float* grads, double* info, const trl_adam_t* adam,
                                          float* workspace, void* stream) {
  return launch_reduce_adam(partial, scal_partial, n_wg, n_wg_pf, D, H, A, grads, info, adam, workspace, nullptr, 0, stream, -1, HEAD_SD);
}
extern "C" int trl_ppo_sd_reduce_adam_net_f32(const float* partial, const double* scal_partial, int n_wg, int net,
                                              int D, int H, int A, float* grads, double* info, const trl_adam_t* adam,
                                              float* workspace, void* stream) {
  TRL_REQUIRE(net == 0 || net == 1, "net: 0 = policy, 1 = value function");
  return launch_reduce_adam(partial, scal_partial, n_wg, 0, D, H, A, grads, info, adam, workspace, nullptr, 0, stream, net, HEAD_SD);
}

extern "C" int trl_ppo_reduce_adam_xrank_f32(const float* partial, const double* scal_partial, int n_wg, int n_wg_pf,
                                             int D, int H, int A, float* grads, double* info, const trl_adam_t* adam,
                                             float* workspace, trl_comm_t* comm, void* stream) {
  const XrArgs* xr = trl_comm_xr(comm);
  if (!xr) { trl_set_error("trl_ppo_reduce_adam_xrank_f32: communicator without mapped peers"); return TRL_EINVAL; }
  return launch_reduce_adam(partial, scal_partial, n_wg, n_wg_pf, D, H, A, grads, info, adam, workspace, xr,
                            trl_comm_wait_blocks(comm), stream);
}

extern "C" int trl_ppo_reduce_adam_xrank_net_f32(const float* partial, const double* scal_partial, int n_wg, int net,
                                                 int D, int H, int A, float* grads, double* info, const trl_adam_t* adam,
                                                 float* workspace, trl_comm_t* comm, void* stream) {
  TRL_REQUIRE(net == 0 || net == 1, "net: 0 = policy, 1 = value function");
  const XrArgs* xr = trl_comm_xr(comm);
  if (!xr) { trl_set_error("trl_ppo_reduce_adam_xrank_net_f32: communicator without mapped peers"); return TRL_EINVAL; }
  const int wb = trl_comm_wait_blocks(comm);
  return launch_reduce_adam(partial, scal_partial, n_wg, 0, D, H, A, grads, info, adam, workspace, xr,
                            wb > 0 ? (wb + 1) / 2 : 0, stream, net);
}

#define TICK_PENDING 0x70000001
static int clip_adam_launch(const trl_adam_t* p, void* stream, bool tick_here);
extern "C" int trl_clip_adam_f32(const trl_adam_t* p, void* stream) { return clip_adam_launch(p, stream, true); }

struct FileRing { const uint32_t* raw; uint32_t* ring; const double* count; int words, slots, ticked; };
__global__ __launch_bounds__(256) void polyak_tick_kernel(float* __restrict__ tgt, const float* __restrict__ src, int64_t n,
                                                          float tau, double* __restrict__ st, float beta1, float beta2,
                                                          FileRing file) {
  if (file.ring && blockIdx.x == 0) {
    const int64_t u = (int64_t)file.count[0] - file.ticked;
    __syncthreads();
    uint32_t* row = file.ring + (int64_t)(((u % file.slots) + file.slots) % file.slots) * file.words;
    for (int w = threadIdx.x; w < file.words; w += 256) row[w] = file.raw[w];
  }
  if (st && blockIdx.x == 0 && threadIdx.x == 0) { st[0] += 1.0; st[1] *= (double)beta1; st[2] *= (double)beta2; }
  for (int64_t e = (int64_t)blockIdx.x * 256 + threadIdx.x; e < n; e += (int64_t)gridDim.x * 256)
    tgt[e] = tgt[e] * (1.0f - tau) + src[e] * tau;
}
static int clip_adam_polyak(const trl_adam_t* p, float* target, const float* source, int64_t n, float tau,
                            const void* raw, int raw_bytes, void* ring, int slots, void* stream) {
  TRL_REQUIRE(n > 0 && target && source, "polyak: empty / null");
  int rc = clip_adam_launch(p, stream, false);
  if (rc != TRL_OK && rc != TICK_PENDING) return rc;
  int grid = trl_ceil_div(n, 256);
  if (grid > 1024) grid = 1024;
  FileRing file = {(const uint32_t*)raw, (uint32_t*)ring, p->step_state, raw_bytes / 4, slots, rc == TICK_PENDING ? 0 : 1};
  hipLaunchKernelGGL(polyak_tick_kernel, dim3(grid), dim3(256), 0, (hipStream_t)stream, target, source, n, tau,
                     rc == TICK_PENDING ? p->step_state : (double*)nullptr, p->beta1, p->beta2, file);
  TRL_LAUNCH_CHECK();
  return TRL_OK;
}
extern "C" int trl_clip_adam_polyak_f32(const trl_adam_t* p, float* target, const float* source, int64_t n, float tau,
                                        const void* raw, int raw_bytes, void* ring, int slots, void* stream) {
  if (!ring) return clip_adam_polyak(p, target, source, n, tau, nullptr, 0, nullptr, 0, stream);
  TRL_REQUIRE(raw && raw_bytes > 0 && raw_bytes % 4 == 0 && slots > 0, "clip_adam_polyak: bad ring");
  TRL_REQUIRE(p && p->step_state, "clip_adam_polyak: the ring row is picked by the device-resident step state");
  return clip_adam_polyak(p, target, source, n, tau, raw, raw_bytes, ring, slots, stream);
}

#define FAP_THREADS 1024
#define FAP_MAX_WG 256
#define FAP_MAX_ENTRIES 32
struct FapDev {
  int count;
  int off[FAP_MAX_ENTRIES + 1];
  int splits[FAP_MAX_ENTRIES];
  const float* part[FAP_MAX_ENTRIES];
  float* target; int target_off, target_n; float tau;
  unsigned long long* slots;
  unsigned* err;
  float* grads_out;
};
__global__ __launch_bounds__(FAP_THREADS) void fold_adam_polyak_kernel(AdamDev a, FapDev f, FileRing file) {
  __shared__ float s_ss[4][FAP_THREADS / 64];
  __shared__ float s_coef[4];
  __shared__ float s_bc[2];
  __shared__ int s_fail;
  __shared__ int s_off[FAP_MAX_ENTRIES + 1], s_splits[FAP_MAX_ENTRIES];
  __shared__ const float* s_part[FAP_MAX_ENTRIES];
  const int tid = threadIdx.x, lane = tid & 63, wave = tid >> 6, nb = gridDim.x;
  if (tid <= f.count) s_off[tid] = f.off[tid];
  if (tid < f.count) { s_splits[tid] = f.splits[tid]; s_part[tid] = f.part[tid]; }
  const int total = a.off[a.n_groups];
  const int per = (total + nb - 1) / nb, lo = blockIdx.x * per, hi = min(total, lo + per);
  const double steps = a.step_state[0];
  const unsigned epoch = (unsigned)(long long)steps + 1u;
  if (tid == 0) {
    s_bc[0] = (float)(1.0 - a.step_state[1] * (double)a.beta1);
// ... 170 lines not shown
```

Measured before the change: 100.9 million.

## Keep a lane-swizzled operand image of PPO weights refreshed by the Adam kernel

Adds a per-network 'operand image' buffer that holds the policy and value weights already permuted into the per-lane f32x4 layout the minibatch gradient kernel wants. The fused reduce+Adam kernel writes each updated parameter into its image position(s) through a precomputed map, and a build kernel fills the image from the flat params in the epoch prologue. The gradient kernel then loads W1, W2-transpose, W3 and the head scalars with coalesced vector loads instead of strided scalar gathers. The cost is extra scattered stores in Adam, one build launch per epoch, and a small FP-contract change in the Adam math.

```diff
diff --git a/include/trl_hip.h b/include/trl_hip.h
--- a/include/trl_hip.h
+++ b/include/trl_hip.h
@@ -122,8 +122,12 @@
   double* scal_partial;
   int n_wg;
   int n_wg_pf;
+  const float* pf_image; const float* vf_image;
 } trl_ppo_batch_t;
 int trl_ppo_partial_stride(int D, int H, int A);
+int trl_ppo_image_size(int D, int H, int A);
+int trl_ppo_image_map(int D, int H, int A, int32_t* map, int32_t* inverse);
+int trl_ppo_image_build_f32(const float* flat, const int32_t* inverse, float* image, void* stream);
 int trl_ppo_wg_split(int D, int H, int A, int n_tiles, int n_wg);
 int trl_ppo_minibatch_grad_f32(const trl_ppo_batch_t* args, void* stream);
 int trl_ppo_reduce_f32(const float* partial, const double* scal_partial, int n_wg, int n_wg_pf,
@@ -179,6 +183,8 @@
   int device_state;
   double* step_state;
   const float* device_lr;
+  float* image;
+  const int32_t* image_map;
 } trl_adam_t;
 int trl_clip_adam_f32(const trl_adam_t* args, void* stream);
 int trl_clip_adam_polyak_f32(const trl_adam_t* args, float* target, const float* source, int64_t n, float tau,
diff --git a/torchrl_amd/_C.py b/torchrl_amd/_C.py
--- a/torchrl_amd/_C.py
+++ b/torchrl_amd/_C.py
@@ -80,6 +80,7 @@
         ("clip_para", C.c_float), ("entropy_coeff", C.c_float),
         ("clipped_value_loss", C.c_int), ("tanh_action", C.c_int), ("loss_mode", C.c_int),
         ("partial", C.c_void_p), ("scal_partial", C.c_void_p), ("n_wg", C.c_int), ("n_wg_pf", C.c_int),
+        ("pf_image", C.c_void_p), ("vf_image", C.c_void_p),
     ]
 
 
@@ -90,6 +91,7 @@
         ("max_norm", C.c_float), ("beta1", C.c_float), ("beta2", C.c_float), ("eps", C.c_float),
         ("step_count", C.c_int), ("grad_scale", C.c_float), ("norms_out", C.c_void_p),
         ("device_state", C.c_int), ("step_state", C.c_void_p), ("device_lr", C.c_void_p),
+        ("image", C.c_void_p), ("image_map", C.c_void_p),
     ]
 
 
@@ -138,6 +140,9 @@
     "trl_mlp2_forward_supported": (C.c_int, [C.c_int, C.c_int, C.c_int]),
     "trl_ppo_minibatch_grad_f32": (C.c_int, [C.POINTER(PpoBatchArgs), C.c_void_p]),
     "trl_ppo_wg_split": (C.c_int, [C.c_int, C.c_int, C.c_int, C.c_int, C.c_int]),
+    "trl_ppo_image_size": (C.c_int, [C.c_int, C.c_int, C.c_int]),
+    "trl_ppo_image_map": (C.c_int, [C.c_int, C.c_int, C.c_int, C.c_void_p, C.c_void_p]),
+    "trl_ppo_image_build_f32": (C.c_int, [C.c_void_p, C.c_void_p, C.c_void_p, C.c_void_p]),
     "trl_rollout_norm_workspace": (C.c_int, [C.c_int]),
     "trl_rollout_norm_max_envs": (C.c_int, [C.c_int, C.c_int, C.c_int, C.c_int]),
     "trl_frame_stream_append_u8": (C.c_int, [C.c_void_p, C.c_void_p, C.c_void_p, C.c_void_p, C.c_int, C.c_int, C.c_int, C.c_int, C.c_int, C.c_void_p]),
@@ -585,6 +590,24 @@
     return _partial_stride("trl_ppo_partial_stride", D, H, A)
 
 
+def ppo_image_floats(D, H, A):
+    return int(lib().trl_ppo_image_size(int(D), int(H), int(A))) // 4
+
+
+def ppo_image_map(D, H, A):
+    n = ppo_image_floats(D, H, A)
+    P = (64 * D + 64 + 64 * 64 + 64) * 2 + (64 * A + A + A) + (64 + 1)
+    fwd, inv = torch.empty(P, 2, dtype=torch.int32), torch.empty(2 * n, dtype=torch.int32)
+    check(lib().trl_ppo_image_map(int(D), int(H), int(A), fwd.data_ptr(), inv.data_ptr()), "trl_ppo_image_map")
+    return fwd, inv
+
+
+def ppo_image_build(flat, inverse, image):
+    dev_ptr(flat, name="flat"), dev_ptr(inverse, torch.int32, name="inverse"), dev_ptr(image, name="image")
+    check(lib().trl_ppo_image_build_f32(flat.data_ptr(), inverse.data_ptr(), image.data_ptr(), stream_ptr(flat.device)),
+          "trl_ppo_image_build_f32")
+
+
 def ppo_cat_partial_stride(D, H, A):
     return _partial_stride("trl_ppo_cat_partial_stride", D, H, A)
 
diff --git a/torchrl_amd/algo/on_policy/ppo.py b/torchrl_amd/algo/on_policy/ppo.py
--- a/torchrl_amd/algo/on_policy/ppo.py
+++ b/torchrl_amd/algo/on_policy/ppo.py
@@ -162,6 +162,26 @@
         self._pending, self._chain_pend, self._chain_seen = None, [], set()
         self._stats2_key = self._chain_rows = self._pro_ws = None
         self.red_ws[4:8].view(torch.float64).fill_(1.0)
+        self._make_images()
+
+    def _make_images(self):
+        self.image = self._img_map = self._img_inv = None
+        if self.head != HEAD_GAUSS or os.environ.get("TRL_PPO_OPERAND_IMAGE", "1") == "0":
+            return
+        n = _C.ppo_image_floats(self.D, self.H, self.A)
+        if n == 0:
+            return
+        fwd, inv = _C.ppo_image_map(self.D, self.H, self.A)
+        if self.P_vf == 0:
+            inv[n:] = -1
+        self.image = torch.zeros(2 * n, device=self.dev)
+        self._img_map = fwd[:self.P_pf + self.P_vf].contiguous().to(self.dev)
+        self._img_inv = inv.to(self.dev)
+
+    def _keep_image(self, a):
+        if self.image is not None:
+            a.image, a.image_map = self.image.data_ptr(), self._img_map.data_ptr()
+        return a
 
     def _home(self, pf_list, vf_list, target_list):
         self.P_pf = sum(p.numel() for p in pf_list)
@@ -238,7 +258,7 @@
     def _adam_args(self, lrs=(0.0, 0.0), **kw):
         return _C.adam_args(self.flat, self.grads, self.m, self.v, (self.P_pf, self.P_vf), lrs, max_norm=0.5, eps=1e-5, **kw)
 
-    def _batch_args(self, t, hyper, loss_mode, rows_mb, N, n_global, partial, scal, n_wg, n_wg_pf):
+    def _batch_args(self, t, hyper, loss_mode, rows_mb, N, n_global, partial, scal, n_wg, n_wg_pf, image=False):
         g = _C.PpoBatchArgs()
         for k in ("obs", "acts", "advs", "rets", "old_values", "old_logp"):
             setattr(g, k, _C.dev_ptr(t[k], name=k).value if t.get(k) is not None else None)
@@ -248,9 +268,12 @@
         g.D, g.H, g.A, g.act = self.D, self.H, self.A, self.act
         g.clip_para, g.entropy_coeff, g.clipped_value_loss, g.tanh_action = hyper
         g.partial, g.scal_partial, g.n_wg, g.n_wg_pf = partial.data_ptr(), scal.data_ptr(), n_wg, n_wg_pf
+        if image and self.image is not None:
+            g.pf_image = self.image.data_ptr()
+            g.vf_image = self.image.data_ptr() + 2 * self.image.numel() if self.P_vf else None
         return g
 
-    def _prologue(self, pre, advs, idx, raw, zero, copies):
+    def _prologue(self, pre, advs, idx, raw, zero, copies, image=False):
         self._copy_in_prologue = False
         if pre is not None:
             pre()
@@ -259,6 +282,8 @@
         if self._copy_in_prologue:
             copies = [(self.target_flat, self.flat[:self.P_pf])] + copies
         _C.ppo_epoch_prologue(advs, idx, raw, self._pro_ws, zero=zero, copies=copies)
+        if image and self.image is not None:
+            _C.ppo_image_build(self.flat, self._img_inv, self.image)
         dist.reduce_adv_raw_(raw)
 
     def _fold(self, kernel, partial, scal, n_wg, which, info, ws, comm=False):
@@ -346,11 +371,14 @@
             0 if t.get(k) is None else t[k].data_ptr() for k in ("obs", "acts", "advs", "rets", "old_values", "old_logp"))
 
         def launch_all():
-            g = self._batch_args(t, hyper, loss_mode, rows_mb, N, n_global, self.partial, self.scal, n_wg, n_wg_pf)
+            img = fused or xrank
+            g = self._batch_args(t, hyper, loss_mode, rows_mb, N, n_global, self.partial, self.scal, n_wg, n_wg_pf, image=img)
             a = self._adam_args((lr_pf, lr_vf), device_state=int(fused or xrank))
+            if img:
+                self._keep_image(a)
             slab = [(idx_dev, self._idx_host), (self.red_ws[2:4], self._hyper_host)] if in_place else []
             self._prologue(pre, t["advs"].reshape(rows_total, N), (self._idx_host if in_place else idx_dev).view(K, rows_mb),
-                           raw, stats[4 * K:], slab)
+                           raw, stats[4 * K:], slab, image=img)
             if fused:
                 fold = self._fold(self._k_fold, self.partial, self.scal, n_wg, n_wg_pf, info, self.red_ws)
             elif xrank:
@@ -452,13 +480,13 @@
 
         def head():
             self._prologue(pre, t["advs"].reshape(rows_total, N), idx_host.view(K, rows_mb), raw, stats2.view(-1)[4 * K:],
-                           [(idx_dev, idx_host), (self.red_ws[2:4], hyper_host), (self.red_ws_v[2:4], hyper_host)])
+                           [(idx_dev, idx_host), (self.red_ws[2:4], hyper_host), (self.red_ws_v[2:4], hyper_host)], image=True)
 
         def chain(net):
             part, scal, ws, wgs, wgs_pf = (self.partial, self.scal, self.red_ws, n_wg_pf, n_wg_pf) if net == 0 else \
                 (partial_v, scal_v, self.red_ws_v, n_wg_vf, -1)
-            g = self._batch_args(t, hyper, loss_mode, rows_mb, N, n_global, part, scal, wgs, wgs_pf)
-            a = self._adam_args((lr_pf, lr_vf), device_state=1)
+            g = self._batch_args(t, hyper, loss_mode, rows_mb, N, n_global, part, scal, wgs, wgs_pf, image=True)
+            a = self._keep_image(self._adam_args((lr_pf, lr_vf), device_state=1))
             _, info, norms = _stat_views(stats2[net], K)
             fold = self._fold(self._k_fold_net_x if xrank else self._k_fold_net, part, scal, wgs, net, info, ws, comm=xrank)
             self._minibatches(K, g, a, idx_dev, raw, norms, fold)
diff --git a/torchrl_amd/algo/on_policy/reinforce.py b/torchrl_amd/algo/on_policy/reinforce.py
--- a/torchrl_amd/algo/on_policy/reinforce.py
+++ b/torchrl_amd/algo/on_policy/reinforce.py
@@ -161,6 +161,7 @@
         self._joint = LastGraph()
         self._pending = None
         self._pro_ws = None
+        self._make_images()
 
     def _n_wg(self, n_samples):
         tiles = (n_samples + 15) // 16
@@ -192,11 +193,13 @@
             t[k].data_ptr() for k in ("obs", "acts", "advs"))
 
         def launch_all():
-            g = self._batch_args(t, hyper, _C.LOSS_REINFORCE, rows_mb, N, n_global, self.partial, self.scal, n_wg, n_wg)
+            g = self._batch_args(t, hyper, _C.LOSS_REINFORCE, rows_mb, N, n_global, self.partial, self.scal, n_wg, n_wg,
+                                 image=True)
             g.vf_params = None
-            a = self._adam_args((lr_pf,), device_state=1)
+            a = self._keep_image(self._adam_args((lr_pf,), device_state=1))
             slab = [(idx_dev, self._idx_host), (self.red_ws[2:4], self._hyper_host)]
-            self._prologue(pre, t["advs"].reshape(rows_total, N), self._idx_host.view(K, rows_mb), raw, stats[4 * K:], slab)
+            self._prologue(pre, t["advs"].reshape(rows_total, N), self._idx_host.view(K, rows_mb), raw, stats[4 * K:], slab,
+                           image=True)
             fold = self._fold(self._k_fold_net, self.partial, self.scal, n_wg, 0, info, self.red_ws)
             self._minibatches(K, g, a, idx_dev, raw, norms, fold)
 
diff --git a/torchrl_amd/csrc/k_ppo.hip b/torchrl_amd/csrc/k_ppo.hip
--- a/torchrl_amd/csrc/k_ppo.hip
+++ b/torchrl_amd/csrc/k_ppo.hip
@@ -2,6 +2,7 @@
 #include "trl_common.h"
 #include "trl_mlp.h"
 #include "trl_head.h"
+#include "trl_ppo_image.h"
 #include "trl_comm.h"
 
 struct PpoDev {
@@ -18,6 +19,7 @@
   double* scal_partial;
   int n_wg, n_pf, p_stride;
   int D, A;
+  const float *pf_image, *vf_image;
 };
 
 template <int D, int H, int A> struct PpoShape {
@@ -207,12 +209,48 @@
       fetch_row(nt + tile_stride);
     }
   };
+  constexpr int NV = H * H / (4 * WV_THREADS);
+  f32x4 wv[NV], wt[NV];
+  float w1[4][5], w3h[4][4], w3t[4][4];
+  float b3v[4], ls_raw[4];
+  constexpr bool IMG_OK = !WIDE && HEAD == HEAD_GAUSS;
+  const f32x4* img = IMG_OK ? reinterpret_cast<const f32x4*>(IS_PF ? a.pf_image : a.vf_image) : nullptr;
+  const bool use_img = IMG_OK && img != nullptr;
+  auto load_image = [&]() {
+    const f32x4* il = img + lane;
+    const f32x4* ig = img + (lane & 48);
+#pragma unroll
+    for (int so = 0; so < 4; ++so) {
+      const f32x4 x = il[(PPO_IMG_S_W1 + so) * 64];
+#pragma unroll
+      for (int r = 0; r < 4; ++r) w1[so][r] = x[r];
+    }
+    const f32x4 c16 = il[PPO_IMG_S_W1C * 64];
+#pragma unroll
+    for (int so = 0; so < 4; ++so) w1[so][4] = c16[so];
+#pragma unroll
+    for (int so = 0; so < 4; ++so) {
+      const f32x4 h = IS_PF ? il[(PPO_IMG_S_W3H + so) * 64] : ig[(PPO_IMG_S_W3H + so) * 64];
+      const f32x4 t = IS_PF ? il[(PPO_IMG_S_W3T + so) * 64] : f32x4{0.f, 0.f, 0.f, 0.f};
+#pragma unroll
+      for (int r = 0; r < 4; ++r) { w3h[so][r] = h[r]; w3t[so][r] = t[r]; }
+    }
+    const f32x4 b3 = IS_PF ? ig[PPO_IMG_S_SC * 64] : f32x4{0.f, 0.f, 0.f, 0.f};
+    const f32x4 ls = IS_PF ? ig[PPO_IMG_S_SC * 64 + 1] : f32x4{0.f, 0.f, 0.f, 0.f};
+#pragma unroll
+    for (int r = 0; r < 4; ++r) { b3v[r] = b3[r]; ls_raw[r] = ls[r]; }
+    const f32x4* iw = il + (PPO_IMG_S_W2T + 4 * __builtin_amdgcn_readfirstlane(wave)) * 64;
+#pragma unroll
+    for (int t = 0; t < NV; ++t) wt[t] = iw[t * 64];
+  };
   if constexpr (CONTIG) {
     const int t0 = __builtin_amdgcn_readfirstlane(tile);
     const int ts = __builtin_amdgcn_readfirstlane(tile_stride);
     st_r = ts / tpr; st_c = ts - st_r * tpr;
     int r0 = t0 / tpr, c0 = t0 - (t0 / tpr) * tpr;
-    fetch_contig(load_ridx(r0), r0, c0);
+    const int64_t ridx0 = load_ridx(r0);
+    if (use_img) load_image();
+    fetch_contig(ridx0, r0, c0);
     p1r = r0; p1c = c0;
     pos_advance(p1r, p1c);
     ridx1 = load_ridx(p1r);
@@ -221,12 +259,11 @@
     ridx2 = load_ridx(p2r);
   } else {
     fetch_row(tile);
+    if (use_img) load_image();
     const int64_t p0 = (tile * 16 + j < B) ? ridx_nn * a.N + e_nn : 0;
     fetch_inputs(p0, tile * 16);
     fetch_row(tile + tile_stride);
   }
-  constexpr int NV = H * H / (4 * WV_THREADS);
-  f32x4 wv[NV], wt[NV];
   const int tc = tid & 63, tq = tid >> 6;
   const float bias1 = tid < H ? gp[F_B1 + tid] : 0.0f, bias2 = tid < H ? gp[F_B2 + tid] : 0.0f;
   {
@@ -240,14 +277,16 @@
         for (int x = 0; x < 4; ++x) wv[t][x] = gp[F_W2 + 4 * (tid + WV_THREADS * t) + x];
       }
     }
-#pragma unroll
-    for (int t = 0; t < NV; ++t)
-#pragma unroll
-      for (int x = 0; x < 4; ++x) wt[t][x] = gp[F_W2 + (4 * (tq + 4 * t) + x) * H + tc];
+    if (!use_img) {
+#pragma unroll
+      for (int t = 0; t < NV; ++t)
+#pragma unroll
+        for (int x = 0; x < 4; ++x) wt[t][x] = gp[F_W2 + (4 * (tq + 4 * t) + x) * H + tc];
+    }
   }
   for (int e = lane; e < 16 * LDT; e += 64) DOS[e] = 0.0f;
-  float w1[4][5], w3h[4][4], w3t[4][4];
   float w1b[4][4];
+  if (!use_img)
 #pragma unroll
   for (int so = 0; so < 4; ++so) {
     const int row = 16 * so + i;
@@ -274,16 +313,21 @@
       }
     }
   }
-  float lsv[4], ivv[4], b3v[4], lspass[4];
+  float lsv[4], ivv[4], lspass[4];
+  if (!use_img)
 #pragma unroll
   for (int r = 0; r < 4; ++r) {
     const int o = 4 * g + r;
-    const float raw = (IS_PF && !CAT && !SDP && o < O) ? gp[F_LS + (o < O ? o : 0)] : 0.0f;
+    ls_raw[r] = (IS_PF && !CAT && !SDP && o < O) ? gp[F_LS + (o < O ? o : 0)] : 0.0f;
+    if constexpr (SDP) b3v[r] = sd_has(o) ? gp[F_B3 + (sd_has(o) ? sd_row(o) : 0)] : 0.0f;
+    else b3v[r] = (o < O) ? gp[F_B3 + (o < O ? o : 0)] : 0.0f;
+  }
+#pragma unroll
+  for (int r = 0; r < 4; ++r) {
+    const float raw = ls_raw[r];
     lsv[r] = fminf(fmaxf(raw, -20.0f), 2.0f);
     ivv[r] = __expf(-2.0f * lsv[r]);
     lspass[r] = (raw >= -20.0f && raw <= 2.0f) ? 1.0f : 0.0f;
-    if constexpr (SDP) b3v[r] = sd_has(o) ? gp[F_B3 + (sd_has(o) ? sd_row(o) : 0)] : 0.0f;
-    else b3v[r] = (o < O) ? gp[F_B3 + (o < O ? o : 0)] : 0.0f;
   }
   const float vb3 = IS_PF ? 0.0f : gp[F_B3];
 #ifdef TRL_EXP_CLK
@@ -986,6 +1030,7 @@
   double* step_state;
   const float* device_lr;
   int self_tick;
+  float* image; const int* img_map;
 };
 __global__ __launch_bounds__(256) void clip_adam_kernel(AdamDev a) {
   __shared__ float s_part[4][4];
@@ -1114,7 +1159,9 @@
   const bool own_ = wave == 0 && pe_ < (net_ == 0 ? p_pf : p_vf);
   const int ge_ = (net_ == 0 ? 0 : p_pf) + pe_;
   float m_old = 0.0f, v_old = 0.0f, p_old = 0.0f;
+  int2 ip_ = make_int2(-1, -1);
   if (own_) { m_old = a.m[ge_]; v_old = a.v[ge_]; p_old = a.params[ge_]; }
+  if (own_ && a.img_map) ip_ = reinterpret_cast<const int2*>(a.img_map)[ge_];
   if (wave < 2 && (only_net < 0 || wave == only_net)) {
     float acc = 0.0f;
     for (int b = lane; b < nb; b += 64) {
@@ -1164,11 +1211,21 @@
       const float g_ = first ? gval0 : grads[ge];
       const float mo = first ? m_old : a.m[ge], vo = first ? v_old : a.v[ge], po = first ? p_old : a.params[ge];
       const float gr = g_ * a.grad_scale * s_coef[net];
-      const float m = a.beta1 * mo + (1.0f - a.beta1) * gr;
-      const float v = a.beta2 * vo + (1.0f - a.beta2) * gr * gr;
+      float m, v;
+      {
+#pragma clang fp contract(off)
+        m = a.beta1 * mo + (1.0f - a.beta1) * gr;
+        v = a.beta2 * vo + (1.0f - a.beta2) * gr * gr;
+      }
       a.m[ge] = m; a.v[ge] = v;
       const float denom = sqrtf(v) / bc2_sqrt + a.eps;
-      a.params[ge] = po - ((net == 0 ? lr_pf : lr_vf) / bc1) * (m / denom);
+      const float pn = __builtin_fmaf(-((net == 0 ? lr_pf : lr_vf) / bc1), m / denom, po);
+      a.params[ge] = pn;
+      if (a.img_map) {
+        const int2 ip = first ? ip_ : reinterpret_cast<const int2*>(a.img_map)[ge];
+        if (ip.x >= 0) a.image[ip.x] = pn;
+        if (ip.y >= 0) a.image[ip.y] = pn;
+      }
     }
   }
 }
@@ -1318,6 +1375,10 @@
   d.partial = p->partial; d.scal_partial = p->scal_partial; d.n_wg = p->n_wg;
   d.n_pf = resolve_pf_wgs(p->n_wg, p->n_wg_pf);
   d.D = D; d.A = A;
+  TRL_REQUIRE((!p->pf_image && !p->vf_image) || ppo_image_supported(D, H, A, head),
+              "this shape's gradient launch takes no operand image (trl_ppo_image_size is 0): pass null images");
+  TRL_REQUIRE((((uintptr_t)p->pf_image | (uintptr_t)p->vf_image) & 15) == 0, "operand images must be 16-byte aligned");
+  d.pf_image = p->pf_image; d.vf_image = p->vf_image;
   hipStream_t s = (hipStream_t)stream;
   d.p_stride = ppo_stride_for(D, H, A, head);
   if (head == HEAD_CAT) d.tanh_action = 0;
@@ -1333,6 +1394,48 @@
 extern "C" int trl_ppo_minibatch_grad_f32(const trl_ppo_batch_t* p, void* stream) { return ppo_grad_launch(p, stream); }
 extern "C" int trl_ppo_cat_minibatch_grad_f32(const trl_ppo_batch_t* p, void* stream) { return ppo_grad_launch(p, stream, HEAD_CAT); }
 extern "C" int trl_ppo_sd_minibatch_grad_f32(const trl_ppo_batch_t* p, void* stream) { return ppo_grad_launch(p, stream, HEAD_SD); }
+
+extern "C" int trl_ppo_image_size(int D, int H, int A) {
+  return ppo_image_supported(D, H, A, HEAD_GAUSS) ? (int)(PPO_IMG_FLOATS * sizeof(float)) : 0;
+}
+extern "C" int trl_ppo_image_map(int D, int H, int A, int32_t* map, int32_t* inverse) {
+  TRL_REQUIRE(map, "null pointer");
+  if (!ppo_image_supported(D, H, A, HEAD_GAUSS)) {
+    trl_set_error("trl_ppo_image_map: shape D=%d H=%d A=%d takes no operand image (H == 64, 2 <= D <= 17, 1 <= A <= 8)", D, H, A);
+    return TRL_EUNSUPPORTED;
+  }
+  const int p_pf = ppo_p_pf(D, H, A, HEAD_GAUSS), p_vf = ppo_p_vf(D, H);
+  if (inverse) for (int q = 0; q < 2 * PPO_IMG_FLOATS; ++q) inverse[q] = -1;
+  for (int e = 0; e < p_pf + p_vf; ++e) {
+    const int net = e < p_pf ? 0 : 1;
+    int pos[2];
+    ppo_image_positions(net, D, A, HEAD_GAUSS, e - net * p_pf, pos);
+    for (int k = 0; k < 2; ++k) {
+      map[2 * e + k] = pos[k] < 0 ? -1 : pos[k] + net * PPO_IMG_FLOATS;
+      if (inverse && pos[k] >= 0) inverse[pos[k] + net * PPO_IMG_FLOATS] = e;
+    }
+  }
+  return TRL_OK;
+}
+__global__ __launch_bounds__(256) void ppo_image_build_kernel(const float* __restrict__ flat, const int4* __restrict__ inverse,
+                                                              f32x4* __restrict__ image, int n4) {
+  const int q = blockIdx.x * 256 + threadIdx.x;
+  if (q >= n4) return;
+  const int4 s = inverse[q];
+  f32x4 v;
+  v[0] = s.x >= 0 ? flat[s.x] : 0.0f; v[1] = s.y >= 0 ? flat[s.y] : 0.0f;
+  v[2] = s.z >= 0 ? flat[s.z] : 0.0f; v[3] = s.w >= 0 ? flat[s.w] : 0.0f;
+  image[q] = v;
+}
+extern "C" int trl_ppo_image_build_f32(const float* flat, const int32_t* inverse, float* image, void* stream) {
+  TRL_REQUIRE(flat && inverse && image, "null pointer");
+  TRL_REQUIRE((((uintptr_t)inverse | (uintptr_t)image) & 15) == 0, "inverse and image must be 16-byte aligned");
+  const int n4 = 2 * PPO_IMG_FLOATS / 4;
+  hipLaunchKernelGGL(ppo_image_build_kernel, dim3(trl_ceil_div(n4, 256)), dim3(256), 0, (hipStream_t)stream, flat,
+                     reinterpret_cast<const int4*>(inverse), reinterpret_cast<f32x4*>(image), n4);
+  TRL_LAUNCH_CHECK();
+  return TRL_OK;
+}
 
 static int launch_reduce(const float* partial, const double* scal_partial, int n_wg, int n_wg_pf, int D, int H, int A,
                          const float* pf_params, float* grads, double* info, void* stream, int head) {
@@ -1364,7 +1467,7 @@
   return launch_reduce(partial, scal_partial, n_wg, n_wg_pf, D, H, A, pf_params, grads, info, stream, HEAD_SD);
 }
 
-static int fill_adam(const trl_adam_t* p, AdamDev& d) {
+static int fill_adam(const trl_adam_t* p, AdamDev& d, bool with_image = false) {
   if (!p) { trl_set_error("clip_adam: null descriptor"); return TRL_EINVAL; }
   TRL_REQUIRE(p->params && p->grads && p->exp_avg && p->exp_avg_sq, "null pointer");
   TRL_REQUIRE(p->n_groups >= 1 && p->n_groups <= 4, "n_groups must be 1..4");
@@ -1385,6 +1488,10 @@
   d.step_state = p->step_state;
   d.device_lr = p->device_lr;
   d.self_tick = 0;
+  TRL_REQUIRE(with_image || (!p->image && !p->image_map), "image / image_map belong to trl_ppo_reduce_adam_*_f32");
+  TRL_REQUIRE(!p->image == !p->image_map, "image and image_map come together");
+  TRL_REQUIRE((((uintptr_t)p->image) & 15) == 0 && (((uintptr_t)p->image_map) & 7) == 0, "image: 16-byte, image_map: 8-byte aligned");
+  d.image = p->image; d.img_map = p->image_map;
   return TRL_OK;
 }
 
@@ -1405,8 +1512,9 @@
   const int ps = ppo_stride_for(D, H, A, head);
   if (ps < 0) return ps;
   AdamDev d;
-  int rc = fill_adam(adam, d);
+  int rc = fill_adam(adam, d, true);
   if (rc) return rc;
+  TRL_REQUIRE(!adam->image_map || ppo_image_supported(D, H, A, head), "this shape's gradient launch takes no operand image");
   const int p_pf = ppo_p_pf(D, H, A, head), p_vf = ppo_p_vf(D, H);
   TRL_REQUIRE((adam->n_groups == 2 && adam->group_sizes[0] == p_pf && adam->group_sizes[1] == p_vf) ||
               (only_net == 0 && !xr && adam->n_groups == 1 && adam->group_sizes[0] == p_pf),
diff --git a/torchrl_amd/csrc/trl_ppo_image.h b/torchrl_amd/csrc/trl_ppo_image.h
--- /dev/null
+++ b/torchrl_amd/csrc/trl_ppo_image.h
@@ -0,0 +1,50 @@
+#pragma once
+#include "trl_head.h"
+
+#define PPO_IMG_S_W1 0
+#define PPO_IMG_S_W1C 4
+#define PPO_IMG_S_W3H 5
+#define PPO_IMG_S_W3T 9
+#define PPO_IMG_S_SC 13
+#define PPO_IMG_S_W2T 14
+#define PPO_IMG_SLOTS 30
+#define PPO_IMG_FLOATS (PPO_IMG_SLOTS * 64 * 4)
+
+__host__ __device__ inline bool ppo_image_supported(int D, int H, int A, int head) {
+  return head == HEAD_GAUSS && H == 64 && D >= 2 && D <= 17 && A >= 1 && A <= 8;
+}
+
+__host__ __device__ inline int ppo_image_pos(int slot, int lane, int comp) { return (slot * 64 + lane) * 4 + comp; }
+
+__host__ __device__ inline int ppo_image_positions(int net, int D, int A, int head, int e, int pos[2]) {
+  (void)head;
+  const int H = 64, O = net == 0 ? A : 1;
+  const int F_B1 = H * D, F_W2 = F_B1 + H, F_B2 = F_W2 + H * H, F_W3 = F_B2 + H, F_B3 = F_W3 + O * H, F_LS = F_B3 + O,
+            F_END = net == 0 ? F_LS + O : F_LS;
+  pos[0] = pos[1] = -1;
+  if (e < 0 || e >= F_END) return 0;
+  if (e < F_B1) {
+    const int row = e / D, col = e - row * D, so = row >> 4, i = row & 15;
+    pos[0] = col < 16 ? ppo_image_pos(PPO_IMG_S_W1 + so, i + 16 * (col >> 2), col & 3) : ppo_image_pos(PPO_IMG_S_W1C, i, so);
+    return 1;
+  }
+  if (e < F_W2) return 0;
+  if (e < F_B2) {
+    const int r = (e - F_W2) >> 6, c = (e - F_W2) & 63, q = r >> 2;
+    pos[0] = ppo_image_pos(PPO_IMG_S_W2T + 4 * (q & 3) + (q >> 2), c, r & 3);
+    return 1;
+  }
+  if (e < F_W3) return 0;
+  if (e < F_B3) {
+    const int o = (e - F_W3) >> 6, k = (e - F_W3) & 63, so = k >> 4;
+    if (net == 1) { pos[0] = ppo_image_pos(PPO_IMG_S_W3H + so, 16 * ((k >> 2) & 3), k & 3); return 1; }
+    pos[0] = ppo_image_pos(PPO_IMG_S_W3H + so, o + 16 * ((k >> 2) & 3), k & 3);
+    pos[1] = ppo_image_pos(PPO_IMG_S_W3T + so, (k & 15) + 16 * (o >> 2), o & 3);
+    return 2;
+  }
+  if (net == 1) return 0;
+  const bool ls = e >= F_LS;
+  const int o = e - (ls ? F_LS : F_B3);
+  pos[0] = ppo_image_pos(PPO_IMG_S_SC, 16 * (o >> 2) + (ls ? 1 : 0), o & 3);
+  return 1;
+}
```

After: 100.6 million (median of 3 runs). About the same (-0.3%).
